# grantjr1842/index-tts

Measured on AMD Instinct MI355X. Metric: synthesised audio seconds per second (IndexTTS-2 infer_v2 hot path), whole job, higher is better.
Workload: dtype f32 (greedy decode + its prefill: exact fp32 MFMA; fp32 accumulate and fp32 activations everywhere) + split-bf16 (fp32 operands as hi+lo bf16, 3 bf16 MFMAs per product) GEMMs, DiT attention and convolutions in s2mel, the latent pass and the vocoder; GPT linear weights STORED as bf16 (rounded once at

## Files before the change

include/idxtts.h:

```cpp
#ifndef IDXTTS_H
#define IDXTTS_H

#include <stddef.h>
#include <stdint.h>

#ifdef __cplusplus
extern "C" {
#endif

typedef struct idxtts_ctx idxtts_ctx;

#define IDXTTS_DTYPE_F32 0
#define IDXTTS_DTYPE_F16 1
#define IDXTTS_DTYPE_BF16 2

int idxtts_version(void);
const char* idxtts_last_error(void);

int idxtts_aa_act_fwd(void* out, const void* in, const float* up_filter, const float* down_filter,
                      const float* log_alpha, const float* log_beta, int B, int C, int T, int dtype,
                      void* stream);

typedef struct idxtts_conv1d idxtts_conv1d;
int idxtts_conv1d_create(const float* weight, const float* bias , int Cout, int Cin, int K,
                         int transposed_stride ,
                         idxtts_conv1d** out);
int idxtts_conv1d_fwd(const idxtts_conv1d* conv, const float* x, float* y, const float* residual ,
                      int B, int T, int dilation, int pad_left, int pad_mode, float scale, int accumulate,
                      void* stream);
int idxtts_conv1d_destroy(idxtts_conv1d* conv);

int idxtts_ctx_load_tensor(idxtts_ctx* ctx, const char* name, const float* data, const int64_t* shape, int ndim);
int idxtts_ctx_finalize(idxtts_ctx* ctx);
int idxtts_ctx_get_tensor(idxtts_ctx* ctx, const char* name, float* host_out, size_t capacity);
int idxtts_ctx_destroy(idxtts_ctx* ctx);
float idxtts_fp8_e4m3_decode(unsigned char code);
unsigned char idxtts_fp8_e4m3_encode(float v);

typedef struct idxtts_bigvgan_config {
  int num_mels;
  int upsample_initial_channel;
  int num_upsamples;
  int upsample_rates[8];
  int upsample_kernel_sizes[8];
  int num_kernels;
  int resblock_kernel_sizes[4];
  int resblock_dilations[4][3];
} idxtts_bigvgan_config;

int idxtts_bigvgan_create(const idxtts_bigvgan_config* cfg, idxtts_ctx** out);
size_t idxtts_bigvgan_workspace_bytes(const idxtts_ctx* ctx, int B, int Tm);
int idxtts_bigvgan_fwd(idxtts_ctx* ctx, const float* mel, float* wav, int B, int Tm, void* workspace,
                       size_t workspace_bytes, int clamp, int stage_idx, float* stage_out, void* stream);
int idxtts_bigvgan_fwd_ragged(idxtts_ctx* ctx, const float* mel, const int* mel_lengths, float* wav, int B, int Tm, void* workspace,
                              size_t workspace_bytes, int clamp, void* stream);

typedef struct idxtts_linear idxtts_linear;
int idxtts_linear_create(const float* weight, const float* bias , int N, int K, int weight_is_kn,
                         idxtts_linear** out);
int idxtts_linear_fwd(const idxtts_linear* lin, const float* x, int ldx, float* y, int ldy, const float* residual ,
                      int ldr, int M, int act, int bf16x3 ,
                      void* stream);
int idxtts_set_gemm_mode(int mode);
int idxtts_get_gemm_mode(void);
int idxtts_set_decode_geometry(int narrow);
int idxtts_get_decode_geometry(void);
int idxtts_set_decode_plane_rows(int min_rows);
int idxtts_get_decode_plane_rows(void);
int idxtts_s2mel_set_overlap(int on);
int idxtts_s2mel_get_overlap(void);
int idxtts_linear_destroy(idxtts_linear* lin);
int idxtts_release_stream(void* stream);
int idxtts_attention_fwd(const float* q, const float* k, const float* v, float* o, long q_batch_stride, int q_token_stride,
                         long kv_batch_stride, int kv_token_stride, long o_batch_stride, int o_token_stride, int B, int H,
                         int Sq, int Sk, int causal, const int* kstart, const int* kend, float scale, void* stream);
int idxtts_attention_bf16x3_fwd(const float* q, const float* k, const float* v, float* o, long q_batch_stride, int q_token_stride,
                         long kv_batch_stride, int kv_token_stride, long o_batch_stride, int o_token_stride, int B, int H,
                         int Sq, int Sk, int causal, const int* kstart, const int* kend, float scale, void* stream);
int idxtts_attention_relkey_fwd(const float* q, const float* k, const float* v, float* o, long batch_stride, int token_stride,
                                long o_batch_stride, int o_token_stride, int B, int H, int S, const int* kend, float scale,
                                const float* rel_key, int rel_left, int rel_right, int split_bf16, void* stream);
int idxtts_layernorm_fwd(const float* x, float* y, const float* gamma, const float* beta, int M, int d, float eps, void* stream);

typedef struct idxtts_gpt_config {
  int model_dim, heads, layers;
  int number_mel_codes;
  int number_text_tokens;
  int start_mel_token, stop_mel_token;
  int mel_pos_len, text_pos_len;
} idxtts_gpt_config;
int idxtts_gpt_create(const idxtts_gpt_config* cfg, idxtts_ctx** out);
int idxtts_gpt_quantize_weights(idxtts_ctx* ctx, int format);
int idxtts_gpt_set_kv_format(idxtts_ctx* ctx, int format);
int idxtts_gpt_get_kv_format(const idxtts_ctx* ctx);
int idxtts_gpt_graph_cache_entries(idxtts_ctx* ctx);
size_t idxtts_gpt_workspace_bytes(const idxtts_ctx* ctx, int B, int S, int max_new_tokens);
int idxtts_gpt_embed(idxtts_ctx* ctx, float* out, int rows, const int* text_ids, const int* text_pos_idx, const int* mel_ids,
                     const int* mel_pos_idx, const float* extra, const int* extra_idx, void* stream);
int idxtts_gpt_generate(idxtts_ctx* ctx, const float* inputs_embeds, const int* pad_left, int B, int P, int max_new_tokens,
                        float repetition_penalty, long long* codes, int* n_steps, float* logits_out, void* workspace,
                        size_t workspace_bytes, int use_graph, void* stream);
int idxtts_gpt_generate_forced(idxtts_ctx* ctx, const float* inputs_embeds, const int* pad_left, int B, int P, int max_new_tokens,
                               float repetition_penalty, const long long* forced_codes, long long* codes, int* n_steps, float* logits_out,
                               void* workspace, size_t workspace_bytes, void* stream);
typedef struct idxtts_sampling {
  int mode;
  float temperature;
  int top_k;
  float top_p;
  const float* exp_noise;
  unsigned long long seed;
} idxtts_sampling;
int idxtts_gpt_generate_sampled(idxtts_ctx* ctx, const float* inputs_embeds, const int* pad_left, int B, int P, int max_new_tokens,
                                float repetition_penalty, const idxtts_sampling* sampling, long long* codes, int* n_steps,
                                float* logits_out, void* workspace, size_t workspace_bytes, int use_graph, void* stream);
typedef struct idxtts_beam {
  int num_beams;
  int do_sample;
  float temperature;
  int top_k;
  float top_p;
  float length_penalty;
  int early_stopping;
  const float* exp_noise;
  unsigned long long seed;
} idxtts_beam;
size_t idxtts_gpt_beam_workspace_bytes(const idxtts_ctx* ctx, int B, int num_beams, int S, int max_new_tokens);
int idxtts_gpt_generate_beam(idxtts_ctx* ctx, const float* inputs_embeds, const int* pad_left, int B, int P, int max_new_tokens,
                             float repetition_penalty, const idxtts_beam* beam, long long* codes, int* n_steps, void* workspace,
                             size_t workspace_bytes, int use_graph, void* stream);
size_t idxtts_gpt_session_workspace_bytes(const idxtts_ctx* ctx, int slots, int max_prompt, int max_new_tokens);
int idxtts_gpt_session_init(idxtts_ctx* ctx, int slots, int max_prompt, int max_new_tokens, float repetition_penalty, void* workspace,
                            size_t workspace_bytes, void* stream);
int idxtts_gpt_session_admit(idxtts_ctx* ctx, int n, const float* inputs_embeds, int ld_rows, const int* prompt_lens,
                             const int* slot_ids, const int* max_new_tokens, void* workspace, void* stream);
#define IDXTTS_SESSION_SAMPLED 1
size_t idxtts_gpt_session_workspace_bytes_ex(const idxtts_ctx* ctx, int slots, int max_prompt, int max_new_tokens, int flags);
int idxtts_gpt_session_init_ex(idxtts_ctx* ctx, int slots, int max_prompt, int max_new_tokens, float repetition_penalty, int flags,
                               void* workspace, size_t workspace_bytes, void* stream);
int idxtts_gpt_session_admit_sampled(idxtts_ctx* ctx, int n, const float* inputs_embeds, int ld_rows, const int* prompt_lens,
                                     const int* slot_ids, const int* max_new_tokens, const idxtts_sampling* per_row, void* workspace,
                                     void* stream);
size_t idxtts_gpt_session_workspace_bytes_beam(const idxtts_ctx* ctx, int slots, int num_beams, int max_prompt, int max_new_tokens);
int idxtts_gpt_session_init_beam(idxtts_ctx* ctx, int slots, int num_beams, int max_prompt, int max_new_tokens, float repetition_penalty,
                                 void* workspace, size_t workspace_bytes, void* stream);
int idxtts_gpt_session_admit_beam(idxtts_ctx* ctx, int n, const float* inputs_embeds, int ld_rows, const int* prompt_lens,
                                  const int* group_ids, const int* max_new_tokens, const idxtts_beam* per_request, void* workspace,
                                  void* stream);
int idxtts_gpt_session_step(idxtts_ctx* ctx, int n_steps, int use_graph, int* finished_slots, int* n_finished, void* workspace,
                            void* stream);
int idxtts_gpt_session_read(idxtts_ctx* ctx, int slot, long long* codes, int* n_codes, void* workspace, void* stream);
int idxtts_gpt_session_release(idxtts_ctx* ctx, void* workspace);
int idxtts_gpt_latent(idxtts_ctx* ctx, const float* emb, const int* pad_left, int B, int S, int mel_start, int M, float* latent,
                      void* workspace, size_t workspace_bytes, void* stream);

typedef struct idxtts_cond_config {
  int input_size;
  int output_size, linear_units, attention_heads, num_blocks, cnn_kernel;
  int perceiver_dim, num_latents, perceiver_depth, perceiver_dim_head, perceiver_mult;
  int emotion;
  int model_dim;
} idxtts_cond_config;
int idxtts_cond_create(const idxtts_cond_config* cfg, idxtts_ctx** out);
size_t idxtts_cond_workspace_bytes(const idxtts_ctx* ctx, int B, int T);
int idxtts_cond_forward(idxtts_ctx* ctx, const float* feats, const int* lengths, int B, int T, float* out, void* workspace,
                        size_t workspace_bytes, void* stream);
int idxtts_emovec_merge(float* out, const float* base, const float* emo, float alpha, size_t n, void* stream);

typedef struct idxtts_w2vbert_config {
  int input_dim, hidden_size, num_heads, intermediate_size;
  int num_layers;
  int left_max, right_max, conv_kernel;
  float layer_norm_eps;
} idxtts_w2vbert_config;
int idxtts_w2vbert_create(const idxtts_w2vbert_config* cfg, idxtts_ctx** out);
size_t idxtts_w2vbert_workspace_bytes(const idxtts_ctx* ctx, int B, int T);
int idxtts_w2vbert_forward(idxtts_ctx* ctx, const float* feats, const int* lengths, int B, int T, float* out, void* workspace,
                           size_t workspace_bytes, void* stream);

typedef struct idxtts_repcodec_config {
  int hidden_size, codebook_size, codebook_dim;
  int vocos_dim, vocos_intermediate_dim, vocos_num_layers;
} idxtts_repcodec_config;
int idxtts_repcodec_create(const idxtts_repcodec_config* cfg, idxtts_ctx** out);
size_t idxtts_repcodec_workspace_bytes(const idxtts_ctx* ctx, int B, int T);
int idxtts_repcodec_quantize(idxtts_ctx* ctx, const float* x, int B, int T, long long* indices, float* quantized, void* workspace,
                             size_t workspace_bytes, void* stream);

typedef struct idxtts_melspec_config {
  int n_fft, hop_size, win_size, num_mels;
} idxtts_melspec_config;
int idxtts_melspec_create(const idxtts_melspec_config* cfg, idxtts_ctx** out);
int idxtts_melspec_frames(const idxtts_ctx* ctx, int n_samples);
size_t idxtts_melspec_workspace_bytes(const idxtts_ctx* ctx, int B, int n_samples);
int idxtts_melspec_forward(idxtts_ctx* ctx, const float* audio, int B, int n_samples, float* mel, void* workspace, size_t workspace_bytes,
                           void* stream);

typedef struct idxtts_campplus_config {
  int feat_dim, embedding_size;
  int m_channels, growth_rate, bn_size, init_channels;
  int num_blocks;
  int block_layers[4], block_dilation[4];
} idxtts_campplus_config;
int idxtts_campplus_create(const idxtts_campplus_config* cfg, idxtts_ctx** out);
size_t idxtts_campplus_workspace_bytes(const idxtts_ctx* ctx, int T);
int idxtts_campplus_forward(idxtts_ctx* ctx, const float* feat, int B, int T, float* style, void* workspace, size_t workspace_bytes, void* stream);

typedef struct idxtts_s2mel_config {
  int hidden_dim, num_heads, depth;
  int in_channels, content_dim, style_dim;
  int wn_hidden, wn_layers, wn_kernel, wn_dilation_rate;
  int lr_channels, lr_in_channels, lr_num_convs;
  int gpt_dim; int gpt_layer_dims[3];
  int codebook_size, codebook_dim, codec_hidden;
  float norm_eps;
} idxtts_s2mel_config;
int idxtts_s2mel_create(const idxtts_s2mel_config* cfg, idxtts_ctx** out);
size_t idxtts_s2mel_cond_workspace_bytes(const idxtts_ctx* ctx, int B, int M, int Tg);
int idxtts_s2mel_prepare_cond(idxtts_ctx* ctx, const float* latent, const long long* codes, const int* code_lens,
                              const int* target_lens, int B, int M, int Tg, float* cond_out, void* workspace,
                              size_t workspace_bytes, void* stream);
int idxtts_s2mel_regulate(idxtts_ctx* ctx, const float* S, const int* in_lens, const int* target_lens, int B, int M, int Tg, float* cond_out,
                          void* workspace, size_t workspace_bytes, void* stream);
size_t idxtts_s2mel_cfm_workspace_bytes(const idxtts_ctx* ctx, int B, int T, int n_steps);
int idxtts_s2mel_cfm(idxtts_ctx* ctx, const float* mu, const int* x_lens, const float* prompt, const int* prompt_lens, int Tp_max,
                     const float* style, const float* z, const float* t_emb, const float* dt, int n_steps, float cfg_rate,
                     float* out, int B, int T, void* workspace, size_t workspace_bytes, void* stream);

size_t idxtts_s2mel_cfm_rows_workspace_bytes(const idxtts_ctx* ctx, int B, int T, int Tp_max, int n_steps);
int idxtts_s2mel_cfm_rows(idxtts_ctx* ctx, const float* gen_cond, const int* target_lens, int Tg_max, const float* const* prompt_conditions,
                          const float* const* ref_mels, const int* prompt_lens, const float* style, const float* z, const float* t_emb,
                          const float* dt, int n_steps, float cfg_rate, float* out, int B, int T, void* workspace, size_t workspace_bytes,
                          void* stream);

int idxtts_s2mel_estimator(idxtts_ctx* ctx, const float* x, const float* prompt, const int* prompt_lens, int Tp_max, const int* x_lens,
                           const float* t_emb, const float* style, const float* mu, float* out, int B, int T, void* workspace,
                           size_t workspace_bytes, void* stream);

typedef struct idxtts_qwen_config {
  int vocab_size;
  int hidden_size;
  int intermediate_size;
  int num_hidden_layers;
  int num_attention_heads;
  int num_key_value_heads;
  int head_dim;
  float rms_norm_eps;
  float rope_theta;
  int tie_word_embeddings;
  int max_context;
} idxtts_qwen_config;
int idxtts_qwen_create(const idxtts_qwen_config* cfg, idxtts_ctx** out);
int idxtts_qwen_set_weight_format(idxtts_ctx* ctx, int format);
size_t idxtts_qwen_workspace_bytes(const idxtts_ctx* ctx, int n_prompt, int max_new_tokens, int n_eos, int n_logit_cols );
int idxtts_qwen_generate(idxtts_ctx* ctx, const int* prompt_ids, int n_prompt, int max_new_tokens, const int* eos_ids, int n_eos,
                         const int* forced_ids , int* out_ids, int* n_out, float* out_logits ,
                         const int* logit_cols , int n_logit_cols, void* workspace, size_t bytes, int use_graph,
                         void* stream);
int idxtts_qwen_step_graph_launches(const idxtts_ctx* ctx);
int idxtts_qwen_max_batch(const idxtts_ctx* ctx);
size_t idxtts_qwen_batch_workspace_bytes(const idxtts_ctx* ctx, int B, const int* n_prompt, const int* max_new_tokens, int n_eos,
                                         int n_logit_cols );
int idxtts_qwen_generate_batch(idxtts_ctx* ctx, int B, const int* prompt_ids, const int* n_prompt, const int* max_new_tokens,
                               const int* eos_ids, int n_eos, const int* forced_ids , int* out_ids, int* n_out,
                               float* out_logits , const int* logit_cols , int n_logit_cols,
                               void* workspace, size_t bytes, int use_graph, void* stream);
int idxtts_qwen_batch_step_graph_launches(const idxtts_ctx* ctx);

int idxtts_profile_enable(int on);
int idxtts_profile_num_kernels(void);
const char* idxtts_profile_kernel_name(int index);
int idxtts_profile_read(int index, double* total_ms, double* flops, double* bytes, long* launches);
int idxtts_profile_event_overhead(void* stream, int launches, double* avg_ms);

#ifdef __cplusplus
}
#endif
#endif
```

index-tts_amd/csrc/capi.hip:

```cpp
#include <cstring>
#include <new>

#include "../../include/idxtts.h"
#include "bigvgan.h"
#include "cond.h"
#include "semantic.h"
#include "codec.h"
#include "audio.h"
#include "campplus.h"
#include "conv1d.h"
#include "ctx.h"
#include "gpt.h"
#include "model_util.h"
#include "s2mel.h"

namespace idxtts {

static thread_local std::string g_last_error;

void set_error(const std::string& msg) { g_last_error = msg; }
int fail(const char* file, int line, const std::string& msg) {
  const char* base = std::strrchr(file, '/');
  g_last_error = std::string(base ? base + 1 : file) + ":" + std::to_string(line) + ": " + msg;
  return 1;
// ... 466 lines not shown
                               static_cast<hipStream_t>(stream));
  API_END
}

int idxtts_gpt_session_step(idxtts_ctx* ctx, int n_steps, int use_graph, int* finished_slots, int* n_finished, void* workspace,
                            void* stream) {
  API_BEGIN
  GPT_MODEL(ctx);
  return m->session_step(workspace, n_steps, use_graph, finished_slots, n_finished, static_cast<hipStream_t>(stream));
  API_END
}

int idxtts_gpt_session_read(idxtts_ctx* ctx, int slot, long long* codes, int* n_codes, void* workspace, void* stream) {
  API_BEGIN
  GPT_MODEL(ctx);
  return m->session_read(workspace, slot, codes, n_codes, static_cast<hipStream_t>(stream));
  API_END
}

int idxtts_gpt_session_release(idxtts_ctx* ctx, void* workspace) {
  API_BEGIN
  GPT_MODEL(ctx);
  return m->session_release(workspace);
  API_END
}

int idxtts_gpt_latent(idxtts_ctx* ctx, const float* emb, const int* pad_left, int B, int S, int mel_start, int M, float* latent,
                      void* workspace, size_t workspace_bytes, void* stream) {
  API_BEGIN
  GPT_MODEL(ctx);
  return m->latent(emb, pad_left, B, S, mel_start, M, latent, workspace, workspace_bytes, static_cast<hipStream_t>(stream));
  API_END
}


int idxtts_cond_create(const idxtts_cond_config* cfg, idxtts_ctx** out) {
  API_BEGIN
  IDX_CHECK(cfg && out, "null pointer");
  std::unique_ptr<idxtts_ctx> ctx(new idxtts_ctx());
  ctx->model.reset(new CondModel(*cfg));
  *out = ctx.release();
  return 0;
  API_END
}

size_t idxtts_cond_workspace_bytes(const idxtts_ctx* ctx, int B, int T) {
  if (!ctx || !ctx->finalized || B <= 0 || T < 3) return 0;
  auto* m = dynamic_cast<const CondModel*>(ctx->model.get());
  return m ? m->workspace_bytes(B, T) : 0;
}

int idxtts_cond_forward(idxtts_ctx* ctx, const float* feats, const int* lengths, int B, int T, float* out, void* workspace,
                        size_t workspace_bytes, void* stream) {
  API_BEGIN
  IDX_CHECK(ctx, "null ctx");
  IDX_CHECK(ctx->finalized, "context not finalized");
  auto* m = dynamic_cast<CondModel*>(ctx->model.get());
  IDX_CHECK(m, "not a conditioning-encoder context");
  return m->forward(feats, lengths, B, T, out, workspace, workspace_bytes, static_cast<hipStream_t>(stream));
  API_END
}

int idxtts_w2vbert_create(const idxtts_w2vbert_config* cfg, idxtts_ctx** out) {
  API_BEGIN
  IDX_CHECK(cfg && out, "null pointer");
  std::unique_ptr<idxtts_ctx> ctx(new idxtts_ctx());
  ctx->model.reset(new W2VBertModel(*cfg));
  *out = ctx.release();
  return 0;
  API_END
}

size_t idxtts_w2vbert_workspace_bytes(const idxtts_ctx* ctx, int B, int T) {
  if (!ctx || !ctx->finalized || B <= 0 || T <= 0) return 0;
  auto* m = dynamic_cast<const W2VBertModel*>(ctx->model.get());
  return m ? m->workspace_bytes(B, T) : 0;
}

int idxtts_w2vbert_forward(idxtts_ctx* ctx, const float* feats, const int* lengths, int B, int T, float* out, void* workspace,
                           size_t workspace_bytes, void* stream) {
  API_BEGIN
  IDX_CHECK(ctx, "null ctx");
  IDX_CHECK(ctx->finalized, "context not finalized");
  auto* m = dynamic_cast<W2VBertModel*>(ctx->model.get());
  IDX_CHECK(m, "not a w2v-bert context");
  return m->forward(feats, lengths, B, T, out, workspace, workspace_bytes, static_cast<hipStream_t>(stream));
  API_END
}

int idxtts_repcodec_create(const idxtts_repcodec_config* cfg, idxtts_ctx** out) {
  API_BEGIN
  IDX_CHECK(cfg && out, "null pointer");
  std::unique_ptr<idxtts_ctx> ctx(new idxtts_ctx());
  ctx->model.reset(new RepCodecModel(*cfg));
  *out = ctx.release();
  return 0;
  API_END
}

size_t idxtts_repcodec_workspace_bytes(const idxtts_ctx* ctx, int B, int T) {
  if (!ctx || !ctx->finalized || B <= 0 || T <= 0) return 0;
  auto* m = dynamic_cast<const RepCodecModel*>(ctx->model.get());
  return m ? m->workspace_bytes(B, T) : 0;
}

int idxtts_repcodec_quantize(idxtts_ctx* ctx, const float* x, int B, int T, long long* indices, float* quantized, void* workspace,
                             size_t workspace_bytes, void* stream) {
  API_BEGIN
  IDX_CHECK(ctx, "null ctx");
  IDX_CHECK(ctx->finalized, "context not finalized");
  auto* m = dynamic_cast<RepCodecModel*>(ctx->model.get());
  IDX_CHECK(m, "not a semantic-codec context");
  return m->quantize(x, B, T, indices, quantized, workspace, workspace_bytes, static_cast<hipStream_t>(stream));
  API_END
}

int idxtts_melspec_create(const idxtts_melspec_config* cfg, idxtts_ctx** out) {
  API_BEGIN
  IDX_CHECK(cfg && out, "null pointer");
  std::unique_ptr<idxtts_ctx> ctx(new idxtts_ctx());
  ctx->model.reset(new MelSpecModel(*cfg));
  *out = ctx.release();
  return 0;
  API_END
}

int idxtts_melspec_frames(const idxtts_ctx* ctx, int n_samples) {
  if (!ctx || n_samples <= 0) return 0;
  auto* m = dynamic_cast<const MelSpecModel*>(ctx->model.get());
  return m ? m->frames(n_samples) : 0;
}

size_t idxtts_melspec_workspace_bytes(const idxtts_ctx* ctx, int B, int n_samples) {
  if (!ctx || !ctx->finalized || B <= 0 || n_samples <= 0) return 0;
  auto* m = dynamic_cast<const MelSpecModel*>(ctx->model.get());
  return m ? m->workspace_bytes(B, n_samples) : 0;
}

int idxtts_melspec_forward(idxtts_ctx* ctx, const float* audio, int B, int n_samples, float* mel, void* workspace, size_t workspace_bytes,
                           void* stream) {
  API_BEGIN
  IDX_CHECK(ctx, "null ctx");
  IDX_CHECK(ctx->finalized, "context not finalized");
  auto* m = dynamic_cast<MelSpecModel*>(ctx->model.get());
  IDX_CHECK(m, "not a mel-spectrogram context");
  return m->forward(audio, B, n_samples, mel, workspace, workspace_bytes, static_cast<hipStream_t>(stream));
  API_END
}

int idxtts_campplus_create(const idxtts_campplus_config* cfg, idxtts_ctx** out) {
  API_BEGIN
  IDX_CHECK(cfg && out, "null pointer");
  std::unique_ptr<idxtts_ctx> ctx(new idxtts_ctx());
  ctx->model.reset(new CamPPlusModel(*cfg));
  *out = ctx.release();
  return 0;
  API_END
}

size_t idxtts_campplus_workspace_bytes(const idxtts_ctx* ctx, int T) {
  if (!ctx || !ctx->finalized || T < 8) return 0;
  auto* m = dynamic_cast<const CamPPlusModel*>(ctx->model.get());
  return m ? m->workspace_bytes(T) : 0;
}

int idxtts_campplus_forward(idxtts_ctx* ctx, const float* feat, int B, int T, float* style, void* workspace, size_t workspace_bytes, void* stream) {
  API_BEGIN
  IDX_CHECK(ctx, "null ctx");
  IDX_CHECK(ctx->finalized, "context not finalized");
  auto* m = dynamic_cast<CamPPlusModel*>(ctx->model.get());
  IDX_CHECK(m, "not a CAMPPlus context");
  return m->forward(feat, B, T, style, workspace, workspace_bytes, static_cast<hipStream_t>(stream));
  API_END
}

int idxtts_emovec_merge(float* out, const float* base, const float* emo, float alpha, size_t n, void* stream) {
  API_BEGIN
  return lerp_rows(out, base, emo, alpha, n, static_cast<hipStream_t>(stream));
  API_END
}

int idxtts_s2mel_create(const idxtts_s2mel_config* cfg, idxtts_ctx** out) {
  API_BEGIN
  IDX_CHECK(cfg && out, "null pointer");
  std::unique_ptr<idxtts_ctx> ctx(new idxtts_ctx());
  ctx->model.reset(new S2MelModel(*cfg));
  *out = ctx.release();
  return 0;
  API_END
}

#define S2MEL_MODEL(ctx)                                      \
  IDX_CHECK(ctx, "null ctx");                                 \
  IDX_CHECK(ctx->finalized, "context not finalized");         \
  auto* m = dynamic_cast<S2MelModel*>(ctx->model.get());      \
  IDX_CHECK(m, "not an s2mel context")

size_t idxtts_s2mel_cond_workspace_bytes(const idxtts_ctx* ctx, int B, int M, int Tg) {
  if (!ctx || !ctx->finalized || B <= 0 || M <= 0 || Tg <= 0) return 0;
  auto* m = dynamic_cast<const S2MelModel*>(ctx->model.get());
  return m ? m->cond_workspace_bytes(B, M, Tg) : 0;
}

int idxtts_s2mel_prepare_cond(idxtts_ctx* ctx, const float* latent, const long long* codes, const int* code_lens,
                              const int* target_lens, int B, int M, int Tg, float* cond_out, void* workspace,
                              size_t workspace_bytes, void* stream) {
  API_BEGIN
  S2MEL_MODEL(ctx);
  return m->prepare_cond(latent, codes, code_lens, target_lens, B, M, Tg, cond_out, workspace, workspace_bytes,
                         static_cast<hipStream_t>(stream));
  API_END
}

int idxtts_s2mel_regulate(idxtts_ctx* ctx, const float* S, const int* in_lens, const int* target_lens, int B, int M, int Tg, float* cond_out,
                          void* workspace, size_t workspace_bytes, void* stream) {
  API_BEGIN
  S2MEL_MODEL(ctx);
  return m->regulate(S, in_lens, target_lens, B, M, Tg, cond_out, workspace, workspace_bytes, static_cast<hipStream_t>(stream));
  API_END
}

size_t idxtts_s2mel_cfm_workspace_bytes(const idxtts_ctx* ctx, int B, int T, int n_steps) {
  if (!ctx || !ctx->finalized || B <= 0 || T <= 0 || n_steps <= 0) return 0;
  auto* m = dynamic_cast<const S2MelModel*>(ctx->model.get());
  return m ? m->cfm_workspace_bytes(B, T, n_steps) : 0;
}

int idxtts_s2mel_cfm(idxtts_ctx* ctx, const float* mu, const int* x_lens, const float* prompt, const int* prompt_lens, int Tp_max,
                     const float* style, const float* z, const float* t_emb, const float* dt, int n_steps, float cfg_rate,
                     float* out, int B, int T, void* workspace, size_t workspace_bytes, void* stream) {
  API_BEGIN
  S2MEL_MODEL(ctx);
  return m->cfm(mu, x_lens, prompt, prompt_lens, Tp_max, style, z, t_emb, dt, n_steps, cfg_rate, out, B, T, workspace,
                workspace_bytes, static_cast<hipStream_t>(stream));
  API_END
}

size_t idxtts_s2mel_cfm_rows_workspace_bytes(const idxtts_ctx* ctx, int B, int T, int Tp_max, int n_steps) {
  if (!ctx || !ctx->finalized || B <= 0 || T <= 0 || Tp_max <= 0 || n_steps <= 0) return 0;
  auto* m = dynamic_cast<const S2MelModel*>(ctx->model.get());
  return m ? m->cfm_rows_workspace_bytes(B, T, Tp_max, n_steps) : 0;
}

int idxtts_s2mel_cfm_rows(idxtts_ctx* ctx, const float* gen_cond, const int* target_lens, int Tg_max, const float* const* prompt_conditions,
                          const float* const* ref_mels, const int* prompt_lens, const float* style, const float* z, const float* t_emb,
                          const float* dt, int n_steps, float cfg_rate, float* out, int B, int T, void* workspace, size_t workspace_bytes,
                          void* stream) {
  API_BEGIN
  S2MEL_MODEL(ctx);
  return m->cfm_rows(gen_cond, target_lens, Tg_max, prompt_conditions, ref_mels, prompt_lens, style, z, t_emb, dt, n_steps, cfg_rate, out,
                     B, T, workspace, workspace_bytes, static_cast<hipStream_t>(stream));
  API_END
}

int idxtts_s2mel_estimator(idxtts_ctx* ctx, const float* x, const float* prompt, const int* prompt_lens, int Tp_max, const int* x_lens,
                           const float* t_emb, const float* style, const float* mu, float* out, int B, int T, void* workspace,
                           size_t workspace_bytes, void* stream) {
  API_BEGIN
  S2MEL_MODEL(ctx);
  return m->estimator(x, prompt, prompt_lens, Tp_max, x_lens, t_emb, style, mu, out, B, T, workspace, workspace_bytes,
                      static_cast<hipStream_t>(stream));
  API_END
}


int idxtts_set_gemm_mode(int mode) {
  set_gemm_mode(mode);
  return 0;
}

int idxtts_get_gemm_mode(void) { return get_gemm_mode(); }

int idxtts_set_decode_geometry(int narrow) {
  set_decode_geometry(narrow);
  return 0;
}

int idxtts_get_decode_geometry(void) { return get_decode_geometry(); }

int idxtts_release_stream(void* stream) {
  API_BEGIN
  hipStream_t st = static_cast<hipStream_t>(stream);
  return gemm_release_stream_scratch(st) || s2mel_release_stream(st);
  API_END
}

int idxtts_set_decode_plane_rows(int min_rows) {
  API_BEGIN
  IDX_CHECK(min_rows == 0 || (min_rows >= 5 && min_rows <= 65), "0 (default), 5..64 or 65 (off)");
  set_decode_plane_rows(min_rows);
  return 0;
  API_END
}

int idxtts_get_decode_plane_rows(void) { return get_decode_plane_rows(); }

int idxtts_s2mel_set_overlap(int on) {
  set_s2mel_overlap(on);
  return 0;
}

int idxtts_s2mel_get_overlap(void) { return get_s2mel_overlap(); }

}
```

index-tts_amd/csrc/gemm.h:

```cpp
#pragma once
#include "common.h"

namespace idxtts {

enum GemmAct { ACT_NONE = 0, ACT_GELU_NEW = 1, ACT_SILU = 2, ACT_SWIGLU = 3, ACT_MISH = 4, ACT_GATE = 5 ,
               ACT_GELU_ERF = 6 , ACT_RELU = 7  };

struct LinearWeights {
  const float* wp = nullptr;
  const float* bias = nullptr;
  int N = 0, K = 0;
  const void* wp16 = nullptr;
};

static inline size_t linear_packed_floats(int N, int K) { return (size_t)cdiv(N, 32) * cdiv(K, 16) * 512; }

void pack_linear(float* dst, const float* w, int N, int K);

struct GemmArgs {
  const float* x = nullptr; int ldx = 0;
  float* y = nullptr; int ldy = 0;
  const void* x_planes = nullptr;
  void* y_planes = nullptr;
  const float* rope = nullptr; int rope_T = 0, rope_cols = 0;
  const float* res = nullptr; int ldr = 0;
  int M = 0;
  int act = ACT_NONE;
  float out_scale = 1.0f;
  int taps = 1, seq_len = 0, dil = 1, pad_left = 0, pad_mode = 0;
  const int* row_len = nullptr;
  int ksplit = 1;
};

int gemm_tn_forward(const LinearWeights& w, const GemmArgs& a, hipStream_t stream);
int gemm_bf16x3_forward(const LinearWeights& w, const GemmArgs& a, hipStream_t stream);
size_t linear_bf16x3_packed_bytes(int N, int K);
void pack_linear_bf16x3(void* dst, const float* w, int N, int K);

enum GemmMode { GEMM_F32 = 0, GEMM_BF16X3 = 1 };
void set_gemm_mode(int mode);
int get_gemm_mode();
int gemm_forward(const LinearWeights& w, const GemmArgs& a, hipStream_t stream);
bool gemm_uses_planes(const LinearWeights& w, const GemmArgs& a);

int gemm_release_stream_scratch(hipStream_t stream);

}
```

index-tts_amd/csrc/gemm.hip:

```cpp
#include <algorithm>
#include <cmath>

#include "device_util.h"
#include "gemm_common.h"
#include "prof.h"

namespace idxtts {

void pack_linear(float* dst, const float* w, int N, int K) {
  const int NT = cdiv(N, 32), KC = cdiv(K, 16);
  for (int nt = 0; nt < NT; ++nt)
    for (int c = 0; c < KC; ++c) {
      float* sub = dst + ((size_t)nt * KC + c) * 512;
      for (int g = 0; g < 2; ++g)
        for (int h = 0; h < 2; ++h)
          for (int j = 0; j < 32; ++j)
            for (int e = 0; e < 4; ++e) {
              const int n = nt * 32 + j, k = c * 16 + 8 * g + 4 * h + e;
              sub[((g * 2 + h) * 32 + j) * 4 + e] = (n < N && k < K) ? w[(size_t)n * K + k] : 0.0f;
            }
    }
}

constexpr int XBLK = 132;

int StreamScratch::acquire(hipStream_t stream, size_t bytes, void** out, bool* grew) {
  int dev_id = 0;
  IDX_HIP(hipGetDevice(&dev_id));
  Block* b = nullptr;
  {
    std::lock_guard<std::mutex> lock(mu_);
    b = &blocks_[std::make_pair(dev_id, stream)];
  }
  const bool grow = b->bytes < bytes;
  if (grew) *grew = grow;
  if (grow) {
    if (b->ptr) IDX_HIP(hipFreeAsync(b->ptr, stream));
    b->ptr = nullptr; b->bytes = 0;
    const size_t nb = bytes + (headroom_div_ ? bytes / headroom_div_ : 0);
    IDX_HIP(hipMallocAsync(&b->ptr, nb, stream));
    b->bytes = nb;
  }
  *out = b->ptr;
  return 0;
}

int StreamScratch::release(hipStream_t stream) {
  int dev_id = 0;
  IDX_HIP(hipGetDevice(&dev_id));
  Block b;
  {
    std::lock_guard<std::mutex> lock(mu_);
    auto it = blocks_.find(std::make_pair(dev_id, stream));
    if (it == blocks_.end()) return 0;
    b = it->second;
    blocks_.erase(it);
  }
  if (b.ptr) IDX_HIP(hipFreeAsync(b.ptr, stream));
  return 0;
}

static StreamScratch g_sk_scratch;
int gemm_release_stream_scratch(hipStream_t stream) { return g_plane_scratch.release(stream) || g_sk_scratch.release(stream); }

__global__ __launch_bounds__(256) void gemm_tn_kernel(const GemmKP p) {
  extern __shared__ __attribute__((aligned(16))) float smem[];
  float (*Xs)[4 * 2 * 4 * XBLK] = reinterpret_cast<float (*)[4 * 2 * 4 * XBLK]>(smem);
  float (*Ws)[4 * 2 * 512] = reinterpret_cast<float (*)[4 * 2 * 512]>(smem + 2 * 4 * 2 * 4 * XBLK);

  const int L = blockIdx.x, xcd = L & 7, q = L >> 3;
  int bn, bm;
  if (p.direct_map) { bn = L / p.mtiles; bm = L - bn * p.mtiles; }
  else if (p.n_fast) { const int bml = q / p.nblocks; bn = q - bml * p.nblocks; bm = bml * 8 + xcd; }
  else { bn = q / p.mt8; bm = (q - bn * p.mt8) * 8 + xcd; }
  if (bm >= p.mtiles) return;

  const int tid = threadIdx.x, wave = tid >> 6, lane = tid & 63;
  const int h = lane >> 5, j = lane & 31;
  const int wm = wave >> 1, wn = wave & 1;

  f32x4 xr[4], wr[4];
  int seq_base[4], seq_t[4], seq_n[4];
  if (p.taps > 1) {
#pragma unroll
    for (int l = 0; l < 4; ++l) {
      const int m = bm * 128 + ((tid + 256 * l) >> 3);
      const int sb = m / p.seq_len;
      seq_base[l] = sb * p.seq_len;
      seq_t[l] = m - sb * p.seq_len;
      seq_n[l] = (p.row_len && m < p.M) ? min(p.row_len[sb], p.seq_len) : p.seq_len;
    }
  }
  auto load_tiles = [&](int kstep) {
    int tap = 0, kk0 = kstep * 32;
    if (p.taps > 1) { tap = kk0 / p.kc; kk0 -= tap * p.kc; }
#pragma unroll
    for (int l = 0; l < 4; ++l) {
      const int idx = tid + 256 * l;
      const int row = idx >> 3, q8 = idx & 7;
      const int m = bm * 128 + row, k = kstep * 32 + q8 * 4;
      f32x4 v = {0.f, 0.f, 0.f, 0.f};
      if (p.taps > 1) {
        int t = seq_t[l] + tap * p.dil - p.pad_left;
        if (p.pad_mode == 1) { t = t < 0 ? -t : t; t = t >= seq_n[l] ? 2 * (seq_n[l] - 1) - t : t; }
        if (m < p.M && k < p.K && t >= 0 && t < seq_n[l])
          v = *reinterpret_cast<const f32x4*>(p.x + (size_t)(seq_base[l] + t) * p.ldx + kk0 + q8 * 4);
      } else if (m < p.M && k < p.K) {
        v = *reinterpret_cast<const f32x4*>(p.x + (size_t)m * p.ldx + k);
      }
      xr[l] = v;
      const int nt = idx >> 8, off = idx & 255;
      const int ntg = bn * 4 + nt, c16 = kstep * 2 + (off >> 7);
      f32x4 u = {0.f, 0.f, 0.f, 0.f};
      if (ntg * 32 < p.N && c16 < p.kc16)
        u = *reinterpret_cast<const f32x4*>(p.wp + ((size_t)ntg * p.kc16 + c16) * 512 + (off & 127) * 4);
      wr[l] = u;
    }
  };
  auto store_tiles = [&](int buf) {
#pragma unroll
    for (int l = 0; l < 4; ++l) {
      const int idx = tid + 256 * l;
      const int row = idx >> 3, q8 = idx & 7;
      const int mt = row >> 5, i = row & 31, c = q8 >> 2, gh = q8 & 3;
      *reinterpret_cast<f32x4*>(&Xs[buf][((mt * 2 + c) * 4 + gh) * XBLK + i * 4]) = xr[l];
      const int nt = idx >> 8, off = idx & 255;
      *reinterpret_cast<f32x4*>(&Ws[buf][nt * 1024 + off * 4]) = wr[l];
    }
  };

  f32x16 acc[2][2], tot[2][2];
#pragma unroll
  for (int a = 0; a < 2; ++a)
#pragma unroll
    for (int b = 0; b < 2; ++b)
#pragma unroll
      for (int r = 0; r < 16; ++r) { acc[a][b][r] = 0.0f; tot[a][b][r] = 0.0f; }

  int ksteps = (p.kc16 + 1) >> 1, ks0 = 0;
  if (p.ksplit > 1) { ks0 = blockIdx.y * p.ksteps_per_split; ksteps = min(ksteps, ks0 + p.ksteps_per_split); }
  int in_group = ks0 % p.kg;
  load_tiles(ks0);
  store_tiles(ks0 & 1);
  __syncthreads();
  for (int ks = ks0; ks < ksteps; ++ks) {
    const bool has_next = ks + 1 < ksteps;
    if (has_next) load_tiles(ks + 1);
    const float* xb = Xs[ks & 1];
    const float* wb = Ws[ks & 1];
#pragma unroll
    for (int c = 0; c < 2; ++c)
#pragma unroll
      for (int g = 0; g < 2; ++g) {
        f32x4 a[2], b[2];
#pragma unroll
        for (int t = 0; t < 2; ++t) {
          a[t] = *reinterpret_cast<const f32x4*>(xb + (((wm * 2 + t) * 2 + c) * 4 + (g * 2 + h)) * XBLK + j * 4);
          b[t] = *reinterpret_cast<const f32x4*>(wb + (wn * 2 + t) * 1024 + c * 512 + (g * 64 + lane) * 4);
        }
#pragma unroll
        for (int s = 0; s < 4; ++s)
#pragma unroll
          for (int mt = 0; mt < 2; ++mt)
#pragma unroll
            for (int nt = 0; nt < 2; ++nt)
              acc[mt][nt] = __builtin_amdgcn_mfma_f32_32x32x2f32(a[mt][s], b[nt][s], acc[mt][nt], 0, 0, 0);
      }
    if (++in_group == p.kg || !has_next) {
      in_group = 0;
#pragma unroll
      for (int mt = 0; mt < 2; ++mt)
#pragma unroll
        for (int nt = 0; nt < 2; ++nt)
#pragma unroll
          for (int r = 0; r < 16; ++r) { tot[mt][nt][r] += acc[mt][nt][r]; acc[mt][nt][r] = 0.0f; }
    }
    if (has_next) store_tiles((ks + 1) & 1);
    __syncthreads();
  }

  if (p.sk_cnt) {
    const __amdgpu_buffer_rsrc_t rs = __builtin_amdgcn_make_buffer_rsrc(p.sk_slab, 0, p.sk_slab_bytes, 0x00020000);
    const int tile = bm * p.nblocks + bn, ntiles = p.mtiles * p.nblocks;
    const int part_stride = ntiles * 16 * 256 * 16;
    const int mine = (tile * 16 * 256 + tid) * 16;
#pragma unroll
    for (int mt = 0; mt < 2; ++mt)
#pragma unroll
      for (int nt = 0; nt < 2; ++nt)
#pragma unroll
        for (int r4 = 0; r4 < 4; ++r4) {
          const f32x4 v = {tot[mt][nt][4 * r4], tot[mt][nt][4 * r4 + 1], tot[mt][nt][4 * r4 + 2], tot[mt][nt][4 * r4 + 3]};
          __builtin_amdgcn_raw_buffer_store_b128(__builtin_bit_cast(u32x4, v), rs, mine + ((mt * 2 + nt) * 4 + r4) * 4096, (int)blockIdx.y * part_stride, 17);
        }
    if (!wg_arrive_last(&p.sk_cnt[tile], (unsigned)p.ksplit)) return;
#pragma unroll
    for (int mt = 0; mt < 2; ++mt)
#pragma unroll
      for (int nt = 0; nt < 2; ++nt)
#pragma unroll
        for (int r = 0; r < 16; ++r) tot[mt][nt][r] = 0.0f;
    for (int g = 0; g < p.ksplit; ++g) {
      u32x4 t[16];
#pragma unroll
      for (int u = 0; u < 16; ++u) t[u] = __builtin_amdgcn_raw_buffer_load_b128(rs, mine + u * 4096, g * part_stride, 16);
#pragma unroll
      for (int u = 0; u < 16; ++u) {
        const f32x4 v = __builtin_bit_cast(f32x4, t[u]);
#pragma unroll
        for (int e = 0; e < 4; ++e) tot[u >> 3][(u >> 2) & 1][4 * (u & 3) + e] += v[e];
      }
    }
    gemm_epilogue(p, tot, bm, bn, wm, wn, h, j);
    return;
  }
  if (p.ksplit > 1) {
    GemmKP q = p;
    q.y = p.y + (size_t)blockIdx.y * p.M * p.ldy;
    q.bias = nullptr; q.res = nullptr; q.row_len = nullptr; q.act = ACT_NONE; q.out_scale = 1.0f;
    gemm_epilogue(q, tot, bm, bn, wm, wn, h, j);
    return;
  }
  gemm_epilogue(p, tot, bm, bn, wm, wn, h, j);
}

int gemm_prepare(const LinearWeights& w, const GemmArgs& a, GemmKP* out, double* flops, double* bytes) {
  IDX_CHECK(a.M > 0 && w.N > 0 && w.K > 0, "bad shape");
  IDX_CHECK((w.K & 3) == 0 && (a.ldx & 3) == 0, "K and ldx must be multiples of 4 (16-byte row segments)");
  IDX_CHECK((reinterpret_cast<uintptr_t>(a.x) & 15) == 0, "x must be 16-byte aligned");
  if (a.act == ACT_SWIGLU || a.act == ACT_GATE) IDX_CHECK((w.N & 63) == 0, "paired activations need N (= 2*hidden) to be a multiple of 64");
  if (a.taps > 1) {
    IDX_CHECK(a.seq_len > 0 && a.M % a.seq_len == 0 && w.K % a.taps == 0 && ((w.K / a.taps) & 31) == 0, "conv mode: K/taps must be a multiple of 32 and M a multiple of seq_len");
    if (a.pad_mode == 1) IDX_CHECK(a.seq_len > (a.taps - 1) * a.dil, "reflect pad needs seq_len > halo");
  }
  if (a.row_len) IDX_CHECK(a.seq_len > 0, "row_len needs seq_len");
  GemmKP p;
  p.x = a.x; p.wp = w.wp; p.bias = w.bias; p.res = a.res; p.y = a.y; p.y_hi = p.y_lo = nullptr; p.rope = nullptr; p.rope_T = 1; p.rope_cols = 0;
  p.M = a.M; p.N = w.N; p.K = w.K; p.ldx = a.ldx; p.ldy = a.ldy; p.ldr = a.ldr;
  p.kc16 = cdiv(w.K, 16);
  p.mtiles = cdiv(a.M, 128);
  p.mt8 = cdiv(p.mtiles, 8);
  p.nblocks = cdiv(w.N, 128);
  p.n_fast = ((double)w.N * w.K * 4.0 <= 8.0 * 1024 * 1024) && a.M > w.N ? 1 : 0;
  p.act = a.act; p.out_scale = a.out_scale;
  p.taps = a.taps; p.kc = w.K / std::max(1, a.taps); p.seq_len = a.seq_len > 0 ? a.seq_len : 1; p.dil = a.dil; p.pad_left = a.pad_left;
  p.pad_mode = a.pad_mode; p.row_len = a.row_len;
  p.ksplit = 1; p.ksteps_per_split = 0;
  p.kg = 0; p.direct_map = 0; p.sk_slab = nullptr; p.sk_cnt = nullptr; p.sk_slab_bytes = 0;
  IDX_CHECK((int64_t)8 * p.nblocks * p.mt8 < (1ll << 31), "grid size");
  *out = p;
  *flops = 2.0 * a.M * (double)w.N * w.K;
  *bytes = 4.0 * ((double)a.M * w.K + (double)w.N * w.K + (double)a.M * w.N * (a.res ? 2.0 : 1.0));
  return 0;
}

int gemm_tn_forward(const LinearWeights& w, const GemmArgs& a, hipStream_t stream) {
  IDX_CHECK(w.wp && a.x && a.y, "null pointer");
  if (a.M == 0) return 0;
  IDX_CHECK(!a.y_planes && !a.rope, "the fp32 GEMM takes and produces fp32 rows only (no fused rotary)");
  GemmKP p;
  double flops, bytes;
  if (gemm_prepare(w, a, &p, &flops, &bytes)) return 1;
  p.ksplit = std::max(1, a.ksplit);
  p.ksteps_per_split = cdiv(cdiv(p.kc16, 2), p.ksplit);
  if (p.ksplit > 1) {
    IDX_CHECK(a.taps <= 1 && a.act == ACT_NONE && !a.res && !a.row_len, "split-K launches produce raw partial slabs");
    IDX_CHECK((p.ksplit - 1) * p.ksteps_per_split < cdiv(p.kc16, 2), "ksplit leaves an empty K range");
  }
  const int ksteps_all = cdiv(p.kc16, 2);
  p.kg = std::max(5, cdiv(ksteps_all, 8));
  const int ngroups = cdiv(ksteps_all, p.kg);
  const int tiles = p.nblocks * p.mtiles;
  if (p.ksplit == 1 && tiles <= 96 && ngroups >= 2) {
    const size_t slab_bytes = (size_t)ngroups * tiles * 65536, cnt_bytes = 4096;
    static_assert(96 * 4 <= 4096, "arrival counters");
    void* sc = nullptr;
    bool grew = false;
    if (g_sk_scratch.acquire(stream, cnt_bytes + slab_bytes, &sc, &grew)) return 1;
    if (grew) IDX_HIP(hipMemsetAsync(sc, 0, cnt_bytes, stream));
    p.sk_cnt = static_cast<unsigned*>(sc);
    p.sk_slab = reinterpret_cast<float*>(static_cast<char*>(sc) + cnt_bytes);
    p.sk_slab_bytes = (int)slab_bytes;
    p.ksplit = ngroups; p.ksteps_per_split = p.kg;
  }
  if (tiles <= 96) p.direct_map = 1;
  const int64_t grid = p.direct_map ? (int64_t)tiles : (int64_t)8 * p.nblocks * p.mt8;
  static const int cat = prof_register("gemm_tn_kernel");
  ProfScope prof(cat, stream, flops, bytes);
  constexpr size_t lds = (size_t)(2 * 4 * 2 * 4 * XBLK + 2 * 4 * 2 * 512) * sizeof(float);
  static DynLdsLimit lds_limit;
  IDX_HIP(lds_limit.set((int)lds, gemm_tn_kernel));
  hipLaunchKernelGGL(gemm_tn_kernel, dim3((unsigned)grid, (unsigned)p.ksplit), dim3(256), lds, stream, p);
  IDX_LAUNCH_CHECK();
  return 0;
}

static int g_gemm_mode = GEMM_BF16X3;
void set_gemm_mode(int mode) { g_gemm_mode = mode == GEMM_F32 ? GEMM_F32 : GEMM_BF16X3; }
int get_gemm_mode() { return g_gemm_mode; }

bool gemm_bf16x3_uses_v2(const LinearWeights& w, const GemmArgs& a);
bool gemm_uses_planes(const LinearWeights& w, const GemmArgs& a) {
  return g_gemm_mode == GEMM_BF16X3 && w.wp16 && a.M >= 256 && gemm_bf16x3_uses_v2(w, a);
}
int gemm_forward(const LinearWeights& w, const GemmArgs& a, hipStream_t stream) {
  if (g_gemm_mode == GEMM_BF16X3 && w.wp16 && a.M >= 256) return gemm_bf16x3_forward(w, a, stream);
  return gemm_tn_forward(w, a, stream);
}

}
```

index-tts_amd/csrc/gemm_bf16x3.hip:

```cpp
#include <algorithm>
#include <cmath>
#include <cstdlib>
#include <cstring>

#include "gemm_common.h"
#include "prof.h"

namespace idxtts {

__device__ __forceinline__ int cdiv_dev(int a, int b) { return (a + b - 1) / b; }

typedef __bf16 bf16x8 __attribute__((ext_vector_type(8)));
typedef __bf16 bf16x4 __attribute__((ext_vector_type(4)));

constexpr int BROW = 40;
constexpr int TILE_HALF = 128 * BROW;
constexpr int WTILE_BYTES = 2 * TILE_HALF * 2;

size_t linear_planes_bytes(int N, int K);
void pack_linear_planes(void* dst, const float* w, int N, int K);
bool gemm_bf16x3_uses_v2(const LinearWeights& w, const GemmArgs& a);
int gemm_bf16x3_v2_forward(GemmKP p, const void* wplanes, const LinearWeights& w, const GemmArgs& a, hipStream_t stream, double flops,
                           double bytes);
bool gemm_bf16x3_uses_v2(const LinearWeights& w, const GemmArgs& a) {
  return w.wp16 && a.M >= 256 && w.N >= 96 && w.K % 16 == 0 && (a.taps <= 1 || (w.K / a.taps) % 16 == 0);
}
static size_t tiles_bytes(int N, int K) { return (size_t)cdiv(N, 128) * cdiv(K, 32) * WTILE_BYTES; }
size_t linear_bf16x3_packed_bytes(int N, int K) { return tiles_bytes(N, K) + linear_planes_bytes(N, K); }

void pack_linear_bf16x3(void* dst, const float* w, int N, int K) {
  uint16_t* o = static_cast<uint16_t*>(dst);
  const int NB = cdiv(N, 128), KS = cdiv(K, 32);
  std::memset(o, 0, tiles_bytes(N, K));
  pack_linear_planes(static_cast<char*>(dst) + tiles_bytes(N, K), w, N, K);
  for (int nb = 0; nb < NB; ++nb)
    for (int ks = 0; ks < KS; ++ks) {
      uint16_t* tile = o + ((size_t)nb * KS + ks) * (2 * TILE_HALF);
      for (int r = 0; r < 128; ++r) {
        const int n = nb * 128 + r;
        if (n >= N) break;
        for (int kk = 0; kk < 32; ++kk) {
          const int k = ks * 32 + kk;
          if (k >= K) break;
          const float x = w[(size_t)n * K + k];
          const uint16_t hi = f2bf(x);
          tile[r * BROW + kk] = hi;
          tile[TILE_HALF + r * BROW + kk] = f2bf(x - bf2f(hi));
        }
      }
    }
}

__global__ __launch_bounds__(256) void gemm_bf16x3_kernel(const GemmKP p) {
  extern __shared__ __attribute__((aligned(16))) __bf16 sm16[];
  __bf16* As = sm16;
  __bf16* Bs = sm16 + 2 * 2 * TILE_HALF;

  const int L = blockIdx.x, xcd = L & 7, q = L >> 3;
  int bn, bm;
  if (p.n_fast) { const int bml = q / p.nblocks; bn = q - bml * p.nblocks; bm = bml * 8 + xcd; }
  else { bn = q / p.mt8; bm = (q - bn * p.mt8) * 8 + xcd; }
  if (bm >= p.mtiles) return;

  const int tid = threadIdx.x, wave = tid >> 6, lane = tid & 63;
  const int h = lane >> 5, j = lane & 31;
  const int wm = wave >> 1, wn = wave & 1;
  const int ksteps = (p.K + 31) >> 5;

  f32x4 xr[4];
  f32x4 wr[5];
  int seq_base[4], seq_t[4], seq_n[4];
  if (p.taps > 1) {
#pragma unroll
    for (int l = 0; l < 4; ++l) {
      const int m = bm * 128 + ((tid + 256 * l) >> 3);
      const int sb = m / p.seq_len;
      seq_base[l] = sb * p.seq_len;
      seq_t[l] = m - sb * p.seq_len;
      seq_n[l] = (p.row_len && m < p.M) ? min(p.row_len[sb], p.seq_len) : p.seq_len;
    }
  }
  const char* wtile0 = reinterpret_cast<const char*>(p.wp) + (size_t)bn * ksteps * WTILE_BYTES;
  auto load_tiles = [&](int kstep) {
    int tap = 0, kk0 = kstep * 32;
    if (p.taps > 1) { tap = kk0 / p.kc; kk0 -= tap * p.kc; }
#pragma unroll
    for (int l = 0; l < 4; ++l) {
      const int idx = tid + 256 * l;
      const int row = idx >> 3, q8 = idx & 7;
      const int m = bm * 128 + row, k = kstep * 32 + q8 * 4;
      f32x4 v = {0.f, 0.f, 0.f, 0.f};
      if (p.taps > 1) {
        int t = seq_t[l] + tap * p.dil - p.pad_left;
        if (p.pad_mode == 1) { t = t < 0 ? -t : t; t = t >= seq_n[l] ? 2 * (seq_n[l] - 1) - t : t; }
        if (m < p.M && k < p.K && t >= 0 && t < seq_n[l])
          v = *reinterpret_cast<const f32x4*>(p.x + (size_t)(seq_base[l] + t) * p.ldx + kk0 + q8 * 4);
      } else if (m < p.M && k < p.K) {
        v = *reinterpret_cast<const f32x4*>(p.x + (size_t)m * p.ldx + k);
      }
      xr[l] = v;
    }
    const f32x4* wsrc = reinterpret_cast<const f32x4*>(wtile0 + (size_t)kstep * WTILE_BYTES);
#pragma unroll
    for (int l = 0; l < 5; ++l) wr[l] = wsrc[tid + 256 * l];
  };
  auto store_tiles = [&](int buf) {
    __bf16* a_hi = As + buf * 2 * TILE_HALF;
    __bf16* a_lo = a_hi + TILE_HALF;
#pragma unroll
    for (int l = 0; l < 4; ++l) {
      const int idx = tid + 256 * l;
      const int row = idx >> 3, q8 = idx & 7;
      const bf16x4 hi = __builtin_convertvector(xr[l], bf16x4);
      const f32x4 back = __builtin_convertvector(hi, f32x4);
      const bf16x4 lo = __builtin_convertvector(xr[l] - back, bf16x4);
      *reinterpret_cast<bf16x4*>(a_hi + row * BROW + q8 * 4) = hi;
      *reinterpret_cast<bf16x4*>(a_lo + row * BROW + q8 * 4) = lo;
    }
    f32x4* wdst = reinterpret_cast<f32x4*>(Bs + buf * 2 * TILE_HALF);
#pragma unroll
    for (int l = 0; l < 5; ++l) wdst[tid + 256 * l] = wr[l];
  };

  f32x16 acc[2][2];
#pragma unroll
  for (int a = 0; a < 2; ++a)
#pragma unroll
    for (int b = 0; b < 2; ++b)
#pragma unroll
      for (int r = 0; r < 16; ++r) acc[a][b][r] = 0.0f;

  load_tiles(0);
  store_tiles(0);
  __syncthreads();
  for (int ks = 0; ks < ksteps; ++ks) {
    const bool has_next = ks + 1 < ksteps;
    if (has_next) load_tiles(ks + 1);
    const __bf16* a_hi = As + (ks & 1) * 2 * TILE_HALF;
    const __bf16* b_hi = Bs + (ks & 1) * 2 * TILE_HALF;
#pragma unroll
    for (int s = 0; s < 2; ++s) {
      bf16x8 ah[2], al[2], bh[2], bl[2];
#pragma unroll
      for (int t = 0; t < 2; ++t) {
        const int ar = (wm * 64 + t * 32 + j) * BROW + s * 16 + h * 8;
        const int br = (wn * 64 + t * 32 + j) * BROW + s * 16 + h * 8;
        ah[t] = *reinterpret_cast<const bf16x8*>(a_hi + ar);
        al[t] = *reinterpret_cast<const bf16x8*>(a_hi + TILE_HALF + ar);
        bh[t] = *reinterpret_cast<const bf16x8*>(b_hi + br);
        bl[t] = *reinterpret_cast<const bf16x8*>(b_hi + TILE_HALF + br);
      }
#pragma unroll
      for (int mt = 0; mt < 2; ++mt)
#pragma unroll
        for (int nt = 0; nt < 2; ++nt) {
          acc[mt][nt] = __builtin_amdgcn_mfma_f32_32x32x16_bf16(al[mt], bh[nt], acc[mt][nt], 0, 0, 0);
          acc[mt][nt] = __builtin_amdgcn_mfma_f32_32x32x16_bf16(ah[mt], bl[nt], acc[mt][nt], 0, 0, 0);
          acc[mt][nt] = __builtin_amdgcn_mfma_f32_32x32x16_bf16(ah[mt], bh[nt], acc[mt][nt], 0, 0, 0);
        }
    }
    if (has_next) store_tiles((ks + 1) & 1);
    __syncthreads();
  }
  gemm_epilogue(p, acc, bm, bn, wm, wn, h, j);
}

template <int TN>
__global__ __launch_bounds__(512) void gemm_bf16x3_big_kernel(const GemmKP p) {
  constexpr int BN = 64 * TN;
  constexpr int NB128 = BN / 128 > 0 ? BN / 128 : 1;
  constexpr int A_HALF = 256 * BROW;
  constexpr int B_HALF = TILE_HALF;
  constexpr int A_STAGE = 2 * A_HALF, B_STAGE = NB128 * 2 * B_HALF;
  constexpr int NWL = (NB128 * 1280 + 511) / 512;
  static_assert(BN == 128 || BN == 256, "tile");
  extern __shared__ __attribute__((aligned(16))) __bf16 sm16[];
  __bf16* As = sm16;
  __bf16* Bs = sm16 + 2 * A_STAGE;

  const int L = blockIdx.x, xcd = L & 7, q = L >> 3;
  int bn, bm;
  if (p.n_fast) { const int bml = q / p.nblocks; bn = q - bml * p.nblocks; bm = bml * 8 + xcd; }
  else { bn = q / p.mt8; bm = (q - bn * p.mt8) * 8 + xcd; }
  if (bm >= p.mtiles) return;

  const int tid = threadIdx.x, wave = tid >> 6, lane = tid & 63;
  const int h = lane >> 5, j = lane & 31;
  const int wm = wave >> 1, wn = wave & 1;
  const int ksteps = (p.K + 31) >> 5;

  f32x4 xr[4];
  f32x4 wr[NWL];
  int seq_base[4], seq_t[4], seq_n[4];
  if (p.taps > 1) {
#pragma unroll
    for (int l = 0; l < 4; ++l) {
      const int m = bm * 256 + ((tid + 512 * l) >> 3);
      const int sb = m / p.seq_len;
      seq_base[l] = sb * p.seq_len;
      seq_t[l] = m - sb * p.seq_len;
      seq_n[l] = (p.row_len && m < p.M) ? min(p.row_len[sb], p.seq_len) : p.seq_len;
    }
  }
  const int n128 = cdiv_dev(p.N, 128);
  auto load_tiles = [&](int kstep) {
    int tap = 0, kk0 = kstep * 32;
    if (p.taps > 1) { tap = kk0 / p.kc; kk0 -= tap * p.kc; }
#pragma unroll
    for (int l = 0; l < 4; ++l) {
      const int idx = tid + 512 * l;
      const int row = idx >> 3, q8 = idx & 7;
      const int m = bm * 256 + row, k = kstep * 32 + q8 * 4;
      f32x4 v = {0.f, 0.f, 0.f, 0.f};
      if (p.taps > 1) {
        int t = seq_t[l] + tap * p.dil - p.pad_left;
        if (p.pad_mode == 1) { t = t < 0 ? -t : t; t = t >= seq_n[l] ? 2 * (seq_n[l] - 1) - t : t; }
        if (m < p.M && k < p.K && t >= 0 && t < seq_n[l])
          v = *reinterpret_cast<const f32x4*>(p.x + (size_t)(seq_base[l] + t) * p.ldx + kk0 + q8 * 4);
      } else if (m < p.M && k < p.K) {
        v = *reinterpret_cast<const f32x4*>(p.x + (size_t)m * p.ldx + k);
      }
      xr[l] = v;
    }
#pragma unroll
    for (int l = 0; l < NWL; ++l) {
      const int idx = tid + 512 * l;
      const int sub = idx / 1280, off = idx - sub * 1280;
      const int nb = bn * NB128 + sub;
      f32x4 v = {0.f, 0.f, 0.f, 0.f};
      if (idx < NB128 * 1280 && nb < n128)
        v = reinterpret_cast<const f32x4*>(reinterpret_cast<const char*>(p.wp) + ((size_t)nb * ksteps + kstep) * WTILE_BYTES)[off];
      wr[l] = v;
    }
  };
  auto store_tiles = [&](int buf) {
    __bf16* a_hi = As + buf * A_STAGE;
    __bf16* a_lo = a_hi + A_HALF;
#pragma unroll
    for (int l = 0; l < 4; ++l) {
      const int idx = tid + 512 * l;
      const int row = idx >> 3, q8 = idx & 7;
      const bf16x4 hi = __builtin_convertvector(xr[l], bf16x4);
      const f32x4 back = __builtin_convertvector(hi, f32x4);
      const bf16x4 lo = __builtin_convertvector(xr[l] - back, bf16x4);
      *reinterpret_cast<bf16x4*>(a_hi + row * BROW + q8 * 4) = hi;
      *reinterpret_cast<bf16x4*>(a_lo + row * BROW + q8 * 4) = lo;
    }
    f32x4* wdst = reinterpret_cast<f32x4*>(Bs + buf * B_STAGE);
#pragma unroll
    for (int l = 0; l < NWL; ++l) {
      const int idx = tid + 512 * l;
      if (idx < NB128 * 1280) wdst[idx] = wr[l];
    }
  };

  f32x16 acc[2][TN];
#pragma unroll
  for (int a = 0; a < 2; ++a)
#pragma unroll
    for (int b = 0; b < TN; ++b)
#pragma unroll
      for (int r = 0; r < 16; ++r) acc[a][b][r] = 0.0f;

  load_tiles(0);
  store_tiles(0);
  __syncthreads();
  for (int ks = 0; ks < ksteps; ++ks) {
    const bool has_next = ks + 1 < ksteps;
    if (has_next) load_tiles(ks + 1);
    const __bf16* a_hi = As + (ks & 1) * A_STAGE;
    const __bf16* b_st = Bs + (ks & 1) * B_STAGE;
#pragma unroll
    for (int s = 0; s < 2; ++s) {
      bf16x8 ah[2], al[2], bh[TN], bl[TN];
#pragma unroll
      for (int t = 0; t < 2; ++t) {
        const int ar = (wm * 64 + t * 32 + j) * BROW + s * 16 + h * 8;
        ah[t] = *reinterpret_cast<const bf16x8*>(a_hi + ar);
        al[t] = *reinterpret_cast<const bf16x8*>(a_hi + A_HALF + ar);
      }
#pragma unroll
      for (int t = 0; t < TN; ++t) {
        const int col = wn * 32 * TN + t * 32 + j;
        const __bf16* bt = b_st + (col >> 7) * 2 * B_HALF + (col & 127) * BROW + s * 16 + h * 8;
        bh[t] = *reinterpret_cast<const bf16x8*>(bt);
        bl[t] = *reinterpret_cast<const bf16x8*>(bt + B_HALF);
      }
#pragma unroll
      for (int mt = 0; mt < 2; ++mt)
#pragma unroll
        for (int nt = 0; nt < TN; ++nt) {
          acc[mt][nt] = __builtin_amdgcn_mfma_f32_32x32x16_bf16(al[mt], bh[nt], acc[mt][nt], 0, 0, 0);
          acc[mt][nt] = __builtin_amdgcn_mfma_f32_32x32x16_bf16(ah[mt], bl[nt], acc[mt][nt], 0, 0, 0);
          acc[mt][nt] = __builtin_amdgcn_mfma_f32_32x32x16_bf16(ah[mt], bh[nt], acc[mt][nt], 0, 0, 0);
        }
    }
    if (has_next) store_tiles((ks + 1) & 1);
    __syncthreads();
  }
  gemm_epilogue_t<2, TN>(p, acc, bm * 256 + wm * 64, bn * BN + wn * 32 * TN, h, j);
}

template <int TN>
static int launch_big(GemmKP p, const LinearWeights& w, const GemmArgs& a, hipStream_t stream, double flops, double bytes) {
  constexpr int BN = 64 * TN, NB128 = BN / 128;
  p.mtiles = cdiv(a.M, 256);
  p.mt8 = cdiv(p.mtiles, 8);
  p.nblocks = cdiv(w.N, BN);
  const int64_t grid = (int64_t)8 * p.nblocks * p.mt8;
  IDX_CHECK(grid < (1ll << 31), "grid size");
  constexpr size_t lds = (size_t)(2 * 2 * 256 * BROW + 2 * NB128 * 2 * TILE_HALF) * sizeof(__bf16);
  static DynLdsLimit lds_limit;
  IDX_HIP(lds_limit.set((int)lds, gemm_bf16x3_big_kernel<TN>));
  static const int cat = prof_register(TN == 2 ? "gemm_bf16x3_big_kernel<2>" : "gemm_bf16x3_big_kernel<4>");
  ProfScope prof(cat, stream, flops, bytes);
  hipLaunchKernelGGL(gemm_bf16x3_big_kernel<TN>, dim3((unsigned)grid), dim3(512), lds, stream, p);
  IDX_LAUNCH_CHECK();
  return 0;
}

int gemm_bf16x3_forward(const LinearWeights& w, const GemmArgs& a, hipStream_t stream) {
  IDX_CHECK(w.wp16 && (a.x || a.x_planes) && (a.y || a.y_planes), "null pointer (split-bf16 weights not packed?)");
  if (a.M == 0) return 0;
  if (a.x_planes || a.y_planes || !a.x || !a.y || a.rope) IDX_CHECK(gemm_bf16x3_uses_v2(w, a), "operand planes are only understood by the LDS-DMA kernel (shape not eligible)");
  IDX_CHECK(a.ksplit <= 1, "split-K is a feature of the exact-fp32 kernel");
  GemmKP p;
  double flops, bytes;
  if (gemm_prepare(w, a, &p, &flops, &bytes)) return 1;
  p.wp = reinterpret_cast<const float*>(w.wp16);
  if (gemm_bf16x3_uses_v2(w, a))
    return gemm_bf16x3_v2_forward(p, static_cast<const char*>(w.wp16) + tiles_bytes(w.N, w.K), w, a, stream, flops, bytes);
  if (a.M >= 4096) {
    const bool paired = a.act == ACT_SWIGLU || a.act == ACT_GATE;
    if (w.N >= 256 && !paired) return launch_big<4>(p, w, a, stream, flops, bytes);
    return launch_big<2>(p, w, a, stream, flops, bytes);
  }
  constexpr size_t lds = (size_t)(2 * 2 * 2 * TILE_HALF) * sizeof(__bf16);
  static DynLdsLimit lds_limit;
  IDX_HIP(lds_limit.set((int)lds, gemm_bf16x3_kernel));
  static const int cat = prof_register("gemm_bf16x3_kernel");
  ProfScope prof(cat, stream, flops, bytes);
  hipLaunchKernelGGL(gemm_bf16x3_kernel, dim3((unsigned)(8 * p.nblocks * p.mt8)), dim3(256), lds, stream, p);
  IDX_LAUNCH_CHECK();
  return 0;
}

}
```

index-tts_amd/csrc/gemm_bf16x3_v2.hip:

```cpp
#include <algorithm>
#include <cstdlib>
#include <cstring>

#include "gemm_common.h"
#include "prof.h"

namespace idxtts {

typedef __bf16 bf16x8 __attribute__((ext_vector_type(8)));
typedef __bf16 bf16x4 __attribute__((ext_vector_type(4)));

size_t linear_planes_bytes(int N, int K) { return (size_t)2 * cdiv(K, 16) * (cdiv(N, 256) * 256) * 16 * sizeof(uint16_t); }

void pack_linear_planes(void* dst, const float* w, int N, int K) {
  uint16_t* o = static_cast<uint16_t*>(dst);
  const int KC = cdiv(K, 16), NP = cdiv(N, 256) * 256;
  std::memset(o, 0, linear_planes_bytes(N, K));
  uint16_t* lo = o + (size_t)KC * NP * 16;
  for (int n = 0; n < N; ++n)
    for (int k = 0; k < K; ++k) {
      const float x = w[(size_t)n * K + k];
      const uint16_t hi = f2bf(x);
      const size_t idx = ((size_t)(k >> 4) * NP + n) * 16 + (k & 15);
      o[idx] = hi;
      lo[idx] = f2bf(x - bf2f(hi));
    }
}

__global__ __launch_bounds__(256) void split_planes_kernel(const float* __restrict__ x, int ldx, int M, int K, __bf16* __restrict__ hi,
                                                           __bf16* __restrict__ lo) {
  const int k = blockIdx.y * 64 + (threadIdx.x & 15) * 4;
#pragma unroll
  for (int i = 0; i < 4; ++i) {
    const int m = blockIdx.x * 64 + (threadIdx.x >> 4) + 16 * i;
    if (m >= M || k >= ((K + 15) & ~15)) continue;
    const f32x4 v = k < K ? *reinterpret_cast<const f32x4*>(x + (size_t)m * ldx + k) : f32x4{0.f, 0.f, 0.f, 0.f};
    bf16x4 h, l;
    split_bf16_x4(v, h, l);
    const size_t o = ((size_t)(k >> 4) * M + m) * 16 + (k & 15);
    *reinterpret_cast<bf16x4*>(hi + o) = h;
    *reinterpret_cast<bf16x4*>(lo + o) = l;
  }
}

#ifdef V2_TIMING
static unsigned long long* g_v2_stamps = nullptr;
extern "C" int idxtts_dbg_v2_stamps(void* buf) { g_v2_stamps = static_cast<unsigned long long*>(buf); return 0; }
#define V2_STAMP(k) do { if (q.stamps && tid == 64) q.stamps[(size_t)blockIdx.x * 8 + (k)] = __builtin_amdgcn_s_memtime(); } while (0)
#define V2_RSTAMP(k) do { if (q.stamps && tid == 64) q.stamps[(size_t)blockIdx.x * 8 + (k)] = __builtin_amdgcn_s_memrealtime(); } while (0)
#else
#define V2_STAMP(k)
#define V2_RSTAMP(k)
#endif

struct GemmV2P {
  GemmKP g;
  const __bf16* a_hi; const __bf16* a_lo;
  const __bf16* b_hi; const __bf16* b_lo;
  int a_rows, npad, nstages;
  int a_bytes, b_bytes;
  int a_plane, b_plane;
  int cs, nbg;
#ifdef V2_TIMING
  unsigned long long* stamps;
#endif
};

struct V2Rsrc { __amdgpu_buffer_rsrc_t a, b; };

#define V2_WAITCNT(vm) __builtin_amdgcn_s_waitcnt(((vm) & 15) | (((vm) >> 4) << 14) | 0x70)

template <bool TAPS, int EPI, int CFG>
__device__ __forceinline__ void gemm_v2_tile(const GemmV2P& q, const int bm, const int bn, const int tid) {
  constexpr int NSTAGE = CFG ? 3 : 4;
  constexpr int WMW = CFG ? 2 : 4, WNW = 2, TN = CFG ? 2 : 4;
  constexpr int BM = 64 * WMW, BN = 32 * TN * WNW;
  static_assert(BM / 32 == WMW * WNW && BN / 32 == WMW * WNW, "one 32-row block of A and of B per wave and plane");
  constexpr int PLANE = BM * 32;
  constexpr int STAGE_BYTES = 4 * PLANE;
  constexpr int PPW = 4;
  const GemmKP& p = q.g;
  extern __shared__ __attribute__((aligned(1024))) char smv2[];

  const int wave = __builtin_amdgcn_readfirstlane(tid >> 6), lane = tid & 63;
  const int h = lane >> 5, j = lane & 31;
  const int wm = wave >> 1, wn = wave & 1;

  const int lrow = lane >> 1;
  const int dunit = (lane & 1) ^ ((lrow >> 3) & 1);
  const int a_m = bm * BM + 32 * wave + lrow;
  const __amdgpu_buffer_rsrc_t rA = __builtin_amdgcn_make_buffer_rsrc(const_cast<__bf16*>(q.a_hi), 0, q.a_bytes, 0x00020000);
  const __amdgpu_buffer_rsrc_t rB = __builtin_amdgcn_make_buffer_rsrc(const_cast<__bf16*>(q.b_hi), 0, q.b_bytes, 0x00020000);
  const int voffB = (bn * BN + 32 * wave + lrow) * 32 + dunit * 16;
  int voffA = min(a_m, q.a_rows - 1) * 32 + dunit * 16;
  int seq_base = 0, seq_t = 0, seq_n = 0;
  if (TAPS) {
    const int sb = a_m / p.seq_len;
    seq_base = sb * p.seq_len;
    seq_t = a_m - seq_base;
    seq_n = (p.row_len && a_m < p.M) ? min(p.row_len[sb], p.seq_len) : p.seq_len;
  }
  auto tap_voff = [&](int tap) -> int {
    int t = seq_t + tap * p.dil - p.pad_left;
    if (p.pad_mode == 1) { t = t < 0 ? -t : t; t = t >= seq_n ? 2 * (seq_n - 1) - t : t; }
    const bool ok = a_m < p.M && t >= 0 && t < seq_n;
    return ok ? (seq_base + t) * 32 + dunit * 16 : (int)0x80000000;
  };
  V2_STAMP(0); V2_RSTAMP(4);
  const int ns = q.nstages;
  const int sA = q.a_rows * 32, sB = q.npad * 32;
  const int cpt = TAPS ? (p.kc >> 4) : ns;
  int ist = 0, soA = 0, soB = 0, ich = 0, itap = 0, wslot = 0, rslot = 0;
  if (TAPS) voffA = tap_voff(0);
  char* const lds_w = smv2 + wave * 1024;
  auto issue_piece = [&](int pi) {
    auto dst = (__attribute__((address_space(3))) void*)(lds_w + wslot * STAGE_BYTES + pi * PLANE);
    if (pi == 0) __builtin_amdgcn_raw_ptr_buffer_load_lds(rA, dst, 16, voffA, soA, 0, 0);
    else if (pi == 1) __builtin_amdgcn_raw_ptr_buffer_load_lds(rA, dst, 16, voffA, soA + q.a_plane, 0, 0);
    else if (pi == 2) __builtin_amdgcn_raw_ptr_buffer_load_lds(rB, dst, 16, voffB, soB, 0, 0);
    else __builtin_amdgcn_raw_ptr_buffer_load_lds(rB, dst, 16, voffB, soB + q.b_plane, 0, 0);
  };
  auto advance = [&]() {
    ++ist;
    wslot = wslot + 1 == NSTAGE ? 0 : wslot + 1;
    soB += sB;
    soA += sA;
    if (TAPS) {
      if (++ich == cpt) { ich = 0; soA = 0; ++itap; voffA = tap_voff(itap); }
    }
  };

  const int sw = (h ^ ((j >> 3) & 1)) * 16;
  const int a_off = (wm * 64 + j) * 32 + sw;
  const int b_offr = (wn * TN * 32 + j) * 32 + sw;

  f32x16 acc[2][TN];
#pragma unroll
  for (int a = 0; a < 2; ++a)
#pragma unroll
    for (int b = 0; b < TN; ++b)
#pragma unroll
      for (int r = 0; r < 16; ++r) acc[a][b][r] = 0.0f;

  for (int s = 0; s < NSTAGE; ++s)
    if (s < ns) {
#pragma unroll
      for (int pi = 0; pi < PPW; ++pi) issue_piece(pi);
      advance();
    }

  struct Frag { bf16x8 ah[2], al[2], bh[TN], bl[TN]; };
  auto wait_stage = [&](int s) {
    const int rem = ns - 1 - s;
    if (NSTAGE >= 4 && rem >= 2) V2_WAITCNT(2 * PPW);
    else if (NSTAGE >= 3 && rem >= 1) V2_WAITCNT(PPW);
    else V2_WAITCNT(0);
    __builtin_amdgcn_s_barrier();
    __builtin_amdgcn_sched_barrier(0);
  };
  auto load_frags = [&](Frag& f) {
    const char* st = smv2 + rslot * STAGE_BYTES;
    rslot = rslot + 1 == NSTAGE ? 0 : rslot + 1;
#pragma unroll
    for (int t = 0; t < 2; ++t) {
      f.ah[t] = *reinterpret_cast<const bf16x8*>(st + a_off + t * 1024);
      f.al[t] = *reinterpret_cast<const bf16x8*>(st + PLANE + a_off + t * 1024);
    }
#pragma unroll
    for (int t = 0; t < TN; ++t) {
      f.bh[t] = *reinterpret_cast<const bf16x8*>(st + 2 * PLANE + b_offr + t * 1024);
      f.bl[t] = *reinterpret_cast<const bf16x8*>(st + 3 * PLANE + b_offr + t * 1024);
    }
  };
  auto compute = [&](const Frag& f, const bool more) {
#define V2_MFMA3(mt, nt)                                                                                         \
    acc[mt][nt] = __builtin_amdgcn_mfma_f32_32x32x16_bf16(f.al[mt], f.bh[nt], acc[mt][nt], 0, 0, 0);             \
    acc[mt][nt] = __builtin_amdgcn_mfma_f32_32x32x16_bf16(f.ah[mt], f.bl[nt], acc[mt][nt], 0, 0, 0);             \
    acc[mt][nt] = __builtin_amdgcn_mfma_f32_32x32x16_bf16(f.ah[mt], f.bh[nt], acc[mt][nt], 0, 0, 0);
    if constexpr (TN == 4) { V2_MFMA3(0, 0) V2_MFMA3(0, 1) } else { V2_MFMA3(0, 0) }
    __builtin_amdgcn_sched_barrier(0);
    if (more) issue_piece(0);
    __builtin_amdgcn_sched_barrier(0);
    if constexpr (TN == 4) { V2_MFMA3(0, 2) V2_MFMA3(0, 3) } else { V2_MFMA3(0, 1) }
    __builtin_amdgcn_sched_barrier(0);
    if (more) issue_piece(1);
    __builtin_amdgcn_sched_barrier(0);
    if constexpr (TN == 4) { V2_MFMA3(1, 0) V2_MFMA3(1, 1) } else { V2_MFMA3(1, 0) }
    __builtin_amdgcn_sched_barrier(0);
    if (more) issue_piece(2);
    __builtin_amdgcn_sched_barrier(0);
    if constexpr (TN == 4) { V2_MFMA3(1, 2) V2_MFMA3(1, 3) } else { V2_MFMA3(1, 1) }
    __builtin_amdgcn_sched_barrier(0);
    if (more) { issue_piece(3); advance(); }
    __builtin_amdgcn_sched_barrier(0);
#undef V2_MFMA3
  };

  Frag f0, f1;
  {
    const int rem = ns - 1;
    if (NSTAGE >= 4 && rem >= 3) V2_WAITCNT(3 * PPW);
    else if (NSTAGE >= 3 && rem >= 2) V2_WAITCNT(2 * PPW);
    else if (rem >= 1) V2_WAITCNT(PPW);
    else V2_WAITCNT(0);
    __builtin_amdgcn_s_barrier();
    __builtin_amdgcn_sched_barrier(0);
  }
  V2_STAMP(1);
  load_frags(f0);
  int i = 0;
  for (; i + NSTAGE + 1 < ns; i += 2) {
    V2_WAITCNT((NSTAGE - 2) * PPW);
    __builtin_amdgcn_s_barrier();
    __builtin_amdgcn_sched_barrier(0);
    load_frags(f1);
    compute(f0, true);
    V2_WAITCNT((NSTAGE - 2) * PPW);
    __builtin_amdgcn_s_barrier();
    __builtin_amdgcn_sched_barrier(0);
    load_frags(f0);
    compute(f1, true);
  }
  for (; i < ns; i += 2) {
    if (i + 1 < ns) { wait_stage(i + 1); load_frags(f1); }
    else V2_WAITCNT(0);
    compute(f0, ist < ns);
    if (i + 1 < ns) {
      if (i + 2 < ns) { wait_stage(i + 2); load_frags(f0); }
      else V2_WAITCNT(0);
      compute(f1, ist < ns);
    }
  }
  V2_STAMP(2);
  auto write_pass = [&](int ps, float* lds, int RS) {
    const int mt = ps >> 1, hh = ps & 1;
#pragma unroll
    for (int nt = 0; nt < TN; ++nt)
#pragma unroll
      for (int qq = 0; qq < 2; ++qq)
#pragma unroll
        for (int e = 0; e < 4; ++e) lds[(8 * qq + 4 * h + e) * RS + nt * 32 + j] = acc[mt][nt][(2 * hh + qq) * 4 + e];
  };
  gemm_epilogue_wave<EPI, TN, 3>(p, write_pass, reinterpret_cast<float*>(smv2), bm * BM + wm * 64, bn * BN + wn * TN * 32, wave, lane);
  V2_STAMP(6);
#ifdef V2_TIMING
  asm volatile("s_waitcnt vmcnt(0)" ::: "memory");
#endif
  V2_STAMP(3); V2_RSTAMP(5);
}

template <bool TAPS, int EPI, int CFG>
__global__ __launch_bounds__(CFG ? 256 : 512, CFG ? 3 : 2) void gemm_bf16x3_v2_kernel(const GemmV2P q) {
  const GemmKP& p = q.g;
  const int L = blockIdx.x, xcd = L & 7, qq = L >> 3;
  int bn, bm;
  if (p.n_fast) {
    const int cs = q.cs, cg = xcd % cs, rc = xcd / cs;
    const int bml = qq / q.nbg, bnl = qq - bml * q.nbg;
    bm = bml * (8 / cs) + rc;
    bn = cg * q.nbg + bnl;
    if (bn >= p.nblocks) return;
  } else { bn = qq / p.mt8; bm = (qq - bn * p.mt8) * 8 + xcd; }
  if (bm >= p.mtiles) return;
  gemm_v2_tile<TAPS, EPI, CFG>(q, bm, bn, threadIdx.x);
}

StreamScratch g_plane_scratch(8);

int gemm_bf16x3_v2_forward(GemmKP p, const void* wplanes, const LinearWeights& w, const GemmArgs& a, hipStream_t stream, double flops,
                           double bytes) {
  IDX_CHECK(w.K % 16 == 0 && (a.taps <= 1 || (w.K / a.taps) % 16 == 0), "v2 needs K % 16 == 0");
  const int xk = a.taps > 1 ? w.K / a.taps : w.K;
  const size_t plane = (size_t)(xk / 16) * a.M * 16 * sizeof(__bf16);
  void* scratch = nullptr;
  if (!a.x_planes && g_plane_scratch.acquire(stream, 2 * plane, &scratch)) return 1;
  const __bf16* hi = static_cast<const __bf16*>(a.x_planes ? a.x_planes : scratch);
  const __bf16* lo = hi + plane / sizeof(__bf16);
  if (!a.x_planes) {
    static const int cat_split = prof_register("split_planes_kernel");
    ProfScope prof(cat_split, stream, 0.0, 8.0 * a.M * (double)xk);
    hipLaunchKernelGGL(split_planes_kernel, dim3(cdiv(a.M, 64), cdiv(xk, 64)), dim3(256), 0, stream, a.x, a.ldx, a.M, xk, const_cast<__bf16*>(hi), const_cast<__bf16*>(lo));
    IDX_LAUNCH_CHECK();
  }
  GemmV2P q;
  q.g = p;
  if (a.y_planes) {
    const int n_out = (a.act == ACT_SWIGLU || a.act == ACT_GATE) ? w.N / 2 : w.N;
    IDX_CHECK(n_out % 16 == 0 && (a.ldy & 3) == 0, "output planes need N_out % 16 == 0");
    q.g.y_hi = static_cast<__bf16*>(a.y_planes);
    q.g.y_lo = q.g.y_hi + plane_elems(a.M, n_out);
  }
  if (a.rope) {
    IDX_CHECK(a.rope_T > 0 && a.rope_cols % 64 == 0 && a.act == ACT_NONE && (a.ldy & 3) == 0, "fused rotary arguments");
    q.g.rope = a.rope; q.g.rope_T = a.rope_T; q.g.rope_cols = a.rope_cols;
  }
  const int cfg = 1;
  const int BMh = cfg ? 128 : 256, BNh = cfg ? 128 : 256;
  q.g.mtiles = cdiv(a.M, BMh);
  q.g.mt8 = cdiv(q.g.mtiles, 8);
  q.g.nblocks = cdiv(w.N, BNh);
  q.a_hi = hi; q.a_lo = lo; q.a_rows = a.M;
  q.npad = cdiv(w.N, 256) * 256;
  q.b_hi = static_cast<const __bf16*>(wplanes);
  q.b_lo = q.b_hi + (size_t)(w.K / 16) * q.npad * 16;
  q.nstages = w.K / 16;
#ifdef V2_TIMING
  q.stamps = g_v2_stamps;
#endif
  const size_t b_plane = (size_t)(w.K / 16) * q.npad * 32;
  IDX_CHECK(2 * plane < (1ull << 31) && 2 * b_plane < (1ull << 31), "operand planes beyond the 2 GiB a buffer offset addresses");
  q.a_plane = (int)plane; q.a_bytes = (int)(2 * plane);
  q.b_plane = (int)b_plane; q.b_bytes = (int)(2 * b_plane);
  q.cs = 1;
  static const double cs_bytes = [] { const char* e = getenv("IDXTTS_GEMM_CS_BYTES"); return e ? atof(e) : 3.2e6; }();
  if (!q.g.n_fast && (double)w.N * w.K * 4.0 <= 8.0 * cs_bytes && a.M > w.N) q.g.n_fast = 1;
  if (q.g.n_fast) {
    while (q.cs < 8 && (double)w.N * w.K * 4.0 / q.cs > cs_bytes && q.g.nblocks >= 2 * q.cs) q.cs *= 2;
  }
  q.nbg = cdiv(q.g.nblocks, q.cs);
  const int64_t grid = q.g.n_fast ? (int64_t)8 * q.nbg * cdiv(q.g.mtiles, 8 / q.cs) : (int64_t)8 * q.g.nblocks * q.g.mt8;
  IDX_CHECK(grid < (1ll << 31), "grid size");
  static const int cat = prof_register("gemm_bf16x3_v2_kernel");
  ProfScope prof(cat, stream, flops, bytes);
  const int lds = cfg ? 3 * (4 * 128 * 32) : 4 * (4 * 256 * 32);
  const bool paired = a.act == ACT_SWIGLU || a.act == ACT_GATE;
  IDX_CHECK(!(a.rope && (a.res || paired)), "the rotary epilogue takes no residual and no paired activation");
  IDX_CHECK(!a.row_len || a.seq_len >= 16, "row masks need seq_len >= 16");
  const int epi = a.rope ? EPI_ROPE : paired ? EPI_PAIRED : a.act != ACT_NONE ? EPI_ACT : EPI_PLAIN;
  typedef void (*KernelFn)(const GemmV2P);
#define V2_ROW(T, C) gemm_bf16x3_v2_kernel<T, EPI_PLAIN, C>, gemm_bf16x3_v2_kernel<T, EPI_ROPE, C>, gemm_bf16x3_v2_kernel<T, EPI_PAIRED, C>, gemm_bf16x3_v2_kernel<T, EPI_ACT, C>
  static const KernelFn kernels[2][2][4] = {{{V2_ROW(false, 0)}, {V2_ROW(true, 0)}}, {{V2_ROW(false, 1)}, {V2_ROW(true, 1)}}};
  static DynLdsLimit lds_limit[2];
  IDX_HIP(lds_limit[0].set(4 * (4 * 256 * 32), V2_ROW(false, 0), V2_ROW(true, 0)));
  IDX_HIP(lds_limit[1].set(3 * (4 * 128 * 32), V2_ROW(false, 1), V2_ROW(true, 1)));
#undef V2_ROW
  hipLaunchKernelGGL(kernels[cfg][a.taps > 1 ? 1 : 0][epi], dim3((unsigned)grid), dim3(cfg ? 256 : 512), lds, stream, q);
  IDX_LAUNCH_CHECK();
  return 0;
}

}
```

index-tts_amd/csrc/s2mel.h:

```cpp
#pragma once
#include "../../include/idxtts.h"
#include "attention.h"
#include "ctx.h"
#include "decode.h"
#include "gemm.h"
#include "norm.h"
#include "prof.h"
#include "s2mel_ops.h"

namespace idxtts {

struct DiTBlock {
  LinearWeights wqkv, wo, w13, w2, skip_a, skip_b;
  const float *attn_g = nullptr, *ffn_g = nullptr;
};

struct WNLayer {
  LinearWeights in_gate;
  LinearWeights res, skip;
  bool has_res = true;
};

struct CfmBuffers;
struct CondBuffers { float *a, *b, *s, *stats; int *idx_code, *idx_row, *idx_interp, *tlen; size_t bytes; };

struct S2MelModel : ModelBase {
  idxtts_s2mel_config cfg;
  std::vector<DiTBlock> blocks;
  const float* final_g = nullptr;
  LinearWeights mod_all, cond_proj, merge, temb0, temb2, t2emb0, t2emb2, skiplin_a, skiplin_b, conv1, res_proj, final_lin,
      final_mod, conv2, wn_cond;
  std::vector<WNLayer> wn;
  LinearWeights lr_in, lr_out;
  std::vector<LinearWeights> lr_conv;
  std::vector<const float*> lr_gn_g, lr_gn_b;
  LinearWeights gl[3];
  const float* vq_table = nullptr;
  const float* rope = nullptr; int rope_len = 0;
  int ffn = 0;

  explicit S2MelModel(const idxtts_s2mel_config& c);
  bool accepts(const std::string& name) const override;
  int finalize(std::map<std::string, HostTensor>& t, DeviceArena& arena) override;

  size_t cfm_workspace_bytes(int B, int T, int n_steps) const;
  int cfm(const float* mu, const int* x_lens_host, const float* prompt, const int* prompt_lens_host, int Tp_max, const float* style,
          const float* z, const float* t_emb, const float* dt_host, int n_steps, float cfg_rate, float* out, int B, int T,
          void* ws, size_t ws_bytes, hipStream_t st);
  size_t cfm_rows_workspace_bytes(int B, int T, int Tp_max, int n_steps) const;
  int cfm_rows(const float* gen_cond, const int* target_lens_host, int Tg_max, const float* const* prompt_cond_host,
               const float* const* ref_mel_host, const int* prompt_lens_host, const float* style, const float* z, const float* t_emb,
               const float* dt_host, int n_steps, float cfg_rate, float* out, int B, int T, void* ws, size_t ws_bytes, hipStream_t st);
  int estimator(const float* x, const float* prompt, const int* prompt_lens_host, int Tp_max, const int* x_lens_host, const float* t_emb,
                const float* style, const float* mu, float* out_tm, int B, int T, void* ws, size_t ws_bytes, hipStream_t st);
  size_t cond_workspace_bytes(int B, int M, int Tg) const;
  int cfm_solve(CfmBuffers& w, const float* mu, const int* x_lens_host, const float* prompt, const int* prompt_lens_host, int Tp_max,
                const float* style, const float* z, const float* t_emb, const float* dt_host, int n_steps, float cfg_rate, int B, int T,
                hipStream_t st);
  int regulate_rows(const float* s_rows, const CondBuffers& w, int B, int M, int Tg, float* cond_out, hipStream_t st);
  int regulate(const float* S, const int* in_lens_host, const int* target_lens_host, int B, int M, int Tg, float* cond_out, void* ws,
               size_t ws_bytes, hipStream_t st);
  int prepare_cond(const float* latent, const long long* codes, const int* code_lens_host, const int* target_lens_host, int B, int M,
                   int Tg, float* cond_out, void* ws, size_t ws_bytes, hipStream_t st);
};

void set_s2mel_overlap(int on);
int get_s2mel_overlap();
int s2mel_release_stream(hipStream_t st);

}
```

index-tts_amd/csrc/s2mel.hip:

```cpp
#include <cmath>
#include <cstring>

#include <map>
#include <mutex>
#include <utility>

#include "model_util.h"
#include "s2mel.h"

namespace idxtts {

S2MelModel::S2MelModel(const idxtts_s2mel_config& c) : cfg(c) {}

bool S2MelModel::accepts(const std::string& name) const {
  static const char* prefixes[] = {"cfm.estimator.", "length_regulator.", "gpt_layer.", "semantic_codec.", "rope_cache"};
  for (const char* p : prefixes)
    if (name.rfind(p, 0) == 0) return true;
  return false;
}

namespace {

std::vector<float> col_slice(const std::vector<float>& w, int N, int K, int k0, int k1) {
  std::vector<float> o((size_t)N * (k1 - k0));
  for (int n = 0; n < N; ++n) std::memcpy(&o[(size_t)n * (k1 - k0)], &w[(size_t)n * K + k0], (k1 - k0) * sizeof(float));
  return o;
}

std::vector<float> pair_pack(const float* a, const float* b, int H, int K) {
  std::vector<float> o((size_t)2 * H * K);
  for (int blk = 0; blk < H / 32; ++blk) {
    std::memcpy(&o[(size_t)(blk * 64) * K], a + (size_t)blk * 32 * K, (size_t)32 * K * sizeof(float));
    std::memcpy(&o[(size_t)(blk * 64 + 32) * K], b + (size_t)blk * 32 * K, (size_t)32 * K * sizeof(float));
  }
  return o;
}

std::vector<float> conv_to_rows(const std::vector<float>& w, int Cout, int Cin, int k) {
  std::vector<float> o((size_t)Cout * Cin * k);
  for (int co = 0; co < Cout; ++co)
    for (int ci = 0; ci < Cin; ++ci)
      for (int kk = 0; kk < k; ++kk) o[((size_t)co * k + kk) * Cin + ci] = w[((size_t)co * Cin + ci) * k + kk];
  return o;
}

}

int S2MelModel::finalize(std::map<std::string, HostTensor>& t, DeviceArena& arena) {
  const int D = cfg.hidden_dim, C = cfg.in_channels, Wh = cfg.wn_hidden, depth = cfg.depth;
  IDX_CHECK(D == cfg.num_heads * 64, "head_dim must be 64");
  IDX_CHECK(Wh == D, "the reference's FinalLayer requires wavenet.hidden_dim == DiT.hidden_dim");
  IDX_CHECK((D & 31) == 0 && (Wh & 31) == 0 && (cfg.lr_channels & 31) == 0, "channel counts must be multiples of 32");
  {
    const int nh = (int)(2 * (4 * D) / 3);
    ffn = (nh % 256 == 0) ? nh : nh + 256 - (nh % 256);
  }
  const std::string e = "cfm.estimator";
  blocks.resize(depth);
  std::vector<float> mod_w, mod_b;
  auto append_mod = [&](const std::string& name) -> int {
    HostTensor *w = nullptr, *b = nullptr;
    if (need(t, name + ".project_layer.weight", {2 * D, D}, &w) || need(t, name + ".project_layer.bias", {2 * D}, &b)) return 1;
    mod_w.insert(mod_w.end(), w->data.begin(), w->data.end());
    mod_b.insert(mod_b.end(), b->data.begin(), b->data.end());
    return 0;
  };
  for (int i = 0; i < depth; ++i) {
    DiTBlock& B = blocks[i];
    const std::string p = e + ".transformer.layers." + std::to_string(i);
    if (linear_from(t, arena, p + ".attention.wqkv", 3 * D, D, false, WP16_ALWAYS, &B.wqkv)) return 1;
    if (linear_from(t, arena, p + ".attention.wo", D, D, false, WP16_ALWAYS, &B.wo)) return 1;
    HostTensor *w1 = nullptr, *w3 = nullptr;
    if (need(t, p + ".feed_forward.w1.weight", {ffn, D}, &w1) || need(t, p + ".feed_forward.w3.weight", {ffn, D}, &w3)) return 1;
    if (make_linear(arena, pair_pack(w1->data.data(), w3->data.data(), ffn, D).data(), nullptr, 2 * ffn, D, {WP16_ALWAYS}, &B.w13)) return 1;
    if (linear_from(t, arena, p + ".feed_forward.w2", D, ffn, false, WP16_ALWAYS, &B.w2)) return 1;
    HostTensor *g = nullptr;
    if (need(t, p + ".attention_norm.norm.weight", {D}, &g) || up(arena, g->data, &B.attn_g)) return 1;
    if (need(t, p + ".ffn_norm.norm.weight", {D}, &g) || up(arena, g->data, &B.ffn_g)) return 1;
    if (append_mod(p + ".attention_norm") || append_mod(p + ".ffn_norm")) return 1;
    if (i > depth / 2) {
      HostTensor *sw = nullptr, *sb = nullptr;
      if (need(t, p + ".skip_in_linear.weight", {D, 2 * D}, &sw) || need(t, p + ".skip_in_linear.bias", {D}, &sb)) return 1;
      if (make_linear(arena, col_slice(sw->data, D, 2 * D, 0, D).data(), sb->data.data(), D, D, {WP16_ALWAYS}, &B.skip_a)) return 1;
      if (make_linear(arena, col_slice(sw->data, D, 2 * D, D, 2 * D).data(), nullptr, D, D, {WP16_ALWAYS}, &B.skip_b)) return 1;
    }
  }
  {
    HostTensor* g = nullptr;
    if (need(t, e + ".transformer.norm.norm.weight", {D}, &g) || up(arena, g->data, &final_g)) return 1;
    if (append_mod(e + ".transformer.norm")) return 1;
    if (make_linear(arena, mod_w.data(), mod_b.data(), (2 * depth + 1) * 2 * D, D, {WP16_ALWAYS}, &mod_all)) return 1;
  }
  const int Win = 2 * C + D + cfg.style_dim;
  if (linear_from(t, arena, e + ".cond_projection", D, cfg.content_dim, true, WP16_ALWAYS, &cond_proj)) return 1;
  if (linear_from(t, arena, e + ".cond_x_merge_linear", D, Win, true, WP16_ALWAYS, &merge)) return 1;
  if (linear_from(t, arena, e + ".t_embedder.mlp.0", D, 256, true, WP16_ALWAYS, &temb0) || linear_from(t, arena, e + ".t_embedder.mlp.2", D, D, true, WP16_ALWAYS, &temb2)) return 1;
  if (linear_from(t, arena, e + ".t_embedder2.mlp.0", Wh, 256, true, WP16_ALWAYS, &t2emb0) || linear_from(t, arena, e + ".t_embedder2.mlp.2", Wh, Wh, true, WP16_ALWAYS, &t2emb2)) return 1;
  {
    HostTensor *sw = nullptr, *sb = nullptr;
    if (need(t, e + ".skip_linear.weight", {D, D + C}, &sw) || need(t, e + ".skip_linear.bias", {D}, &sb)) return 1;
    if (make_linear(arena, col_slice(sw->data, D, D + C, 0, D).data(), sb->data.data(), D, D, {WP16_ALWAYS}, &skiplin_a)) return 1;
    if (make_linear(arena, col_slice(sw->data, D, D + C, D, D + C).data(), nullptr, D, C, {WP16_ALWAYS}, &skiplin_b)) return 1;
  }
  if (linear_from(t, arena, e + ".conv1", Wh, D, true, WP16_ALWAYS, &conv1)) return 1;
  if (linear_from(t, arena, e + ".res_projection", Wh, D, true, WP16_ALWAYS, &res_proj)) return 1;
  if (linear_from(t, arena, e + ".final_layer.linear", Wh, Wh, true, WP16_ALWAYS, &final_lin)) return 1;
  if (linear_from(t, arena, e + ".final_layer.adaLN_modulation.1", 2 * Wh, Wh, true, WP16_ALWAYS, &final_mod)) return 1;
  {
    HostTensor *w = nullptr, *b = nullptr;
    if (need(t, e + ".conv2.weight", {C, Wh, 1}, &w) || need(t, e + ".conv2.bias", {C}, &b)) return 1;
    if (make_linear(arena, w->data.data(), b->data.data(), C, Wh, {WP16_ALWAYS}, &conv2)) return 1;
  }
  const int L = cfg.wn_layers, k = cfg.wn_kernel;
  wn.resize(L);
  {
    HostTensor *cw = nullptr, *cb = nullptr;
    if (need(t, e + ".wavenet.cond_layer.conv.conv.weight", {2 * Wh * L, Wh, 1}, &cw) ||
        need(t, e + ".wavenet.cond_layer.conv.conv.bias", {2 * Wh * L}, &cb)) return 1;
    std::vector<float> cw_perm, cb_perm;
    for (int l = 0; l < L; ++l) {
      WNLayer& W = wn[l];
      const std::string p = e + ".wavenet.in_layers." + std::to_string(l) + ".conv.conv";
      HostTensor *iw = nullptr, *ib = nullptr;
      if (need(t, p + ".weight", {2 * Wh, Wh, k}, &iw) || need(t, p + ".bias", {2 * Wh}, &ib)) return 1;
      const std::vector<float> rows = conv_to_rows(iw->data, 2 * Wh, Wh, k);
      if (make_linear(arena, pair_pack(rows.data(), rows.data() + (size_t)Wh * k * Wh, Wh, k * Wh).data(), nullptr, 2 * Wh, k * Wh, {WP16_ALWAYS}, &W.in_gate)) return 1;
      const float* cwl = cw->data.data() + (size_t)l * 2 * Wh * Wh;
      const std::vector<float> cwp = pair_pack(cwl, cwl + (size_t)Wh * Wh, Wh, Wh);
      cw_perm.insert(cw_perm.end(), cwp.begin(), cwp.end());
      std::vector<float> bsum(2 * Wh);
      for (int c = 0; c < 2 * Wh; ++c) bsum[c] = cb->data[(size_t)l * 2 * Wh + c] + ib->data[c];
      const std::vector<float> bp = pair_pack(bsum.data(), bsum.data() + Wh, Wh, 1);
      cb_perm.insert(cb_perm.end(), bp.begin(), bp.end());
      const std::string r = e + ".wavenet.res_skip_layers." + std::to_string(l) + ".conv.conv";
      const int rc = l < L - 1 ? 2 * Wh : Wh;
      HostTensor *rw = nullptr, *rb = nullptr;
      if (need(t, r + ".weight", {rc, Wh, 1}, &rw) || need(t, r + ".bias", {rc}, &rb)) return 1;
      if (l < L - 1) {
        std::vector<float> w_res(rw->data.begin(), rw->data.begin() + (size_t)Wh * Wh), b_res(rb->data.begin(), rb->data.begin() + Wh);
        std::vector<float> w_skip(rw->data.begin() + (size_t)Wh * Wh, rw->data.end()), b_skip(rb->data.begin() + Wh, rb->data.end());
        if (make_linear(arena, w_res.data(), b_res.data(), Wh, Wh, {WP16_ALWAYS}, &W.res) || make_linear(arena, w_skip.data(), b_skip.data(), Wh, Wh, {WP16_ALWAYS}, &W.skip)) return 1;
      } else {
        W.has_res = false;
        if (make_linear(arena, rw->data.data(), rb->data.data(), Wh, Wh, {WP16_ALWAYS}, &W.skip)) return 1;
      }
    }
    if (make_linear(arena, cw_perm.data(), cb_perm.data(), 2 * Wh * L, Wh, {WP16_ALWAYS}, &wn_cond)) return 1;
  }
  const int LC = cfg.lr_channels;
  if (linear_from(t, arena, "length_regulator.content_in_proj", LC, cfg.lr_in_channels, true, WP16_ALWAYS, &lr_in)) return 1;
  lr_conv.resize(cfg.lr_num_convs);
  lr_gn_g.resize(cfg.lr_num_convs);
  lr_gn_b.resize(cfg.lr_num_convs);
  for (int n = 0; n < cfg.lr_num_convs; ++n) {
    HostTensor *w = nullptr, *b = nullptr, *g = nullptr, *bb = nullptr;
    const std::string p = "length_regulator.model." + std::to_string(3 * n);
    if (need(t, p + ".weight", {LC, LC, 3}, &w) || need(t, p + ".bias", {LC}, &b)) return 1;
    if (make_linear(arena, conv_to_rows(w->data, LC, LC, 3).data(), b->data.data(), LC, 3 * LC, {WP16_ALWAYS}, &lr_conv[n])) return 1;
    const std::string q = "length_regulator.model." + std::to_string(3 * n + 1);
    if (need(t, q + ".weight", {LC}, &g) || need(t, q + ".bias", {LC}, &bb)) return 1;
    if (up(arena, g->data, &lr_gn_g[n]) || up(arena, bb->data, &lr_gn_b[n])) return 1;
  }
  {
    HostTensor *w = nullptr, *b = nullptr;
    const std::string p = "length_regulator.model." + std::to_string(3 * cfg.lr_num_convs);
    if (need(t, p + ".weight", {LC, LC, 1}, &w) || need(t, p + ".bias", {LC}, &b)) return 1;
    if (make_linear(arena, w->data.data(), b->data.data(), LC, LC, {WP16_ALWAYS}, &lr_out)) return 1;
  }
  {
    const int dims[4] = {cfg.gpt_dim, cfg.gpt_layer_dims[0], cfg.gpt_layer_dims[1], cfg.gpt_layer_dims[2]};
    for (int n = 0; n < 3; ++n)
      if (linear_from(t, arena, "gpt_layer." + std::to_string(n), dims[n + 1], dims[n], true, WP16_ALWAYS, &gl[n])) return 1;
    IDX_CHECK(dims[3] == cfg.codec_hidden && cfg.codec_hidden == cfg.lr_in_channels, "gpt_layer / codec / length-regulator widths");
  }
  {
    HostTensor *cb = nullptr, *ow = nullptr, *ob = nullptr;
    const std::string q = "semantic_codec.quantizer.quantizers.0";
    if (need(t, q + ".codebook.weight", {cfg.codebook_size, cfg.codebook_dim}, &cb) ||
        need(t, q + ".out_project.weight", {cfg.codec_hidden, cfg.codebook_dim, 1}, &ow) ||
        need(t, q + ".out_project.bias", {cfg.codec_hidden}, &ob)) return 1;
    std::vector<float> table((size_t)cfg.codebook_size * cfg.codec_hidden);
    for (int v = 0; v < cfg.codebook_size; ++v)
      for (int h = 0; h < cfg.codec_hidden; ++h) {
        float acc = 0.0f;
        for (int c = 0; c < cfg.codebook_dim; ++c) acc = std::fmaf(cb->data[(size_t)v * cfg.codebook_dim + c], ow->data[(size_t)h * cfg.codebook_dim + c], acc);
        table[(size_t)v * cfg.codec_hidden + h] = acc + ob->data[h];
      }
    if (up(arena, table, &vq_table)) return 1;
  }
  {
    auto it = t.find("rope_cache");
    if (it == t.end()) IDX_FAIL("missing tensor 'rope_cache' ([T][32][2] cos/sin table, precompute_freqs_cis)");
    IDX_CHECK(it->second.shape.size() == 3 && it->second.shape[1] == 32 && it->second.shape[2] == 2, "rope_cache must be [T][32][2]");
    rope_len = (int)it->second.shape[0];
    if (up(arena, it->second.data, &rope)) return 1;
  }
  return 0;
}

struct CfmBuffers {
  float *x_in, *ha, *hb, *hmid, *hn, *qkv, *att, *ff, *xres, *wn_x, *wn_acts, *wn_out, *vout, *condp, *xstate;
  void *hn_p, *att_p, *ff_p, *acts_p;
  void *h_p, *wnx_p, *xres_p;
  std::vector<void*> skips_p;
  std::vector<float*> skips;
  float *t1, *t1s, *mods, *fmod, *t2, *wnb, *tmp_steps;
  int *lens2, *plen, *lens2t;
  int tail_t0 = 0;
  size_t bytes;
};

static CfmBuffers carve_cfm(const S2MelModel& m, void* ws, int B, int T, int n_steps) {
  const auto& c = m.cfg;
  const int D = c.hidden_dim, C = c.in_channels, Wh = c.wn_hidden;
  const size_t M2 = (size_t)2 * B * T;
  const int Win = 2 * C + D + c.style_dim;
  CfmBuffers b;
  Carver k(ws);
  b.x_in = k.take<float>(M2 * Win);
  b.ha = k.take<float>(M2 * D);
  b.hb = k.take<float>(M2 * D);
  b.hmid = k.take<float>(M2 * D);
  b.hn = k.take<float>(M2 * D);
  b.qkv = k.take<float>(M2 * 3 * D);
  b.att = k.take<float>(M2 * D);
  b.ff = k.take<float>(M2 * m.ffn);
  b.xres = k.take<float>(M2 * D);
  b.hn_p = k.take<float>(M2 * std::max(D, Wh));
  b.att_p = k.take<float>(M2 * D);
  b.ff_p = k.take<float>(M2 * m.ffn);
  b.acts_p = k.take<float>(M2 * Wh);
  b.h_p = k.take<float>(M2 * D);
  b.wnx_p = k.take<float>(M2 * Wh);
  b.xres_p = k.take<float>(M2 * D);
  b.wn_x = k.take<float>(M2 * Wh);
  b.wn_acts = k.take<float>(M2 * Wh);
  b.wn_out = k.take<float>(M2 * Wh);
  b.vout = k.take<float>(M2 * C);
  b.condp = k.take<float>((size_t)B * T * D);
  b.xstate = k.take<float>((size_t)B * C * T);
  for (int i = 0; i < c.depth / 2; ++i) b.skips.push_back(k.take<float>(M2 * D));
  for (int i = 0; i < c.depth / 2; ++i) b.skips_p.push_back(k.take<float>(M2 * D));
  b.t1 = k.take<float>((size_t)n_steps * D);
  b.t1s = k.take<float>((size_t)n_steps * D);
  b.tmp_steps = k.take<float>((size_t)n_steps * std::max(D, Wh));
  b.mods = k.take<float>((size_t)n_steps * (2 * c.depth + 1) * 2 * D);
  b.fmod = k.take<float>((size_t)n_steps * 2 * Wh);
  b.t2 = k.take<float>((size_t)n_steps * Wh);
  b.wnb = k.take<float>((size_t)n_steps * c.wn_layers * 2 * Wh);
  b.lens2 = k.take<int>(2 * B);
  b.plen = k.take<int>(B);
  b.lens2t = k.take<int>(2 * B);
  b.bytes = (k.off + 255) & ~(size_t)255;
  return b;
}

size_t S2MelModel::cfm_workspace_bytes(int B, int T, int n_steps) const { return carve_cfm(*this, nullptr, B, T, n_steps).bytes; }

static CfmBuffers half_view(const S2MelModel& m, const CfmBuffers& w, int h, int B, int T) {
  const auto& c = m.cfg;
  const int D = c.hidden_dim, C = c.in_channels, Wh = c.wn_hidden, Win = 2 * C + D + c.style_dim;
  const size_t R = (size_t)h * B * T;
  CfmBuffers v = w;
  auto sh = [&](float* p, int cols) { return p + R * cols; };
  auto shp = [&](void* p, int cols) -> void* { return static_cast<float*>(p) + R * cols; };
  v.x_in = sh(w.x_in, Win); v.ha = sh(w.ha, D); v.hb = sh(w.hb, D); v.hmid = sh(w.hmid, D); v.hn = sh(w.hn, D); v.qkv = sh(w.qkv, 3 * D);
  v.att = sh(w.att, D); v.ff = sh(w.ff, m.ffn); v.xres = sh(w.xres, D); v.wn_x = sh(w.wn_x, Wh); v.wn_acts = sh(w.wn_acts, Wh);
  v.wn_out = sh(w.wn_out, Wh); v.vout = sh(w.vout, C);
  v.hn_p = shp(w.hn_p, std::max(D, Wh)); v.att_p = shp(w.att_p, D); v.ff_p = shp(w.ff_p, m.ffn); v.acts_p = shp(w.acts_p, Wh);
  v.h_p = shp(w.h_p, D); v.wnx_p = shp(w.wnx_p, Wh); v.xres_p = shp(w.xres_p, D);
  for (size_t i = 0; i < w.skips.size(); ++i) { v.skips[i] = sh(w.skips[i], D); v.skips_p[i] = shp(w.skips_p[i], D); }
  v.lens2 = w.lens2 + h * B; v.lens2t = w.lens2t + h * B;
  return v;
}

static int gemm(const LinearWeights& w, const float* x, int ldx, float* y, int ldy, int M, hipStream_t st, int act = ACT_NONE,
                const float* res = nullptr, int ldr = 0, const void* xp = nullptr, void* yp = nullptr) {
  GemmArgs a;
  a.x = xp ? nullptr : x; a.ldx = ldx; a.y = y; a.ldy = ldy; a.M = M; a.act = act; a.res = res; a.ldr = ldr;
  a.x_planes = xp; a.y_planes = yp;
  return gemm_forward(w, a, st);
}

static int dit_eval(S2MelModel& m, CfmBuffers& w, int N2, int T, int step, hipStream_t st, hipEvent_t lag_event) {
  const auto& c = m.cfg;
  const int D = c.hidden_dim, C = c.in_channels, Wh = c.wn_hidden, depth = c.depth, half = depth / 2;
  const int M = N2 * T, Win = 2 * C + D + c.style_dim;
  const float* mods = w.mods + (size_t)step * (2 * depth + 1) * 2 * D;
  bool chain = true;
  {
    GemmArgs pr;
    pr.M = M;
    const LinearWeights* used[] = {&m.blocks[0].wqkv, &m.blocks[0].wo, &m.blocks[0].w13, &m.blocks[0].w2, &m.skiplin_a, &m.final_lin,
                                   &m.wn[0].skip};
    for (const LinearWeights* lw : used) chain = chain && gemm_uses_planes(*lw, pr);
  }
  bool chain_wn = chain;
  {
    GemmArgs pr;
    pr.M = M;
    const LinearWeights* used[] = {&m.skiplin_b, &m.conv1, &m.res_proj, &m.wn[0].res};
    for (const LinearWeights* lw : used) chain_wn = chain_wn && gemm_uses_planes(*lw, pr);
    pr.taps = c.wn_kernel; pr.seq_len = T;
    chain_wn = chain_wn && gemm_uses_planes(m.wn[0].in_gate, pr);
  }
  void* const hn_p = chain ? w.hn_p : nullptr;
  const int t0 = w.tail_t0, Tt = T - t0, Mt = N2 * Tt;
  bool chain_t = chain, chain_wn_t = chain_wn;
  if (t0 > 0) {
    GemmArgs pr;
    pr.M = Mt;
    const LinearWeights* used[] = {&m.blocks[0].wo, &m.blocks[0].w13, &m.blocks[0].w2, &m.skiplin_a, &m.final_lin, &m.wn[0].skip};
    for (const LinearWeights* lw : used) chain_t = chain_t && gemm_uses_planes(*lw, pr);
    chain_wn_t = chain_t && chain_wn && gemm_uses_planes(m.skiplin_b, pr) && gemm_uses_planes(m.conv1, pr) && gemm_uses_planes(m.res_proj, pr) &&
                 gemm_uses_planes(m.wn[0].res, pr);
    pr.taps = c.wn_kernel; pr.seq_len = Tt;
    chain_wn_t = chain_wn_t && gemm_uses_planes(m.wn[0].in_gate, pr);
  }
  float* const hnt_f = chain_t ? nullptr : w.hn;
  void* const hnt_p = chain_t ? w.hn_p : nullptr;
  auto ada_rows = [&](const float* x, const float* g, int mod_idx, int rows, bool planes) {
    RowsNormArgs n;
    n.x_in = x; n.ld_in = D; n.y = planes ? nullptr : w.hn; n.y_planes = planes ? w.hn_p : nullptr; n.ld_y = D; n.M = rows; n.d = D;
    n.mode = NORM_ADA_RMS; n.eps = c.norm_eps; n.g1 = g;
    n.mod_a = mods + (size_t)mod_idx * 2 * D; n.mod_b = n.mod_a + D; n.ld_mod = 0; n.rows_per_batch = 0;
    return rows_norm_forward(n, st);
  };
  auto ada = [&](const float* x, const float* g, int mod_idx) { return ada_rows(x, g, mod_idx, M, chain); };
  if (lag_event && depth < 2) IDX_HIP(hipEventRecord(lag_event, st));
  bool h_compact = false;
  if (gemm(m.merge, w.x_in, Win, w.ha, D, M, st)) return 1;
  float* h = w.ha;
  int pushed = 0;
  for (int i = 0; i < depth; ++i) {
    DiTBlock& B = m.blocks[i];
    if (i > half) {
      float* skip = w.skips[--pushed];
      void* skip_p = chain ? w.skips_p[pushed] : nullptr;
      if (gemm(B.skip_a, h, D, w.hmid, D, M, st, ACT_NONE, nullptr, 0, chain ? w.h_p : nullptr)) return 1;
      float* dst = (h == w.ha) ? w.hb : w.ha;
      if (gemm(B.skip_b, skip, D, dst, D, M, st, ACT_NONE, w.hmid, D, skip_p)) return 1;
      h = dst;
    }
    if (ada(h, B.attn_g, 2 * i)) return 1;
    bool qkv_planes = false;
    {
      GemmArgs g;
      g.x = chain ? nullptr : w.hn; g.x_planes = hn_p; g.ldx = D; g.y = w.qkv; g.ldy = 3 * D; g.M = M;
      const bool fuse_rope = gemm_uses_planes(B.wqkv, g);
      qkv_planes = fuse_rope && D == 64 * c.num_heads;
      if (fuse_rope) { g.rope = m.rope; g.rope_T = T; g.rope_cols = 2 * D; }
      if (qkv_planes) { g.y = nullptr; g.y_planes = w.qkv; }
      if (gemm_forward(B.wqkv, g, st)) return 1;
      if (!fuse_rope && rotary_qk(w.qkv, M, c.num_heads, T, m.rope, st)) return 1;
    }
    AttnPlanesArgs ap;
    ap.planes = w.qkv; ap.Mrows = M; ap.ncols = 3 * D; ap.q_col = 0; ap.k_col = D; ap.v_col = 2 * D; ap.T = T; ap.q_row0 = 0; ap.Sq = T;
    ap.B = N2; ap.H = c.num_heads; ap.kend = w.lens2; ap.scale = 0.125f; ap.o = w.att; ap.o_bs = (long)T * D; ap.o_ts = D;
    AttnArgs a;
    a.q = w.qkv; a.k = w.qkv + D; a.v = w.qkv + 2 * D; a.o = w.att;
    a.q_bs = a.k_bs = a.v_bs = (long)T * 3 * D; a.o_bs = (long)T * D;
    a.q_ts = a.k_ts = a.v_ts = 3 * D; a.o_ts = D;
    a.B = N2; a.H = c.num_heads; a.Sq = T; a.Sk = T; a.causal = 0; a.kend = w.lens2; a.scale = 0.125f;
    a.split_bf16 = get_gemm_mode() == GEMM_BF16X3;
    if (i == depth - 1 && t0 > 0 && i >= half) {
      a.q = w.qkv + (size_t)t0 * 3 * D; a.Sq = Tt; a.o_bs = (long)Tt * D;
      ap.q_row0 = t0; ap.Sq = Tt; ap.o_bs = (long)Tt * D;
      if (chain_t) { a.o = nullptr; a.o_planes = w.att_p; ap.o = nullptr; ap.o_planes = w.att_p; }
      if (qkv_planes ? flash_attn_planes_forward(ap, st) : flash_attn_forward(a, st)) return 1;
      if (gather_tail_rows(w.xres, D, h, D, D, N2, T, t0, st)) return 1;
      if (gemm(B.wo, w.att, D, w.hmid, D, Mt, st, ACT_NONE, w.xres, D, chain_t ? w.att_p : nullptr)) return 1;
      if (ada_rows(w.hmid, B.ffn_g, 2 * i + 1, Mt, chain_t)) return 1;
      if (gemm(B.w13, w.hn, D, chain_t ? nullptr : w.ff, m.ffn, Mt, st, ACT_SWIGLU, nullptr, 0, hnt_p, chain_t ? w.ff_p : nullptr)) return 1;
      float* dst = (h == w.ha) ? w.hb : w.ha;
      if (gemm(B.w2, w.ff, m.ffn, dst, D, Mt, st, ACT_NONE, w.hmid, D, chain_t ? w.ff_p : nullptr, nullptr)) return 1;
      h = dst;
      h_compact = true;
      break;
    }
    if (chain) { a.o = nullptr; a.o_planes = w.att_p; ap.o = nullptr; ap.o_planes = w.att_p; }
    if (qkv_planes ? flash_attn_planes_forward(ap, st) : flash_attn_forward(a, st)) return 1;
    if (i == 0 && lag_event) IDX_HIP(hipEventRecord(lag_event, st));
    if (gemm(B.wo, w.att, D, w.hmid, D, M, st, ACT_NONE, h, D, chain ? w.att_p : nullptr)) return 1;
    if (ada(w.hmid, B.ffn_g, 2 * i + 1)) return 1;
    if (gemm(B.w13, w.hn, D, chain ? nullptr : w.ff, m.ffn, M, st, ACT_SWIGLU, nullptr, 0, hn_p, chain ? w.ff_p : nullptr)) return 1;
    float* dst = (i < half) ? w.skips[pushed] : ((h == w.ha) ? w.hb : w.ha);
    void* dst_p = !chain ? nullptr : (i < half ? w.skips_p[pushed] : (i + 1 < depth && i + 1 > half ? w.h_p : nullptr));
    if (gemm(B.w2, w.ff, m.ffn, dst, D, M, st, ACT_NONE, w.hmid, D, chain ? w.ff_p : nullptr, dst_p)) return 1;
    if (i < half) ++pushed;
    h = dst;
  }
  const float* ht = h;
  const float* xin_t = w.x_in;
  int ld_xin = Win;
  const int* lens_t = w.lens2;
  if (t0 > 0) {
    if (!h_compact) {
      float* hc = (h == w.ha) ? w.hb : w.ha;
      if (gather_tail_rows(hc, D, h, D, D, N2, T, t0, st)) return 1;
      ht = hc;
    }
    if (gather_tail_rows(w.qkv, C, w.x_in, Win, C, N2, T, t0, st)) return 1;
    xin_t = w.qkv; ld_xin = C; lens_t = w.lens2t;
  }
  {
    RowsNormArgs n;
    n.x_in = ht; n.ld_in = D; n.y = hnt_f; n.y_planes = hnt_p; n.ld_y = D; n.M = Mt; n.d = D; n.mode = NORM_ADA_RMS; n.eps = c.norm_eps; n.g1 = m.final_g;
    n.mod_a = mods + (size_t)(2 * depth) * 2 * D; n.mod_b = n.mod_a + D; n.ld_mod = 0; n.rows_per_batch = 0;
    if (rows_norm_forward(n, st)) return 1;
  }
  if (gemm(m.skiplin_a, w.hn, D, w.hmid, D, Mt, st, ACT_NONE, nullptr, 0, hnt_p)) return 1;
  if (gemm(m.skiplin_b, xin_t, ld_xin, w.xres, D, Mt, st, ACT_NONE, w.hmid, D, nullptr, chain_wn_t ? w.xres_p : nullptr)) return 1;
  if (gemm(m.conv1, w.xres, D, w.wn_x, Wh, Mt, st, ACT_NONE, nullptr, 0, chain_wn_t ? w.xres_p : nullptr, chain_wn_t ? w.wnx_p : nullptr)) return 1;
  const int L = c.wn_layers, k = c.wn_kernel;
  for (int l = 0; l < L; ++l) {
    WNLayer& W = m.wn[l];
    int dil = 1;
    for (int q = 0; q < l; ++q) dil *= c.wn_dilation_rate;
    LinearWeights in = W.in_gate;
    in.bias = w.wnb + ((size_t)step * L + l) * 2 * Wh;
    GemmArgs g;
    g.x = chain_wn_t ? nullptr : w.wn_x; g.x_planes = chain_wn_t ? w.wnx_p : nullptr; g.ldx = Wh; g.y = chain_t ? nullptr : w.wn_acts; g.y_planes = chain_t ? w.acts_p : nullptr; g.ldy = Wh; g.M = Mt; g.act = ACT_GATE;
    g.taps = k; g.seq_len = Tt; g.dil = dil; g.pad_left = (k - 1) / 2 * dil; g.pad_mode = 1; g.row_len = lens_t;
    if (gemm_forward(in, g, st)) return 1;
    if (W.has_res) {
      GemmArgs r;
      r.x = chain_t ? nullptr : w.wn_acts; r.x_planes = chain_t ? w.acts_p : nullptr; r.ldx = Wh; r.y = w.wn_x; r.y_planes = chain_wn_t ? w.wnx_p : nullptr; r.ldy = Wh; r.res = w.wn_x; r.ldr = Wh; r.M = Mt; r.seq_len = Tt; r.row_len = lens_t;
      if (gemm_forward(W.res, r, st)) return 1;
    }
    GemmArgs sk;
    sk.x = chain_t ? nullptr : w.wn_acts; sk.x_planes = chain_t ? w.acts_p : nullptr; sk.ldx = Wh; sk.y = w.wn_out; sk.ldy = Wh; sk.M = Mt;
    if (l > 0) { sk.res = w.wn_out; sk.ldr = Wh; }
    if (l == L - 1) { sk.seq_len = Tt; sk.row_len = lens_t; }
    if (gemm_forward(W.skip, sk, st)) return 1;
  }
  if (gemm(m.res_proj, w.xres, D, w.hmid, Wh, Mt, st, ACT_NONE, w.wn_out, Wh, chain_wn_t ? w.xres_p : nullptr)) return 1;
  {
    RowsNormArgs n;
    n.x_in = w.hmid; n.ld_in = Wh; n.y = hnt_f; n.y_planes = hnt_p; n.ld_y = Wh; n.M = Mt; n.d = Wh; n.mode = NORM_MOD_LN; n.eps = 1e-6f;
    n.mod_a = w.fmod + (size_t)step * 2 * Wh; n.mod_b = n.mod_a + Wh; n.ld_mod = 0; n.rows_per_batch = 0;
    if (rows_norm_forward(n, st)) return 1;
  }
  if (gemm(m.final_lin, w.hn, Wh, w.att, Wh, Mt, st, ACT_NONE, nullptr, 0, hnt_p)) return 1;
  return gemm(m.conv2, w.att, Wh, w.vout, C, Mt, st);
}

struct HalfStreams { hipStream_t side = nullptr; hipEvent_t fork = nullptr, lag = nullptr, join = nullptr; };
static std::map<std::pair<int, hipStream_t>, HalfStreams> g_half_streams;
static std::mutex g_half_mu;
static int g_s2mel_overlap = 0;
void set_s2mel_overlap(int on) { g_s2mel_overlap = on ? 1 : 0; }
int get_s2mel_overlap() { return g_s2mel_overlap; }

static int half_streams_for(hipStream_t st, HalfStreams* out) {
  int dev = 0;
  IDX_HIP(hipGetDevice(&dev));
  std::lock_guard<std::mutex> lk(g_half_mu);
  HalfStreams& hs = g_half_streams[std::make_pair(dev, st)];
  if (!hs.side) {
    int prio = 0;
    if (st) IDX_HIP(hipStreamGetPriority(st, &prio));
    IDX_HIP(hipStreamCreateWithPriority(&hs.side, hipStreamNonBlocking, prio));
    IDX_HIP(hipEventCreateWithFlags(&hs.fork, hipEventDisableTiming));
    IDX_HIP(hipEventCreateWithFlags(&hs.lag, hipEventDisableTiming));
    IDX_HIP(hipEventCreateWithFlags(&hs.join, hipEventDisableTiming));
  }
  *out = hs;
  return 0;
}

int s2mel_release_stream(hipStream_t st) {
  int dev = 0;
  IDX_HIP(hipGetDevice(&dev));
  HalfStreams hs;
  {
    std::lock_guard<std::mutex> lk(g_half_mu);
    auto it = g_half_streams.find(std::make_pair(dev, st));
    if (it == g_half_streams.end()) return 0;
    hs = it->second;
    g_half_streams.erase(it);
  }
  if (hs.side) { (void)hipStreamSynchronize(hs.side); (void)hipStreamDestroy(hs.side); }
  if (hs.fork) (void)hipEventDestroy(hs.fork);
  if (hs.lag) (void)hipEventDestroy(hs.lag);
  if (hs.join) (void)hipEventDestroy(hs.join);
  return 0;
}

static bool halves_on_two_streams(hipStream_t st) {
  hipStreamCaptureStatus cap = hipStreamCaptureStatusNone;
  (void)hipStreamIsCapturing(st, &cap);
  return g_s2mel_overlap && !prof_enabled() && cap == hipStreamCaptureStatusNone;
}

static int dit_eval_halves(S2MelModel& m, CfmBuffers& w, int B, int T, int step, bool two_streams, hipStream_t st) {
  if (!two_streams) return dit_eval(m, w, 2 * B, T, step, st, nullptr);
  CfmBuffers v0 = half_view(m, w, 0, B, T);
  CfmBuffers v1 = half_view(m, w, 1, B, T);
  HalfStreams hs;
  if (half_streams_for(st, &hs)) return 1;
  IDX_HIP(hipEventRecord(hs.fork, st));
  IDX_HIP(hipStreamWaitEvent(hs.side, hs.fork, 0));
  if (dit_eval(m, v0, B, T, step, st, hs.lag)) return 1;
  IDX_HIP(hipStreamWaitEvent(hs.side, hs.lag, 0));
  if (dit_eval(m, v1, B, T, step, hs.side, nullptr)) return 1;
  IDX_HIP(hipEventRecord(hs.join, hs.side));
  IDX_HIP(hipStreamWaitEvent(st, hs.join, 0));
  return 0;
}

int S2MelModel::cfm(const float* mu, const int* x_lens_host, const float* prompt, const int* prompt_lens_host, int Tp_max,
                    const float* style, const float* z, const float* t_emb, const float* dt_host, int n_steps, float cfg_rate,
                    float* out, int B, int T, void* ws, size_t ws_bytes, hipStream_t st) {
  IDX_CHECK(mu && x_lens_host && prompt && prompt_lens_host && style && z && t_emb && dt_host && out, "null pointer");
  IDX_CHECK(B > 0 && T > 0 && n_steps > 0 && Tp_max > 0, "shape");
  IDX_CHECK(cfg_rate > 0.0f, "the stacked-CFG path needs inference_cfg_rate > 0 (reference default 0.7)");
  IDX_CHECK(T <= rope_len, "sequence longer than the rope cache");
  IDX_CHECK(ws && ws_bytes >= cfm_workspace_bytes(B, T, n_steps), "workspace too small");
  CfmBuffers w = carve_cfm(*this, ws, B, T, n_steps);
  if (cfm_solve(w, mu, x_lens_host, prompt, prompt_lens_host, Tp_max, style, z, t_emb, dt_host, n_steps, cfg_rate, B, T, st)) return 1;
  IDX_HIP(hipMemcpyAsync(out, w.xstate, (size_t)B * cfg.in_channels * T * sizeof(float), hipMemcpyDeviceToDevice, st));
  return 0;
}

int S2MelModel::cfm_solve(CfmBuffers& w, const float* mu, const int* x_lens_host, const float* prompt, const int* prompt_lens_host,
                          int Tp_max, const float* style, const float* z, const float* t_emb, const float* dt_host, int n_steps,
                          float cfg_rate, int B, int T, hipStream_t st) {
  const int D = cfg.hidden_dim, C = cfg.in_channels, Wh = cfg.wn_hidden, depth = cfg.depth, L = cfg.wn_layers;
  std::vector<int> lens2(2 * B), plen(B);
  for (int b = 0; b < B; ++b) {
    IDX_CHECK(x_lens_host[b] > 0 && x_lens_host[b] <= T && prompt_lens_host[b] >= 0 && prompt_lens_host[b] <= std::min(Tp_max, x_lens_host[b]), "lengths");
    lens2[b] = lens2[B + b] = x_lens_host[b];
    plen[b] = prompt_lens_host[b];
  }
  {
    int halo = 0, dil = 1, pmin = plen[0];
    for (int l = 0; l < L; ++l) { halo += (cfg.wn_kernel - 1) / 2 * dil; dil *= cfg.wn_dilation_rate; }
    for (int b = 0; b < B; ++b) pmin = std::min(pmin, plen[b]);
    w.tail_t0 = pmin - halo >= 64 ? pmin - halo : 0;
  }
  std::vector<int> lens2t(2 * B);
  for (int i = 0; i < 2 * B; ++i) lens2t[i] = lens2[i] - w.tail_t0;
  IDX_HIP(hipMemcpyAsync(w.lens2, lens2.data(), 2 * B * sizeof(int), hipMemcpyHostToDevice, st));
  IDX_HIP(hipMemcpyAsync(w.lens2t, lens2t.data(), 2 * B * sizeof(int), hipMemcpyHostToDevice, st));
  IDX_HIP(hipMemcpyAsync(w.plen, plen.data(), B * sizeof(int), hipMemcpyHostToDevice, st));
  IDX_HIP(hipStreamSynchronize(st));
  if (gemm(temb0, t_emb, 256, w.tmp_steps, D, n_steps, st, ACT_SILU) || gemm(temb2, w.tmp_steps, D, w.t1, D, n_steps, st)) return 1;
  if (gemm(mod_all, w.t1, D, w.mods, (2 * depth + 1) * 2 * D, n_steps, st)) return 1;
  if (silu_rows(w.t1s, w.t1, (size_t)n_steps * D, st) || gemm(final_mod, w.t1s, Wh, w.fmod, 2 * Wh, n_steps, st)) return 1;
  if (gemm(t2emb0, t_emb, 256, w.tmp_steps, Wh, n_steps, st, ACT_SILU) || gemm(t2emb2, w.tmp_steps, Wh, w.t2, Wh, n_steps, st)) return 1;
  if (gemm(wn_cond, w.t2, Wh, w.wnb, L * 2 * Wh, n_steps, st)) return 1;
  if (gemm(cond_proj, mu, cfg.content_dim, w.condp, D, B * T, st)) return 1;
  if (cfm_init_state(w.xstate, z, w.plen, B, C, T, st)) return 1;
  const bool two_streams = halves_on_two_streams(st);
  for (int s = 0; s < n_steps; ++s) {
    CfmPackArgs pk;
    pk.x_in = w.x_in; pk.ld = 2 * C + D + cfg.style_dim; pk.x = w.xstate; pk.prompt = prompt; pk.prompt_len = w.plen;
    pk.cond = w.condp; pk.cond_null = cond_proj.bias; pk.style = style;
    pk.B = B; pk.T = T; pk.C = C; pk.D = D; pk.S = cfg.style_dim; pk.Tp_max = Tp_max;
    pk.x_only = s > 0;
    if (cfm_pack(pk, st)) return 1;
    if (dit_eval_halves(*this, w, B, T, s, two_streams, st)) return 1;
    CfmEulerArgs eu;
    eu.x = w.xstate; eu.v = w.vout; eu.v_null = two_streams ? w.vout + (size_t)B * T * C : nullptr; eu.ldv = C; eu.prompt_len = w.plen; eu.B = B; eu.T = T; eu.C = C; eu.dt = dt_host[s]; eu.cfg_rate = cfg_rate;
    eu.v_t0 = w.tail_t0; eu.v_T = T - w.tail_t0;
    if (cfm_euler(eu, st)) return 1;
  }
  return 0;
}

struct CfmRowsBuffers { float *mu, *prompt; const float **pcond, **ref_mel; int* gen_len; size_t bytes; };

static CfmRowsBuffers carve_cfm_rows(const S2MelModel& m, void* ws, size_t base, int B, int T, int Tp_max) {
  const auto& c = m.cfg;
  CfmRowsBuffers b;
  Carver k(ws ? static_cast<char*>(ws) + base : nullptr);
  b.mu = k.take<float>((size_t)B * T * c.content_dim);
  b.prompt = k.take<float>((size_t)B * c.in_channels * Tp_max);
  b.pcond = k.take<const float*>(B);
  b.ref_mel = k.take<const float*>(B);
  b.gen_len = k.take<int>(B);
  b.bytes = base + ((k.off + 255) & ~(size_t)255);
  return b;
}

size_t S2MelModel::cfm_rows_workspace_bytes(int B, int T, int Tp_max, int n_steps) const {
  return carve_cfm_rows(*this, nullptr, cfm_workspace_bytes(B, T, n_steps), B, T, Tp_max).bytes;
}

int S2MelModel::cfm_rows(const float* gen_cond, const int* target_lens_host, int Tg_max, const float* const* prompt_cond_host,
                         const float* const* ref_mel_host, const int* prompt_lens_host, const float* style, const float* z,
                         const float* t_emb, const float* dt_host, int n_steps, float cfg_rate, float* out, int B, int T, void* ws,
                         size_t ws_bytes, hipStream_t st) {
  IDX_CHECK(gen_cond && target_lens_host && prompt_cond_host && ref_mel_host && prompt_lens_host && style && z && t_emb && dt_host && out,
            "null pointer");
  IDX_CHECK(B > 0 && T > 0 && Tg_max > 0 && n_steps > 0, "shape");
  IDX_CHECK(cfg_rate > 0.0f, "the stacked-CFG path needs inference_cfg_rate > 0 (reference default 0.7)");
  IDX_CHECK(T <= rope_len, "sequence longer than the rope cache");
  IDX_CHECK(cfg.content_dim % 4 == 0 && ((uintptr_t)gen_cond & 15) == 0, "gen_cond must be 16-byte aligned (content_dim % 4 == 0)");
  std::vector<int> xl(B), tg(B);
  int Tp_max = 0, T_need = 0;
  for (int b = 0; b < B; ++b) {
    const int Tp = prompt_lens_host[b], Tg = target_lens_host[b];
    IDX_CHECK(Tp > 0 && Tg > 0 && Tg <= Tg_max, "prompt_lens / target_lens out of range");
    IDX_CHECK(prompt_cond_host[b] && ref_mel_host[b], "null prompt table entry");
    IDX_CHECK(((uintptr_t)prompt_cond_host[b] & 15) == 0, "prompt_condition rows must be 16-byte aligned");
    xl[b] = Tp + Tg;
    tg[b] = Tg;
    Tp_max = std::max(Tp_max, Tp);
    T_need = std::max(T_need, Tp + Tg);
  }
  IDX_CHECK(T == T_need, "T must be max_b(prompt_lens[b] + target_lens[b])");
  IDX_CHECK(ws && ws_bytes >= cfm_rows_workspace_bytes(B, T, Tp_max, n_steps), "workspace too small");
  CfmBuffers w = carve_cfm(*this, ws, B, T, n_steps);
  CfmRowsBuffers r = carve_cfm_rows(*this, ws, w.bytes, B, T, Tp_max);
  IDX_HIP(hipMemcpyAsync(r.pcond, prompt_cond_host, B * sizeof(float*), hipMemcpyHostToDevice, st));
  IDX_HIP(hipMemcpyAsync(r.ref_mel, ref_mel_host, B * sizeof(float*), hipMemcpyHostToDevice, st));
  IDX_HIP(hipMemcpyAsync(r.gen_len, tg.data(), B * sizeof(int), hipMemcpyHostToDevice, st));
  IDX_HIP(hipMemcpyAsync(w.plen, prompt_lens_host, B * sizeof(int), hipMemcpyHostToDevice, st));
  CfmRowsPackArgs pk;
  pk.mu = r.mu; pk.prompt = r.prompt; pk.pcond = r.pcond; pk.ref_mel = r.ref_mel; pk.gen = gen_cond; pk.prompt_len = w.plen;
  pk.gen_len = r.gen_len; pk.B = B; pk.T = T; pk.Dc = cfg.content_dim; pk.C = cfg.in_channels; pk.Tp_max = Tp_max; pk.Tg_max = Tg_max;
  if (cfm_rows_pack(pk, st)) return 1;
  if (cfm_solve(w, r.mu, xl.data(), r.prompt, prompt_lens_host, Tp_max, style, z, t_emb, dt_host, n_steps, cfg_rate, B, T, st)) return 1;
  return cfm_rows_emit(out, w.xstate, w.plen, r.gen_len, B, cfg.in_channels, T, Tg_max, st);
}

int S2MelModel::estimator(const float* x, const float* prompt, const int* prompt_lens_host, int Tp_max, const int* x_lens_host,
                          const float* t_emb, const float* style, const float* mu, float* out_tm, int B, int T, void* ws, size_t ws_bytes,
                          hipStream_t st) {
  IDX_CHECK(x && prompt && prompt_lens_host && x_lens_host && t_emb && style && mu && out_tm, "null pointer");
  IDX_CHECK(B > 0 && T > 0 && Tp_max > 0 && T <= rope_len, "shape");
  IDX_CHECK(ws && ws_bytes >= cfm_workspace_bytes(B, T, 1), "workspace too small");
  const int D = cfg.hidden_dim, C = cfg.in_channels, Wh = cfg.wn_hidden, depth = cfg.depth, L = cfg.wn_layers;
  CfmBuffers w = carve_cfm(*this, ws, B, T, 1);
  std::vector<int> lens2(2 * B), plen(B);
  for (int b = 0; b < B; ++b) {
    IDX_CHECK(x_lens_host[b] > 0 && x_lens_host[b] <= T && prompt_lens_host[b] >= 0 && prompt_lens_host[b] <= std::min(Tp_max, T), "lengths");
    lens2[b] = lens2[B + b] = x_lens_host[b];
    plen[b] = prompt_lens_host[b];
  }
  IDX_HIP(hipMemcpyAsync(w.lens2, lens2.data(), 2 * B * sizeof(int), hipMemcpyHostToDevice, st));
  IDX_HIP(hipMemcpyAsync(w.plen, plen.data(), B * sizeof(int), hipMemcpyHostToDevice, st));
  IDX_HIP(hipStreamSynchronize(st));
  if (gemm(temb0, t_emb, 256, w.tmp_steps, D, 1, st, ACT_SILU) || gemm(temb2, w.tmp_steps, D, w.t1, D, 1, st)) return 1;
  if (gemm(mod_all, w.t1, D, w.mods, (2 * depth + 1) * 2 * D, 1, st)) return 1;
  if (silu_rows(w.t1s, w.t1, (size_t)D, st) || gemm(final_mod, w.t1s, Wh, w.fmod, 2 * Wh, 1, st)) return 1;
  if (gemm(t2emb0, t_emb, 256, w.tmp_steps, Wh, 1, st, ACT_SILU) || gemm(t2emb2, w.tmp_steps, Wh, w.t2, Wh, 1, st)) return 1;
  if (gemm(wn_cond, w.t2, Wh, w.wnb, L * 2 * Wh, 1, st)) return 1;
  if (gemm(cond_proj, mu, cfg.content_dim, w.condp, D, B * T, st)) return 1;
  IDX_HIP(hipMemcpyAsync(w.xstate, x, (size_t)B * C * T * sizeof(float), hipMemcpyDeviceToDevice, st));
  CfmPackArgs pk;
  pk.x_in = w.x_in; pk.ld = 2 * C + D + cfg.style_dim; pk.x = w.xstate; pk.prompt = prompt; pk.prompt_len = w.plen;
  pk.cond = w.condp; pk.cond_null = cond_proj.bias; pk.style = style;
  pk.B = B; pk.T = T; pk.C = C; pk.D = D; pk.S = cfg.style_dim; pk.Tp_max = Tp_max;
  if (cfm_pack(pk, st)) return 1;
  {
    CfmBuffers v0 = half_view(*this, w, 0, B, T);
    if (dit_eval(*this, v0, B, T, 0, st, nullptr)) return 1;
  }
  IDX_HIP(hipMemcpyAsync(out_tm, w.vout, (size_t)B * T * C * sizeof(float), hipMemcpyDeviceToDevice, st));
  return 0;
}


static CondBuffers carve_cond(const S2MelModel& m, void* ws, int B, int M, int Tg) {
  const auto& c = m.cfg;
  CondBuffers b;
  Carver k(ws);
  const size_t rows = (size_t)B * std::max(M, Tg);
  const int wide = std::max(std::max(c.codec_hidden, c.lr_channels), std::max(c.gpt_layer_dims[0], c.gpt_layer_dims[1]));
  b.a = k.take<float>(rows * wide);
  b.b = k.take<float>(rows * wide);
  b.s = k.take<float>(rows * wide);
  b.stats = k.take<float>(2 * B);
  b.idx_code = k.take<int>((size_t)B * M);
  b.idx_row = k.take<int>((size_t)B * M);
  b.idx_interp = k.take<int>((size_t)B * Tg);
  b.tlen = k.take<int>(B);
  b.bytes = (k.off + 255) & ~(size_t)255;
  return b;
}

size_t S2MelModel::cond_workspace_bytes(int B, int M, int Tg) const { return carve_cond(*this, nullptr, B, M, Tg).bytes; }

int S2MelModel::prepare_cond(const float* latent, const long long* codes, const int* code_lens_host, const int* target_lens_host,
                             int B, int M, int Tg, float* cond_out, void* ws, size_t ws_bytes, hipStream_t st) {
  IDX_CHECK(latent && codes && code_lens_host && target_lens_host && cond_out, "null pointer");
  IDX_CHECK(B > 0 && M > 0 && Tg > 0, "shape");
  IDX_CHECK(ws && ws_bytes >= cond_workspace_bytes(B, M, Tg), "workspace too small");
  const int Hc = cfg.codec_hidden;
  CondBuffers w = carve_cond(*this, ws, B, M, Tg);
  std::vector<long long> hc((size_t)B * M);
  IDX_HIP(hipMemcpyAsync(hc.data(), codes, hc.size() * sizeof(long long), hipMemcpyDeviceToHost, st));
  IDX_HIP(hipStreamSynchronize(st));
  std::vector<int> ic((size_t)B * M), ir((size_t)B * M), ii((size_t)B * Tg, -1), tl(B);
  for (int b = 0; b < B; ++b) {
    const int mb = code_lens_host[b], tb = target_lens_host[b];
    IDX_CHECK(mb > 0 && mb <= M && tb > 0 && tb <= Tg, "code_lens / target_lens out of range");
    tl[b] = tb;
    for (int i = 0; i < M; ++i) {
      const long long cde = hc[(size_t)b * M + i];
      IDX_CHECK(i >= mb || (cde >= 0 && cde < cfg.codebook_size), "semantic code out of the codebook");
      ic[(size_t)b * M + i] = i < mb ? (int)cde : -1;
      ir[(size_t)b * M + i] = i < mb ? b * M + i : -1;
    }
    const float scale = (float)mb / (float)tb;
    for (int j = 0; j < tb; ++j) ii[(size_t)b * Tg + j] = b * M + std::min((int)std::floor((float)j * scale), mb - 1);
  }
  IDX_HIP(hipMemcpyAsync(w.idx_code, ic.data(), ic.size() * sizeof(int), hipMemcpyHostToDevice, st));
  IDX_HIP(hipMemcpyAsync(w.idx_row, ir.data(), ir.size() * sizeof(int), hipMemcpyHostToDevice, st));
  IDX_HIP(hipMemcpyAsync(w.idx_interp, ii.data(), ii.size() * sizeof(int), hipMemcpyHostToDevice, st));
  IDX_HIP(hipMemcpyAsync(w.tlen, tl.data(), B * sizeof(int), hipMemcpyHostToDevice, st));
  IDX_HIP(hipStreamSynchronize(st));
  const int rowsM = B * M;
  if (gemm(gl[0], latent, cfg.gpt_dim, w.a, gl[0].N, rowsM, st) || gemm(gl[1], w.a, gl[0].N, w.b, gl[1].N, rowsM, st) ||
      gemm(gl[2], w.b, gl[1].N, w.a, Hc, rowsM, st)) return 1;
  GatherArgs ga;
  ga.out = w.s; ga.ld_out = Hc; ga.d = Hc;
  ga.table[0] = vq_table; ga.idx[0] = w.idx_code;
  ga.table[1] = w.a; ga.idx[1] = w.idx_row;
  if (gather_sum_rows(ga, rowsM, st)) return 1;
  return regulate_rows(w.s, w, B, M, Tg, cond_out, st);
}

int S2MelModel::regulate_rows(const float* s_rows, const CondBuffers& w, int B, int M, int Tg, float* cond_out, hipStream_t st) {
  const int Hc = cfg.codec_hidden, LC = cfg.lr_channels;
  const int rowsM = B * M, rowsT = B * Tg;
  if (gemm(lr_in, s_rows, Hc, w.a, LC, rowsM, st)) return 1;
  GatherArgs gi;
  gi.out = w.b; gi.ld_out = LC; gi.d = LC; gi.table[0] = w.a; gi.idx[0] = w.idx_interp;
  if (gather_sum_rows(gi, rowsT, st)) return 1;
  float* cur = w.b;
  float* other = w.a;
  for (int n = 0; n < cfg.lr_num_convs; ++n) {
    GemmArgs g;
    g.x = cur; g.ldx = LC; g.y = other; g.ldy = LC; g.M = rowsT; g.taps = 3; g.seq_len = Tg; g.dil = 1; g.pad_left = 1; g.pad_mode = 0;
    if (gemm_forward(lr_conv[n], g, st)) return 1;
    if (groupnorm1_mish(cur, other, lr_gn_g[n], lr_gn_b[n], w.tlen, B, Tg, LC, 1e-5f, w.stats, st)) return 1;
  }
  GemmArgs o;
  o.x = cur; o.ldx = LC; o.y = cond_out; o.ldy = LC; o.M = rowsT; o.seq_len = Tg; o.row_len = w.tlen;
  return gemm_forward(lr_out, o, st);
}

int S2MelModel::regulate(const float* S, const int* in_lens_host, const int* target_lens_host, int B, int M, int Tg, float* cond_out,
                         void* ws, size_t ws_bytes, hipStream_t st) {
  IDX_CHECK(S && in_lens_host && target_lens_host && cond_out, "null pointer");
  IDX_CHECK(B > 0 && M > 0 && Tg > 0, "shape");
  IDX_CHECK(ws && ws_bytes >= cond_workspace_bytes(B, M, Tg), "workspace too small");
  CondBuffers w = carve_cond(*this, ws, B, M, Tg);
  std::vector<int> ii((size_t)B * Tg, -1), tl(B);
  for (int b = 0; b < B; ++b) {
    const int mb = in_lens_host[b], tb = target_lens_host[b];
    IDX_CHECK(mb > 0 && mb <= M && tb > 0 && tb <= Tg, "in_lens / target_lens out of range");
    tl[b] = tb;
    const float scale = (float)mb / (float)tb;
    for (int j = 0; j < tb; ++j) ii[(size_t)b * Tg + j] = b * M + std::min((int)std::floor((float)j * scale), mb - 1);
  }
  IDX_HIP(hipMemcpyAsync(w.idx_interp, ii.data(), ii.size() * sizeof(int), hipMemcpyHostToDevice, st));
  IDX_HIP(hipMemcpyAsync(w.tlen, tl.data(), B * sizeof(int), hipMemcpyHostToDevice, st));
  IDX_HIP(hipStreamSynchronize(st));
  return regulate_rows(S, w, B, M, Tg, cond_out, st);
}

}
```

index-tts_amd/indextts_amd/_lib.py:

```python
from __future__ import annotations

import ctypes
import os
from ctypes import POINTER, c_char_p, c_float, c_int, c_int64, c_size_t, c_void_p

_HERE = os.path.dirname(os.path.abspath(__file__))
LIB_PATH = os.path.join(_HERE, "libidxtts_hip.so")

SYMBOLS = [
    "idxtts_version", "idxtts_last_error", "idxtts_aa_act_fwd",
    "idxtts_conv1d_create", "idxtts_conv1d_fwd", "idxtts_conv1d_destroy",
    "idxtts_ctx_load_tensor", "idxtts_ctx_finalize", "idxtts_ctx_get_tensor", "idxtts_ctx_destroy",
    "idxtts_fp8_e4m3_decode", "idxtts_fp8_e4m3_encode",
    "idxtts_bigvgan_create", "idxtts_bigvgan_workspace_bytes", "idxtts_bigvgan_fwd", "idxtts_bigvgan_fwd_ragged",
    "idxtts_profile_enable", "idxtts_profile_num_kernels", "idxtts_profile_kernel_name", "idxtts_profile_read", "idxtts_profile_event_overhead",
    "idxtts_linear_create", "idxtts_linear_fwd", "idxtts_linear_destroy", "idxtts_release_stream", "idxtts_attention_fwd", "idxtts_attention_bf16x3_fwd", "idxtts_attention_relkey_fwd", "idxtts_layernorm_fwd",
    "idxtts_gpt_create", "idxtts_gpt_quantize_weights", "idxtts_gpt_set_kv_format", "idxtts_gpt_get_kv_format", "idxtts_gpt_workspace_bytes", "idxtts_gpt_embed", "idxtts_gpt_generate", "idxtts_gpt_generate_forced", "idxtts_gpt_generate_sampled", "idxtts_gpt_latent",
    "idxtts_gpt_beam_workspace_bytes", "idxtts_gpt_generate_beam",
    "idxtts_gpt_session_workspace_bytes", "idxtts_gpt_session_init", "idxtts_gpt_session_admit", "idxtts_gpt_session_step",
    "idxtts_gpt_session_read", "idxtts_gpt_session_release", "idxtts_gpt_session_workspace_bytes_ex", "idxtts_gpt_session_init_ex",
    "idxtts_gpt_session_admit_sampled", "idxtts_gpt_session_workspace_bytes_beam", "idxtts_gpt_session_init_beam",
    "idxtts_gpt_session_admit_beam",
    "idxtts_s2mel_create", "idxtts_s2mel_cond_workspace_bytes", "idxtts_s2mel_prepare_cond",
    "idxtts_s2mel_cfm_workspace_bytes", "idxtts_s2mel_cfm", "idxtts_set_gemm_mode", "idxtts_get_gemm_mode", "idxtts_set_decode_geometry", "idxtts_get_decode_geometry", "idxtts_set_decode_plane_rows", "idxtts_get_decode_plane_rows", "idxtts_s2mel_set_overlap", "idxtts_s2mel_get_overlap",
    "idxtts_s2mel_estimator", "idxtts_s2mel_cfm_rows_workspace_bytes", "idxtts_s2mel_cfm_rows", "idxtts_s2mel_regulate", "idxtts_cond_create", "idxtts_cond_workspace_bytes", "idxtts_cond_forward", "idxtts_emovec_merge",
    "idxtts_gpt_graph_cache_entries", "idxtts_w2vbert_create", "idxtts_w2vbert_workspace_bytes", "idxtts_w2vbert_forward",
    "idxtts_repcodec_create", "idxtts_repcodec_workspace_bytes", "idxtts_repcodec_quantize",
    "idxtts_melspec_create", "idxtts_melspec_frames", "idxtts_melspec_workspace_bytes", "idxtts_melspec_forward",
    "idxtts_campplus_create", "idxtts_campplus_workspace_bytes", "idxtts_campplus_forward",
    "idxtts_qwen_create", "idxtts_qwen_set_weight_format", "idxtts_qwen_workspace_bytes", "idxtts_qwen_generate",
    "idxtts_qwen_step_graph_launches", "idxtts_qwen_max_batch", "idxtts_qwen_batch_workspace_bytes", "idxtts_qwen_generate_batch",
    "idxtts_qwen_batch_step_graph_launches",
]


class BigVGANConfigC(ctypes.Structure):
    _fields_ = [
        ("num_mels", c_int), ("upsample_initial_channel", c_int), ("num_upsamples", c_int),
        ("upsample_rates", c_int * 8), ("upsample_kernel_sizes", c_int * 8),
        ("num_kernels", c_int), ("resblock_kernel_sizes", c_int * 4),
        ("resblock_dilations", (c_int * 3) * 4),
    ]


class GPTConfigC(ctypes.Structure):
    _fields_ = [(n, c_int) for n in ("model_dim", "heads", "layers", "number_mel_codes", "number_text_tokens",
                                     "start_mel_token", "stop_mel_token", "mel_pos_len", "text_pos_len")]


class SamplingC(ctypes.Structure):
    _fields_ = [("mode", c_int), ("temperature", c_float), ("top_k", c_int), ("top_p", c_float), ("exp_noise", c_void_p),
                ("seed", ctypes.c_ulonglong)]


class CondConfigC(ctypes.Structure):
    _fields_ = [(n, c_int) for n in ("input_size", "output_size", "linear_units", "attention_heads", "num_blocks", "cnn_kernel",
                                     "perceiver_dim", "num_latents", "perceiver_depth", "perceiver_dim_head", "perceiver_mult",
                                     "emotion", "model_dim")]


class W2VBertConfigC(ctypes.Structure):
    _fields_ = [(n, c_int) for n in ("input_dim", "hidden_size", "num_heads", "intermediate_size", "num_layers", "left_max", "right_max",
                                     "conv_kernel")] + [("layer_norm_eps", c_float)]


class RepCodecConfigC(ctypes.Structure):
    _fields_ = [(n, c_int) for n in ("hidden_size", "codebook_size", "codebook_dim", "vocos_dim", "vocos_intermediate_dim", "vocos_num_layers")]


class MelSpecConfigC(ctypes.Structure):
    _fields_ = [(n, c_int) for n in ("n_fft", "hop_size", "win_size", "num_mels")]


class CamPPlusConfigC(ctypes.Structure):
    _fields_ = [(n, c_int) for n in ("feat_dim", "embedding_size", "m_channels", "growth_rate", "bn_size", "init_channels", "num_blocks")] + [
        ("block_layers", c_int * 4), ("block_dilation", c_int * 4)]


class QwenConfigC(ctypes.Structure):
    _fields_ = ([(n, c_int) for n in ("vocab_size", "hidden_size", "intermediate_size", "num_hidden_layers", "num_attention_heads",
                                      "num_key_value_heads", "head_dim")]
                + [("rms_norm_eps", c_float), ("rope_theta", c_float), ("tie_word_embeddings", c_int), ("max_context", c_int)])


class BeamC(ctypes.Structure):
    _fields_ = [("num_beams", c_int), ("do_sample", c_int), ("temperature", c_float), ("top_k", c_int), ("top_p", c_float),
                ("length_penalty", c_float), ("early_stopping", c_int), ("exp_noise", c_void_p), ("seed", ctypes.c_ulonglong)]


class S2MelConfigC(ctypes.Structure):
    _fields_ = ([(n, c_int) for n in ("hidden_dim", "num_heads", "depth", "in_channels", "content_dim", "style_dim", "wn_hidden",
                                      "wn_layers", "wn_kernel", "wn_dilation_rate", "lr_channels", "lr_in_channels",
                                      "lr_num_convs", "gpt_dim")]
                + [("gpt_layer_dims", c_int * 3)]
                + [(n, c_int) for n in ("codebook_size", "codebook_dim", "codec_hidden")] + [("norm_eps", c_float)])


_lib = None


def load() -> ctypes.CDLL:
    global _lib
    if _lib is not None:
        return _lib
    if not os.path.exists(LIB_PATH):
        raise RuntimeError(
            f"libidxtts_hip.so not found at {LIB_PATH}: build it with "
            "`python -c 'import __graft_entry__ as g; g.build()'` (or `make -C index-tts_amd/csrc`). "
            "There is no CPU/PyTorch fallback for the HIP path.")
    lib = ctypes.CDLL(LIB_PATH)
    lib.idxtts_version.restype = c_int
    lib.idxtts_last_error.restype = c_char_p
    lib.idxtts_aa_act_fwd.argtypes = [c_void_p] * 6 + [c_int] * 4 + [c_void_p]
    lib.idxtts_conv1d_create.argtypes = [c_void_p, c_void_p, c_int, c_int, c_int, c_int, POINTER(c_void_p)]
    lib.idxtts_conv1d_fwd.argtypes = [c_void_p, c_void_p, c_void_p, c_void_p, c_int, c_int, c_int, c_int, c_int,
                                      c_float, c_int, c_void_p]
    lib.idxtts_conv1d_destroy.argtypes = [c_void_p]
    lib.idxtts_ctx_load_tensor.argtypes = [c_void_p, c_char_p, c_void_p, POINTER(c_int64), c_int]
    lib.idxtts_ctx_finalize.argtypes = [c_void_p]
    lib.idxtts_ctx_get_tensor.argtypes = [c_void_p, c_char_p, c_void_p, c_size_t]
    lib.idxtts_fp8_e4m3_decode.argtypes = [ctypes.c_ubyte]
    lib.idxtts_fp8_e4m3_decode.restype = ctypes.c_float
    lib.idxtts_fp8_e4m3_encode.argtypes = [ctypes.c_float]
    lib.idxtts_fp8_e4m3_encode.restype = ctypes.c_ubyte
    lib.idxtts_gpt_quantize_weights.argtypes = [c_void_p, c_int]
    lib.idxtts_gpt_set_kv_format.argtypes = [c_void_p, c_int]
    lib.idxtts_gpt_get_kv_format.argtypes = [c_void_p]
    lib.idxtts_ctx_destroy.argtypes = [c_void_p]
    lib.idxtts_bigvgan_create.argtypes = [POINTER(BigVGANConfigC), POINTER(c_void_p)]
    lib.idxtts_bigvgan_workspace_bytes.argtypes = [c_void_p, c_int, c_int]
    lib.idxtts_bigvgan_workspace_bytes.restype = c_size_t
    lib.idxtts_bigvgan_fwd.argtypes = [c_void_p, c_void_p, c_void_p, c_int, c_int, c_void_p, c_size_t, c_int, c_int,
                                       c_void_p, c_void_p]
    lib.idxtts_bigvgan_fwd_ragged.argtypes = [c_void_p, c_void_p, c_void_p, c_void_p, c_int, c_int, c_void_p, c_size_t, c_int, c_void_p]
    c_long = ctypes.c_long
    lib.idxtts_linear_create.argtypes = [c_void_p, c_void_p, c_int, c_int, c_int, POINTER(c_void_p)]
    lib.idxtts_linear_fwd.argtypes = [c_void_p, c_void_p, c_int, c_void_p, c_int, c_void_p, c_int, c_int, c_int, c_int, c_void_p]
    lib.idxtts_set_gemm_mode.argtypes = [c_int]
    lib.idxtts_linear_destroy.argtypes = [c_void_p]
    lib.idxtts_attention_fwd.argtypes = [c_void_p] * 4 + [c_long, c_int, c_long, c_int, c_long, c_int, c_int, c_int, c_int, c_int,
                                                          c_int, c_void_p, c_void_p, c_float, c_void_p]
    lib.idxtts_attention_bf16x3_fwd.argtypes = lib.idxtts_attention_fwd.argtypes
    lib.idxtts_attention_relkey_fwd.argtypes = [c_void_p] * 4 + [c_long, c_int, c_long, c_int, c_int, c_int, c_int, c_void_p, c_float, c_void_p, c_int, c_int,
                                                                 c_int, c_void_p]
    lib.idxtts_layernorm_fwd.argtypes = [c_void_p, c_void_p, c_void_p, c_void_p, c_int, c_int, c_float, c_void_p]
    lib.idxtts_gpt_create.argtypes = [POINTER(GPTConfigC), POINTER(c_void_p)]
    lib.idxtts_gpt_workspace_bytes.argtypes = [c_void_p, c_int, c_int, c_int]
    lib.idxtts_gpt_workspace_bytes.restype = c_size_t
    lib.idxtts_gpt_embed.argtypes = [c_void_p, c_void_p, c_int] + [c_void_p] * 7
    lib.idxtts_gpt_generate.argtypes = [c_void_p, c_void_p, c_void_p, c_int, c_int, c_int, c_float, c_void_p, POINTER(c_int),
                                        c_void_p, c_void_p, c_size_t, c_int, c_void_p]
    lib.idxtts_gpt_generate_forced.argtypes = [c_void_p, c_void_p, c_void_p, c_int, c_int, c_int, c_float, c_void_p, c_void_p, POINTER(c_int),
                                               c_void_p, c_void_p, c_size_t, c_void_p]
    lib.idxtts_gpt_generate_sampled.argtypes = [c_void_p, c_void_p, c_void_p, c_int, c_int, c_int, c_float, POINTER(SamplingC), c_void_p,
                                                POINTER(c_int), c_void_p, c_void_p, c_size_t, c_int, c_void_p]
    lib.idxtts_gpt_beam_workspace_bytes.argtypes = [c_void_p, c_int, c_int, c_int, c_int]
    lib.idxtts_gpt_beam_workspace_bytes.restype = c_size_t
    lib.idxtts_gpt_generate_beam.argtypes = [c_void_p, c_void_p, c_void_p, c_int, c_int, c_int, c_float, POINTER(BeamC), c_void_p,
                                             POINTER(c_int), c_void_p, c_size_t, c_int, c_void_p]
    lib.idxtts_gpt_session_workspace_bytes.argtypes = [c_void_p, c_int, c_int, c_int]
    lib.idxtts_gpt_session_workspace_bytes.restype = c_size_t
    lib.idxtts_gpt_session_init.argtypes = [c_void_p, c_int, c_int, c_int, c_float, c_void_p, c_size_t, c_void_p]
    lib.idxtts_gpt_session_admit.argtypes = [c_void_p, c_int, c_void_p, c_int, c_void_p, c_void_p, c_void_p, c_void_p, c_void_p]
    lib.idxtts_gpt_session_step.argtypes = [c_void_p, c_int, c_int, c_void_p, POINTER(c_int), c_void_p, c_void_p]
    lib.idxtts_gpt_session_read.argtypes = [c_void_p, c_int, c_void_p, POINTER(c_int), c_void_p, c_void_p]
    lib.idxtts_gpt_session_release.argtypes = [c_void_p, c_void_p]
    lib.idxtts_gpt_session_workspace_bytes_ex.argtypes = [c_void_p, c_int, c_int, c_int, c_int]
    lib.idxtts_gpt_session_workspace_bytes_ex.restype = c_size_t
    lib.idxtts_gpt_session_init_ex.argtypes = [c_void_p, c_int, c_int, c_int, c_float, c_int, c_void_p, c_size_t, c_void_p]
    lib.idxtts_gpt_session_admit_sampled.argtypes = [c_void_p, c_int, c_void_p, c_int, c_void_p, c_void_p, c_void_p, c_void_p, c_void_p,
                                                     c_void_p]
    lib.idxtts_gpt_session_workspace_bytes_beam.argtypes = [c_void_p, c_int, c_int, c_int, c_int]
    lib.idxtts_gpt_session_workspace_bytes_beam.restype = c_size_t
    lib.idxtts_gpt_session_init_beam.argtypes = [c_void_p, c_int, c_int, c_int, c_int, c_float, c_void_p, c_size_t, c_void_p]
    lib.idxtts_gpt_session_admit_beam.argtypes = [c_void_p, c_int, c_void_p, c_int, c_void_p, c_void_p, c_void_p, c_void_p, c_void_p,
                                                  c_void_p]
    lib.idxtts_gpt_latent.argtypes = [c_void_p, c_void_p, c_void_p, c_int, c_int, c_int, c_int, c_void_p, c_void_p, c_size_t, c_void_p]
    lib.idxtts_s2mel_create.argtypes = [POINTER(S2MelConfigC), POINTER(c_void_p)]
    lib.idxtts_s2mel_cond_workspace_bytes.argtypes = [c_void_p, c_int, c_int, c_int]
    lib.idxtts_s2mel_cond_workspace_bytes.restype = c_size_t
    lib.idxtts_s2mel_prepare_cond.argtypes = [c_void_p, c_void_p, c_void_p, c_void_p, c_void_p, c_int, c_int, c_int, c_void_p,
                                              c_void_p, c_size_t, c_void_p]
    lib.idxtts_s2mel_cfm_workspace_bytes.argtypes = [c_void_p, c_int, c_int, c_int]
    lib.idxtts_s2mel_cfm_workspace_bytes.restype = c_size_t
    lib.idxtts_s2mel_cfm.argtypes = [c_void_p, c_void_p, c_void_p, c_void_p, c_void_p, c_int, c_void_p, c_void_p, c_void_p, c_void_p,
                                     c_int, c_float, c_void_p, c_int, c_int, c_void_p, c_size_t, c_void_p]
    lib.idxtts_s2mel_cfm_rows_workspace_bytes.argtypes = [c_void_p, c_int, c_int, c_int, c_int]
    lib.idxtts_s2mel_cfm_rows_workspace_bytes.restype = c_size_t
    lib.idxtts_s2mel_cfm_rows.argtypes = [c_void_p, c_void_p, c_void_p, c_int, c_void_p, c_void_p, c_void_p, c_void_p, c_void_p, c_void_p,
                                          c_void_p, c_int, c_float, c_void_p, c_int, c_int, c_void_p, c_size_t, c_void_p]
    lib.idxtts_s2mel_regulate.argtypes = [c_void_p, c_void_p, c_void_p, c_void_p, c_int, c_int, c_int, c_void_p, c_void_p, c_size_t, c_void_p]
    lib.idxtts_s2mel_estimator.argtypes = [c_void_p, c_void_p, c_void_p, c_void_p, c_int, c_void_p, c_void_p, c_void_p, c_void_p, c_void_p,
                                           c_int, c_int, c_void_p, c_size_t, c_void_p]
    lib.idxtts_cond_create.argtypes = [POINTER(CondConfigC), POINTER(c_void_p)]
    lib.idxtts_cond_workspace_bytes.argtypes = [c_void_p, c_int, c_int]
    lib.idxtts_cond_workspace_bytes.restype = c_size_t
    lib.idxtts_cond_forward.argtypes = [c_void_p, c_void_p, c_void_p, c_int, c_int, c_void_p, c_void_p, c_size_t, c_void_p]
    lib.idxtts_emovec_merge.argtypes = [c_void_p, c_void_p, c_void_p, c_float, c_size_t, c_void_p]
    lib.idxtts_campplus_create.argtypes = [POINTER(CamPPlusConfigC), POINTER(c_void_p)]
    lib.idxtts_campplus_workspace_bytes.argtypes = [c_void_p, c_int]
    lib.idxtts_campplus_workspace_bytes.restype = c_size_t
    lib.idxtts_campplus_forward.argtypes = [c_void_p, c_void_p, c_int, c_int, c_void_p, c_void_p, c_size_t, c_void_p]
    lib.idxtts_melspec_create.argtypes = [POINTER(MelSpecConfigC), POINTER(c_void_p)]
    lib.idxtts_melspec_frames.argtypes = [c_void_p, c_int]
    lib.idxtts_melspec_workspace_bytes.argtypes = [c_void_p, c_int, c_int]
    lib.idxtts_melspec_workspace_bytes.restype = c_size_t
    lib.idxtts_melspec_forward.argtypes = [c_void_p, c_void_p, c_int, c_int, c_void_p, c_void_p, c_size_t, c_void_p]
    lib.idxtts_repcodec_create.argtypes = [POINTER(RepCodecConfigC), POINTER(c_void_p)]
    lib.idxtts_repcodec_workspace_bytes.argtypes = [c_void_p, c_int, c_int]
    lib.idxtts_repcodec_workspace_bytes.restype = c_size_t
    lib.idxtts_repcodec_quantize.argtypes = [c_void_p, c_void_p, c_int, c_int, c_void_p, c_void_p, c_void_p, c_size_t, c_void_p]
    lib.idxtts_gpt_graph_cache_entries.argtypes = [c_void_p]
    lib.idxtts_w2vbert_create.argtypes = [POINTER(W2VBertConfigC), POINTER(c_void_p)]
    lib.idxtts_w2vbert_workspace_bytes.argtypes = [c_void_p, c_int, c_int]
    lib.idxtts_w2vbert_workspace_bytes.restype = c_size_t
    lib.idxtts_w2vbert_forward.argtypes = [c_void_p, c_void_p, c_void_p, c_int, c_int, c_void_p, c_void_p, c_size_t, c_void_p]
    lib.idxtts_qwen_create.argtypes = [POINTER(QwenConfigC), POINTER(c_void_p)]
    lib.idxtts_qwen_set_weight_format.argtypes = [c_void_p, c_int]
    lib.idxtts_qwen_workspace_bytes.argtypes = [c_void_p, c_int, c_int, c_int, c_int]
    lib.idxtts_qwen_workspace_bytes.restype = c_size_t
    lib.idxtts_qwen_generate.argtypes = [c_void_p, c_void_p, c_int, c_int, c_void_p, c_int, c_void_p, c_void_p, POINTER(c_int), c_void_p,
                                         c_void_p, c_int, c_void_p, c_size_t, c_int, c_void_p]
    lib.idxtts_qwen_step_graph_launches.argtypes = [c_void_p]
    lib.idxtts_qwen_max_batch.argtypes = [c_void_p]
    lib.idxtts_qwen_batch_workspace_bytes.argtypes = [c_void_p, c_int, c_void_p, c_void_p, c_int, c_int]
    lib.idxtts_qwen_batch_workspace_bytes.restype = c_size_t
    lib.idxtts_qwen_generate_batch.argtypes = [c_void_p, c_int, c_void_p, c_void_p, c_void_p, c_void_p, c_int, c_void_p, c_void_p, c_void_p,
                                               c_void_p, c_void_p, c_int, c_void_p, c_size_t, c_int, c_void_p]
    lib.idxtts_qwen_batch_step_graph_launches.argtypes = [c_void_p]
    lib.idxtts_profile_enable.argtypes = [c_int]
    lib.idxtts_profile_kernel_name.argtypes = [c_int]
    lib.idxtts_profile_kernel_name.restype = c_char_p
    lib.idxtts_profile_read.argtypes = [c_int, POINTER(ctypes.c_double), POINTER(ctypes.c_double),
                                        POINTER(ctypes.c_double), POINTER(ctypes.c_long)]
    for name in SYMBOLS:
        getattr(lib, name)
    _lib = lib
    return lib


def check(rc: int) -> None:
    if rc != 0:
        msg = load().idxtts_last_error()
        raise RuntimeError("libidxtts_hip: " + (msg.decode("utf-8", "replace") if msg else f"error {rc}"))


def ptr(t) -> c_void_p:
    if t is None:
        return c_void_p(0)
    return c_void_p(t.data_ptr())


def current_stream() -> c_void_p:
    import torch
    return c_void_p(torch.cuda.current_stream().cuda_stream)


def load_state_dict(ctx: c_void_p, state_dict, before_finalize=None) -> None:
    import numpy as np
    import torch
    lib = load()
    for name, value in state_dict.items():
        if isinstance(value, torch.Tensor):
            arr = value.detach().to(dtype=torch.float32).contiguous()
            shape = tuple(arr.shape)
            dptr = c_void_p(arr.data_ptr())
        else:
            arr = np.ascontiguousarray(value, dtype=np.float32)
            shape = arr.shape
            dptr = c_void_p(arr.ctypes.data)
        cshape = (c_int64 * max(1, len(shape)))(*shape)
        check(lib.idxtts_ctx_load_tensor(ctx, name.encode(), dptr, cshape, len(shape)))
    if before_finalize is not None:
        before_finalize(ctx)
    check(lib.idxtts_ctx_finalize(ctx))


def get_tensor(ctx: c_void_p, name: str, shape):
    import numpy as np
    out = np.empty(shape, dtype=np.float32)
    check(load().idxtts_ctx_get_tensor(ctx, name.encode(), c_void_p(out.ctypes.data), out.size))
    return out


def profile_enable(on: bool) -> None:
    check(load().idxtts_profile_enable(int(on)))


def profile_event_overhead(launches: int = 200) -> float:
    out = ctypes.c_double()
    lib = load()
    lib.idxtts_profile_event_overhead.argtypes = [c_void_p, c_int, POINTER(ctypes.c_double)]
    check(lib.idxtts_profile_event_overhead(current_stream(), int(launches), ctypes.byref(out)))
    return out.value


def profile_read() -> dict:
    lib = load()
    out = {}
    for i in range(lib.idxtts_profile_num_kernels()):
        ms, fl, by, n = ctypes.c_double(), ctypes.c_double(), ctypes.c_double(), ctypes.c_long()
        check(lib.idxtts_profile_read(i, ctypes.byref(ms), ctypes.byref(fl), ctypes.byref(by), ctypes.byref(n)))
        if n.value:
            out[lib.idxtts_profile_kernel_name(i).decode()] = {
                "ms": ms.value, "flops": fl.value, "bytes": by.value, "launches": n.value}
    return out


GEMM_F32, GEMM_BF16X3 = 0, 1
SESSION_SAMPLED = 1


class StreamWorkspaces:

    def __init__(self, max_entries: int = 8):
        import collections
        import threading
        self.max_entries = max_entries
        self._ws = collections.OrderedDict()
        self._lock = threading.Lock()

    def get(self, need: int, device):
        import torch
        if need <= 0:
            raise RuntimeError("workspace query returned 0")
        device = torch.device(device)
        key = (device.index, int(torch.cuda.current_stream(device).cuda_stream))
        with self._lock:
            ws = self._ws.pop(key, None)
            if ws is None or ws.numel() < need:
                ws = None
                ws = torch.empty(need, dtype=torch.uint8, device=device)
            self._ws[key] = ws
            while len(self._ws) > self.max_entries:
                self._ws.popitem(last=False)
        return ws


def set_gemm_mode(mode: int) -> None:
    check(load().idxtts_set_gemm_mode(int(mode)))


def get_gemm_mode() -> int:
    return int(load().idxtts_get_gemm_mode())


def set_decode_geometry(narrow: bool) -> None:
    check(load().idxtts_set_decode_geometry(int(bool(narrow))))


def get_decode_geometry() -> bool:
    return bool(load().idxtts_get_decode_geometry())


def release_stream(stream) -> None:
    check(load().idxtts_release_stream(c_void_p(int(stream.cuda_stream))))


def set_decode_plane_rows(min_rows: int) -> None:
    check(load().idxtts_set_decode_plane_rows(int(min_rows)))


def get_decode_plane_rows() -> int:
    return int(load().idxtts_get_decode_plane_rows())


def set_s2mel_overlap(on: bool) -> None:
    check(load().idxtts_s2mel_set_overlap(int(bool(on))))


def get_s2mel_overlap() -> bool:
    return bool(load().idxtts_s2mel_get_overlap())
```

Measured before the change: 183.6.

## Fuse s2mel skip-in, WN res/skip and step-invariant merge GEMMs in split-bf16 kernel

Extends the split-bf16 LDS-DMA GEMM with two variants: one reads its K dimension from two separate operand plane buffers, and one routes the two column halves of its output to separate destinations with separate residuals. These variants merge the two DiT skip_in GEMMs into a single launch and the WaveNet res and skip GEMMs into a single launch. The condition part of the cond_x merge linear, which does not change across Euler steps, is computed once per call, and each step then adds it as a residual to a smaller x-only GEMM. This reduces kernel launches and redundant arithmetic in the CFM loop, at the cost of extra weight copies, a new base buffer and more kernel template instances. Everything is on by default and controlled by a bitmask.

```diff
diff --git a/include/idxtts.h b/include/idxtts.h
--- a/include/idxtts.h
+++ b/include/idxtts.h
@@ -69,6 +69,9 @@
 int idxtts_get_decode_plane_rows(void);
 int idxtts_s2mel_set_overlap(int on);
 int idxtts_s2mel_get_overlap(void);
+int idxtts_s2mel_set_fused(int mask);
+int idxtts_s2mel_get_fused(void);
+long long idxtts_s2mel_fused_launches(int form);
 int idxtts_linear_destroy(idxtts_linear* lin);
 int idxtts_release_stream(void* stream);
 int idxtts_attention_fwd(const float* q, const float* k, const float* v, float* o, long q_batch_stride, int q_token_stride,
diff --git a/index-tts_amd/csrc/capi.hip b/index-tts_amd/csrc/capi.hip
--- a/index-tts_amd/csrc/capi.hip
+++ b/index-tts_amd/csrc/capi.hip
@@ -792,4 +792,13 @@
 
 int idxtts_s2mel_get_overlap(void) { return get_s2mel_overlap(); }
 
-}
+int idxtts_s2mel_set_fused(int mask) {
+  set_s2mel_fused(mask);
+  return 0;
+}
+
+int idxtts_s2mel_get_fused(void) { return get_s2mel_fused(); }
+
+long long idxtts_s2mel_fused_launches(int form) { return s2mel_fused_launches(form); }
+
+}
diff --git a/index-tts_amd/csrc/gemm.h b/index-tts_amd/csrc/gemm.h
--- a/index-tts_amd/csrc/gemm.h
+++ b/index-tts_amd/csrc/gemm.h
@@ -22,6 +22,12 @@
   float* y = nullptr; int ldy = 0;
   const void* x_planes = nullptr;
   void* y_planes = nullptr;
+  const void* x2_planes = nullptr; int k2_chunk = 0;
+  int n_split = 0;
+  float* y2 = nullptr; int ldy2 = 0;
+  const float* res2 = nullptr; int ldr2 = 0;
+  void* y2_planes = nullptr;
+  bool mask_lo = true, mask_hi = true;
   const float* rope = nullptr; int rope_T = 0, rope_cols = 0;
   const float* res = nullptr; int ldr = 0;
   int M = 0;
diff --git a/index-tts_amd/csrc/gemm.hip b/index-tts_amd/csrc/gemm.hip
--- a/index-tts_amd/csrc/gemm.hip
+++ b/index-tts_amd/csrc/gemm.hip
@@ -257,7 +257,7 @@
 int gemm_tn_forward(const LinearWeights& w, const GemmArgs& a, hipStream_t stream) {
   IDX_CHECK(w.wp && a.x && a.y, "null pointer");
   if (a.M == 0) return 0;
-  IDX_CHECK(!a.y_planes && !a.rope, "the fp32 GEMM takes and produces fp32 rows only (no fused rotary)");
+  IDX_CHECK(!a.y_planes && !a.rope && !a.x2_planes && !a.n_split, "the fp32 GEMM takes and produces fp32 rows only (no fused rotary, one input, one output)");
   GemmKP p;
   double flops, bytes;
   if (gemm_prepare(w, a, &p, &flops, &bytes)) return 1;
diff --git a/index-tts_amd/csrc/gemm_bf16x3.hip b/index-tts_amd/csrc/gemm_bf16x3.hip
--- a/index-tts_amd/csrc/gemm_bf16x3.hip
+++ b/index-tts_amd/csrc/gemm_bf16x3.hip
@@ -322,7 +322,7 @@
 int gemm_bf16x3_forward(const LinearWeights& w, const GemmArgs& a, hipStream_t stream) {
   IDX_CHECK(w.wp16 && (a.x || a.x_planes) && (a.y || a.y_planes), "null pointer (split-bf16 weights not packed?)");
   if (a.M == 0) return 0;
-  if (a.x_planes || a.y_planes || !a.x || !a.y || a.rope) IDX_CHECK(gemm_bf16x3_uses_v2(w, a), "operand planes are only understood by the LDS-DMA kernel (shape not eligible)");
+  if (a.x_planes || a.y_planes || !a.x || !a.y || a.rope || a.x2_planes || a.n_split) IDX_CHECK(gemm_bf16x3_uses_v2(w, a), "operand planes are only understood by the LDS-DMA kernel (shape not eligible)");
   IDX_CHECK(a.ksplit <= 1, "split-K is a feature of the exact-fp32 kernel");
   GemmKP p;
   double flops, bytes;
diff --git a/index-tts_amd/csrc/gemm_bf16x3_v2.hip b/index-tts_amd/csrc/gemm_bf16x3_v2.hip
--- a/index-tts_amd/csrc/gemm_bf16x3_v2.hip
+++ b/index-tts_amd/csrc/gemm_bf16x3_v2.hip
@@ -61,6 +61,9 @@
   int a_bytes, b_bytes;
   int a_plane, b_plane;
   int cs, nbg;
+  const __bf16* a2_hi; int k2_chunk, a2_bytes, a2_plane;
+  int n_split, ldy2, ldr2, mask_lo, mask_hi;
+  float* y2; const float* res2; __bf16* y2_hi; __bf16* y2_lo;
 #ifdef V2_TIMING
   unsigned long long* stamps;
 #endif
@@ -70,7 +73,11 @@
 
 #define V2_WAITCNT(vm) __builtin_amdgcn_s_waitcnt(((vm) & 15) | (((vm) >> 4) << 14) | 0x70)
 
-template <bool TAPS, int EPI, int CFG>
+enum { V2_PLAIN = 0, V2_K2 = 1, V2_NSPLIT = 2 };
+template <bool ON> struct V2K2State { __amdgpu_buffer_rsrc_t second, cur; int lo_plane; };
+template <> struct V2K2State<false> {};
+
+template <bool TAPS, int EPI, int CFG, int VAR = V2_PLAIN>
 __device__ __forceinline__ void gemm_v2_tile(const GemmV2P& q, const int bm, const int bn, const int tid) {
   constexpr int NSTAGE = CFG ? 3 : 4;
   constexpr int WMW = CFG ? 2 : 4, WNW = 2, TN = CFG ? 2 : 4;
@@ -106,6 +113,11 @@
     const bool ok = a_m < p.M && t >= 0 && t < seq_n;
     return ok ? (seq_base + t) * 32 + dunit * 16 : (int)0x80000000;
   };
+  V2K2State<VAR == V2_K2> k2;
+  if constexpr (VAR == V2_K2) {
+    k2.second = __builtin_amdgcn_make_buffer_rsrc(const_cast<__bf16*>(q.a2_hi), 0, q.a2_bytes, 0x00020000);
+    k2.cur = rA; k2.lo_plane = q.a_plane;
+  }
   V2_STAMP(0); V2_RSTAMP(4);
   const int ns = q.nstages;
   const int sA = q.a_rows * 32, sB = q.npad * 32;
@@ -115,6 +127,10 @@
   char* const lds_w = smv2 + wave * 1024;
   auto issue_piece = [&](int pi) {
     auto dst = (__attribute__((address_space(3))) void*)(lds_w + wslot * STAGE_BYTES + pi * PLANE);
+    if constexpr (VAR == V2_K2) {
+      if (pi == 0) { __builtin_amdgcn_raw_ptr_buffer_load_lds(k2.cur, dst, 16, voffA, soA, 0, 0); return; }
+      if (pi == 1) { __builtin_amdgcn_raw_ptr_buffer_load_lds(k2.cur, dst, 16, voffA, soA + k2.lo_plane, 0, 0); return; }
+    }
     if (pi == 0) __builtin_amdgcn_raw_ptr_buffer_load_lds(rA, dst, 16, voffA, soA, 0, 0);
     else if (pi == 1) __builtin_amdgcn_raw_ptr_buffer_load_lds(rA, dst, 16, voffA, soA + q.a_plane, 0, 0);
     else if (pi == 2) __builtin_amdgcn_raw_ptr_buffer_load_lds(rB, dst, 16, voffB, soB, 0, 0);
@@ -127,6 +143,11 @@
     soA += sA;
     if (TAPS) {
       if (++ich == cpt) { ich = 0; soA = 0; ++itap; voffA = tap_voff(itap); }
+    }
+    if constexpr (VAR == V2_K2) {
+      const bool second = ist >= q.k2_chunk;
+      k2.cur = second ? k2.second : rA;
+      k2.lo_plane = second ? q.a2_plane : q.a_plane;
     }
   };
 
@@ -241,7 +262,15 @@
 #pragma unroll
         for (int e = 0; e < 4; ++e) lds[(8 * qq + 4 * h + e) * RS + nt * 32 + j] = acc[mt][nt][(2 * hh + qq) * 4 + e];
   };
-  gemm_epilogue_wave<EPI, TN, 3>(p, write_pass, reinterpret_cast<float*>(smv2), bm * BM + wm * 64, bn * BN + wn * TN * 32, wave, lane);
+  if constexpr (VAR == V2_NSPLIT) {
+    GemmKP pe = p;
+    const bool hi_side = bn * BN >= q.n_split;
+    if (hi_side) { pe.y = q.y2; pe.ldy = q.ldy2; pe.res = q.res2; pe.ldr = q.ldr2; pe.y_hi = q.y2_hi; pe.y_lo = q.y2_lo; }
+    if (!(hi_side ? q.mask_hi : q.mask_lo)) pe.row_len = nullptr;
+    gemm_epilogue_wave<EPI, TN, 3>(pe, write_pass, reinterpret_cast<float*>(smv2), bm * BM + wm * 64, bn * BN + wn * TN * 32, wave, lane);
+  } else {
+    gemm_epilogue_wave<EPI, TN, 3>(p, write_pass, reinterpret_cast<float*>(smv2), bm * BM + wm * 64, bn * BN + wn * TN * 32, wave, lane);
+  }
   V2_STAMP(6);
 #ifdef V2_TIMING
   asm volatile("s_waitcnt vmcnt(0)" ::: "memory");
@@ -249,7 +278,7 @@
   V2_STAMP(3); V2_RSTAMP(5);
 }
 
-template <bool TAPS, int EPI, int CFG>
+template <bool TAPS, int EPI, int CFG, int VAR = V2_PLAIN>
 __global__ __launch_bounds__(CFG ? 256 : 512, CFG ? 3 : 2) void gemm_bf16x3_v2_kernel(const GemmV2P q) {
   const GemmKP& p = q.g;
   const int L = blockIdx.x, xcd = L & 7, qq = L >> 3;
@@ -262,7 +291,7 @@
     if (bn >= p.nblocks) return;
   } else { bn = qq / p.mt8; bm = (qq - bn * p.mt8) * 8 + xcd; }
   if (bm >= p.mtiles) return;
-  gemm_v2_tile<TAPS, EPI, CFG>(q, bm, bn, threadIdx.x);
+  gemm_v2_tile<TAPS, EPI, CFG, VAR>(q, bm, bn, threadIdx.x);
 }
 
 StreamScratch g_plane_scratch(8);
@@ -270,7 +299,12 @@
 int gemm_bf16x3_v2_forward(GemmKP p, const void* wplanes, const LinearWeights& w, const GemmArgs& a, hipStream_t stream, double flops,
                            double bytes) {
   IDX_CHECK(w.K % 16 == 0 && (a.taps <= 1 || (w.K / a.taps) % 16 == 0), "v2 needs K % 16 == 0");
-  const int xk = a.taps > 1 ? w.K / a.taps : w.K;
+  const int var = a.x2_planes ? V2_K2 : a.n_split ? V2_NSPLIT : V2_PLAIN;
+  if (var != V2_PLAIN)
+    IDX_CHECK(a.taps <= 1 && !a.rope && a.act == ACT_NONE && !(a.x2_planes && a.n_split), "a second operand / a column split: plain linear launches only");
+  if (var == V2_K2) IDX_CHECK(a.x_planes && a.k2_chunk > 0 && a.k2_chunk < w.K / 16, "x2_planes: both inputs as planes, k2_chunk inside K");
+  if (var == V2_NSPLIT) IDX_CHECK(a.n_split % 128 == 0 && a.n_split < w.N && (a.y2 || a.y2_planes), "n_split: a multiple of the 128-column tile, inside N");
+  const int xk = a.taps > 1 ? w.K / a.taps : var == V2_K2 ? a.k2_chunk * 16 : w.K;
   const size_t plane = (size_t)(xk / 16) * a.M * 16 * sizeof(__bf16);
   void* scratch = nullptr;
   if (!a.x_planes && g_plane_scratch.acquire(stream, 2 * plane, &scratch)) return 1;
@@ -285,7 +319,7 @@
   GemmV2P q;
   q.g = p;
   if (a.y_planes) {
-    const int n_out = (a.act == ACT_SWIGLU || a.act == ACT_GATE) ? w.N / 2 : w.N;
+    const int n_out = (a.act == ACT_SWIGLU || a.act == ACT_GATE) ? w.N / 2 : var == V2_NSPLIT ? a.n_split : w.N;
     IDX_CHECK(n_out % 16 == 0 && (a.ldy & 3) == 0, "output planes need N_out % 16 == 0");
     q.g.y_hi = static_cast<__bf16*>(a.y_planes);
     q.g.y_lo = q.g.y_hi + plane_elems(a.M, n_out);
@@ -310,6 +344,26 @@
   const size_t b_plane = (size_t)(w.K / 16) * q.npad * 32;
   IDX_CHECK(2 * plane < (1ull << 31) && 2 * b_plane < (1ull << 31), "operand planes beyond the 2 GiB a buffer offset addresses");
   q.a_plane = (int)plane; q.a_bytes = (int)(2 * plane);
+  q.a2_hi = nullptr; q.k2_chunk = 0; q.a2_bytes = 0; q.a2_plane = 0;
+  q.n_split = 0; q.ldy2 = q.ldr2 = 0; q.mask_lo = q.mask_hi = 1; q.y2 = nullptr; q.res2 = nullptr; q.y2_hi = q.y2_lo = nullptr;
+  if (var == V2_K2) {
+    const size_t lead = (size_t)a.k2_chunk * a.M * 32;
+    const size_t plane2 = (size_t)(w.K / 16 - a.k2_chunk) * a.M * 32;
+    IDX_CHECK(lead + 2 * plane2 < (1ull << 31), "operand planes beyond the 2 GiB a buffer offset addresses");
+    q.a2_hi = reinterpret_cast<const __bf16*>(static_cast<const char*>(a.x2_planes) - lead);
+    q.k2_chunk = a.k2_chunk; q.a2_plane = (int)plane2; q.a2_bytes = (int)(lead + 2 * plane2);
+  }
+  if (var == V2_NSPLIT) {
+    const int n2 = w.N - a.n_split;
+    IDX_CHECK((!a.y2 || (a.ldy2 & 3) == 0) && (!a.y2_planes || n2 % 16 == 0), "second output: ldy2 % 4 == 0, planes need columns % 16 == 0");
+    q.n_split = a.n_split; q.ldy2 = a.ldy2; q.ldr2 = a.ldr2; q.mask_lo = a.mask_lo; q.mask_hi = a.mask_hi;
+    q.y2 = a.y2 ? a.y2 - a.n_split : nullptr;
+    q.res2 = a.res2 ? a.res2 - a.n_split : nullptr;
+    if (a.y2_planes) {
+      q.y2_hi = static_cast<__bf16*>(a.y2_planes) - plane_elems(a.M, a.n_split);
+      q.y2_lo = q.y2_hi + plane_elems(a.M, n2);
+    }
+  }
   q.b_plane = (int)b_plane; q.b_bytes = (int)(2 * b_plane);
   q.cs = 1;
   static const double cs_bytes = [] { const char* e = getenv("IDXTTS_GEMM_CS_BYTES"); return e ? atof(e) : 3.2e6; }();
@@ -334,7 +388,13 @@
   IDX_HIP(lds_limit[0].set(4 * (4 * 256 * 32), V2_ROW(false, 0), V2_ROW(true, 0)));
   IDX_HIP(lds_limit[1].set(3 * (4 * 128 * 32), V2_ROW(false, 1), V2_ROW(true, 1)));
 #undef V2_ROW
-  hipLaunchKernelGGL(kernels[cfg][a.taps > 1 ? 1 : 0][epi], dim3((unsigned)grid), dim3(cfg ? 256 : 512), lds, stream, q);
+  KernelFn fn = kernels[cfg][a.taps > 1 ? 1 : 0][epi];
+  if (var != V2_PLAIN) {
+    static DynLdsLimit lds_limit_var;
+    IDX_HIP(lds_limit_var.set(3 * (4 * 128 * 32), gemm_bf16x3_v2_kernel<false, EPI_PLAIN, 1, V2_K2>, gemm_bf16x3_v2_kernel<false, EPI_PLAIN, 1, V2_NSPLIT>));
+    fn = var == V2_K2 ? gemm_bf16x3_v2_kernel<false, EPI_PLAIN, 1, V2_K2> : gemm_bf16x3_v2_kernel<false, EPI_PLAIN, 1, V2_NSPLIT>;
+  }
+  hipLaunchKernelGGL(fn, dim3((unsigned)grid), dim3(cfg ? 256 : 512), lds, stream, q);
   IDX_LAUNCH_CHECK();
   return 0;
 }
diff --git a/index-tts_amd/csrc/s2mel.h b/index-tts_amd/csrc/s2mel.h
--- a/index-tts_amd/csrc/s2mel.h
+++ b/index-tts_amd/csrc/s2mel.h
@@ -11,13 +11,16 @@
 namespace idxtts {
 
 struct DiTBlock {
-  LinearWeights wqkv, wo, w13, w2, skip_a, skip_b;
+  LinearWeights wqkv, wo, w13, w2;
+  LinearWeights skip_in;
+  LinearWeights skip_a, skip_b;
   const float *attn_g = nullptr, *ffn_g = nullptr;
 };
 
 struct WNLayer {
   LinearWeights in_gate;
   LinearWeights res, skip;
+  LinearWeights res_skip;
   bool has_res = true;
 };
 
@@ -28,6 +31,7 @@
   idxtts_s2mel_config cfg;
   std::vector<DiTBlock> blocks;
   const float* final_g = nullptr;
+  LinearWeights merge_x, merge_c;
   LinearWeights mod_all, cond_proj, merge, temb0, temb2, t2emb0, t2emb2, skiplin_a, skiplin_b, conv1, res_proj, final_lin,
       final_mod, conv2, wn_cond;
   std::vector<WNLayer> wn;
@@ -67,5 +71,9 @@
 void set_s2mel_overlap(int on);
 int get_s2mel_overlap();
 int s2mel_release_stream(hipStream_t st);
+enum { S2MEL_FUSE_SKIP_IN = 1, S2MEL_FUSE_RES_SKIP = 2, S2MEL_FUSE_MERGE = 4, S2MEL_FUSE_ALL = 7 };
+void set_s2mel_fused(int mask);
+int get_s2mel_fused();
+long long s2mel_fused_launches(int form);
 
 }
diff --git a/index-tts_amd/csrc/s2mel.hip b/index-tts_amd/csrc/s2mel.hip
--- a/index-tts_amd/csrc/s2mel.hip
+++ b/index-tts_amd/csrc/s2mel.hip
@@ -1,6 +1,8 @@
 #include <cmath>
+#include <cstdlib>
 #include <cstring>
 
+#include <atomic>
 #include <map>
 #include <mutex>
 #include <utility>
@@ -81,6 +83,7 @@
     if (i > depth / 2) {
       HostTensor *sw = nullptr, *sb = nullptr;
       if (need(t, p + ".skip_in_linear.weight", {D, 2 * D}, &sw) || need(t, p + ".skip_in_linear.bias", {D}, &sb)) return 1;
+      if (make_linear(arena, sw->data.data(), sb->data.data(), D, 2 * D, {WP16_ALWAYS}, &B.skip_in)) return 1;
       if (make_linear(arena, col_slice(sw->data, D, 2 * D, 0, D).data(), sb->data.data(), D, D, {WP16_ALWAYS}, &B.skip_a)) return 1;
       if (make_linear(arena, col_slice(sw->data, D, 2 * D, D, 2 * D).data(), nullptr, D, D, {WP16_ALWAYS}, &B.skip_b)) return 1;
     }
@@ -94,6 +97,12 @@
   const int Win = 2 * C + D + cfg.style_dim;
   if (linear_from(t, arena, e + ".cond_projection", D, cfg.content_dim, true, WP16_ALWAYS, &cond_proj)) return 1;
   if (linear_from(t, arena, e + ".cond_x_merge_linear", D, Win, true, WP16_ALWAYS, &merge)) return 1;
+  if (C % 16 == 0 && (Win - C) % 16 == 0) {
+    HostTensor *mw = nullptr, *mb = nullptr;
+    if (need(t, e + ".cond_x_merge_linear.weight", {D, Win}, &mw) || need(t, e + ".cond_x_merge_linear.bias", {D}, &mb)) return 1;
+    if (make_linear(arena, col_slice(mw->data, D, Win, 0, C).data(), nullptr, D, C, {WP16_ALWAYS}, &merge_x)) return 1;
+    if (make_linear(arena, col_slice(mw->data, D, Win, C, Win).data(), mb->data.data(), D, Win - C, {WP16_ALWAYS}, &merge_c)) return 1;
+  }
   if (linear_from(t, arena, e + ".t_embedder.mlp.0", D, 256, true, WP16_ALWAYS, &temb0) || linear_from(t, arena, e + ".t_embedder.mlp.2", D, D, true, WP16_ALWAYS, &temb2)) return 1;
   if (linear_from(t, arena, e + ".t_embedder2.mlp.0", Wh, 256, true, WP16_ALWAYS, &t2emb0) || linear_from(t, arena, e + ".t_embedder2.mlp.2", Wh, Wh, true, WP16_ALWAYS, &t2emb2)) return 1;
   {
@@ -139,6 +148,7 @@
       if (l < L - 1) {
         std::vector<float> w_res(rw->data.begin(), rw->data.begin() + (size_t)Wh * Wh), b_res(rb->data.begin(), rb->data.begin() + Wh);
         std::vector<float> w_skip(rw->data.begin() + (size_t)Wh * Wh, rw->data.end()), b_skip(rb->data.begin() + Wh, rb->data.end());
+        if (make_linear(arena, rw->data.data(), rb->data.data(), 2 * Wh, Wh, {WP16_ALWAYS}, &W.res_skip)) return 1;
         if (make_linear(arena, w_res.data(), b_res.data(), Wh, Wh, {WP16_ALWAYS}, &W.res) || make_linear(arena, w_skip.data(), b_skip.data(), Wh, Wh, {WP16_ALWAYS}, &W.skip)) return 1;
       } else {
         W.has_res = false;
@@ -200,6 +210,8 @@
 
 struct CfmBuffers {
   float *x_in, *ha, *hb, *hmid, *hn, *qkv, *att, *ff, *xres, *wn_x, *wn_acts, *wn_out, *vout, *condp, *xstate;
+  float* base;
+  bool base_ready = false;
   void *hn_p, *att_p, *ff_p, *acts_p;
   void *h_p, *wnx_p, *xres_p;
   std::vector<void*> skips_p;
@@ -239,6 +251,7 @@
   b.vout = k.take<float>(M2 * C);
   b.condp = k.take<float>((size_t)B * T * D);
   b.xstate = k.take<float>((size_t)B * C * T);
+  b.base = k.take<float>(M2 * D);
   for (int i = 0; i < c.depth / 2; ++i) b.skips.push_back(k.take<float>(M2 * D));
   for (int i = 0; i < c.depth / 2; ++i) b.skips_p.push_back(k.take<float>(M2 * D));
   b.t1 = k.take<float>((size_t)n_steps * D);
@@ -266,7 +279,7 @@
   auto shp = [&](void* p, int cols) -> void* { return static_cast<float*>(p) + R * cols; };
   v.x_in = sh(w.x_in, Win); v.ha = sh(w.ha, D); v.hb = sh(w.hb, D); v.hmid = sh(w.hmid, D); v.hn = sh(w.hn, D); v.qkv = sh(w.qkv, 3 * D);
   v.att = sh(w.att, D); v.ff = sh(w.ff, m.ffn); v.xres = sh(w.xres, D); v.wn_x = sh(w.wn_x, Wh); v.wn_acts = sh(w.wn_acts, Wh);
-  v.wn_out = sh(w.wn_out, Wh); v.vout = sh(w.vout, C);
+  v.wn_out = sh(w.wn_out, Wh); v.vout = sh(w.vout, C); v.base = sh(w.base, D);
   v.hn_p = shp(w.hn_p, std::max(D, Wh)); v.att_p = shp(w.att_p, D); v.ff_p = shp(w.ff_p, m.ffn); v.acts_p = shp(w.acts_p, Wh);
   v.h_p = shp(w.h_p, D); v.wnx_p = shp(w.wnx_p, Wh); v.xres_p = shp(w.xres_p, D);
   for (size_t i = 0; i < w.skips.size(); ++i) { v.skips[i] = sh(w.skips[i], D); v.skips_p[i] = shp(w.skips_p[i], D); }
@@ -280,6 +293,24 @@
   a.x = xp ? nullptr : x; a.ldx = ldx; a.y = y; a.ldy = ldy; a.M = M; a.act = act; a.res = res; a.ldr = ldr;
   a.x_planes = xp; a.y_planes = yp;
   return gemm_forward(w, a, st);
+}
+
+static int g_s2mel_fused = [] { const char* e = getenv("IDXTTS_S2MEL_FUSED"); return e ? atoi(e) & S2MEL_FUSE_ALL : (int)S2MEL_FUSE_ALL; }();
+static std::atomic<long long> g_fused_launches[3];
+void set_s2mel_fused(int mask) { g_s2mel_fused = mask & S2MEL_FUSE_ALL; }
+int get_s2mel_fused() { return g_s2mel_fused; }
+long long s2mel_fused_launches(int form) { return form >= 0 && form < 3 ? g_fused_launches[form].load() : -1; }
+
+static int merge_base(S2MelModel& m, CfmBuffers& w, int rows, int M, hipStream_t st) {
+  const auto& c = m.cfg;
+  const int D = c.hidden_dim, C = c.in_channels, Win = 2 * C + D + c.style_dim;
+  w.base_ready = false;
+  GemmArgs pr;
+  pr.M = M;
+  if (!(g_s2mel_fused & S2MEL_FUSE_MERGE) || !gemm_uses_planes(m.merge_x, pr) || !gemm_uses_planes(m.merge_c, pr)) return 0;
+  if (gemm(m.merge_c, w.x_in + C, Win, w.base, D, rows, st)) return 1;
+  w.base_ready = true;
+  return 0;
 }
 
 static int dit_eval(S2MelModel& m, CfmBuffers& w, int N2, int T, int step, hipStream_t st, hipEvent_t lag_event) {
@@ -329,7 +360,10 @@
   auto ada = [&](const float* x, const float* g, int mod_idx) { return ada_rows(x, g, mod_idx, M, chain); };
   if (lag_event && depth < 2) IDX_HIP(hipEventRecord(lag_event, st));
   bool h_compact = false;
-  if (gemm(m.merge, w.x_in, Win, w.ha, D, M, st)) return 1;
+  if (w.base_ready) {
+    if (gemm(m.merge_x, w.x_in, Win, w.ha, D, M, st, ACT_NONE, w.base, D)) return 1;
+    ++g_fused_launches[2];
+  } else if (gemm(m.merge, w.x_in, Win, w.ha, D, M, st)) return 1;
   float* h = w.ha;
   int pushed = 0;
   for (int i = 0; i < depth; ++i) {
@@ -337,9 +371,16 @@
     if (i > half) {
       float* skip = w.skips[--pushed];
       void* skip_p = chain ? w.skips_p[pushed] : nullptr;
-      if (gemm(B.skip_a, h, D, w.hmid, D, M, st, ACT_NONE, nullptr, 0, chain ? w.h_p : nullptr)) return 1;
       float* dst = (h == w.ha) ? w.hb : w.ha;
-      if (gemm(B.skip_b, skip, D, dst, D, M, st, ACT_NONE, w.hmid, D, skip_p)) return 1;
+      GemmArgs g;
+      g.x_planes = w.h_p; g.x2_planes = skip_p; g.k2_chunk = D / 16; g.ldx = D; g.y = dst; g.ldy = D; g.M = M;
+      if (chain && (g_s2mel_fused & S2MEL_FUSE_SKIP_IN) && gemm_uses_planes(B.skip_in, g)) {
+        if (gemm_forward(B.skip_in, g, st)) return 1;
+        ++g_fused_launches[0];
+      } else {
+        if (gemm(B.skip_a, h, D, w.hmid, D, M, st, ACT_NONE, nullptr, 0, chain ? w.h_p : nullptr)) return 1;
+        if (gemm(B.skip_b, skip, D, dst, D, M, st, ACT_NONE, w.hmid, D, skip_p)) return 1;
+      }
       h = dst;
     }
     if (ada(h, B.attn_g, 2 * i)) return 1;
@@ -426,6 +467,13 @@
     if (W.has_res) {
       GemmArgs r;
       r.x = chain_t ? nullptr : w.wn_acts; r.x_planes = chain_t ? w.acts_p : nullptr; r.ldx = Wh; r.y = w.wn_x; r.y_planes = chain_wn_t ? w.wnx_p : nullptr; r.ldy = Wh; r.res = w.wn_x; r.ldr = Wh; r.M = Mt; r.seq_len = Tt; r.row_len = lens_t;
+      if ((g_s2mel_fused & S2MEL_FUSE_RES_SKIP) && Wh % 128 == 0 && gemm_uses_planes(W.res_skip, r)) {
+        r.n_split = Wh; r.y2 = w.wn_out; r.ldy2 = Wh; r.mask_hi = false;
+        if (l > 0) { r.res2 = w.wn_out; r.ldr2 = Wh; }
+        if (gemm_forward(W.res_skip, r, st)) return 1;
+        ++g_fused_launches[1];
+        continue;
+      }
       if (gemm_forward(W.res, r, st)) return 1;
     }
     GemmArgs sk;
@@ -560,6 +608,7 @@
     pk.B = B; pk.T = T; pk.C = C; pk.D = D; pk.S = cfg.style_dim; pk.Tp_max = Tp_max;
     pk.x_only = s > 0;
     if (cfm_pack(pk, st)) return 1;
+    if (s == 0 && merge_base(*this, w, 2 * B * T, two_streams ? B * T : 2 * B * T, st)) return 1;
     if (dit_eval_halves(*this, w, B, T, s, two_streams, st)) return 1;
     CfmEulerArgs eu;
     eu.x = w.xstate; eu.v = w.vout; eu.v_null = two_streams ? w.vout + (size_t)B * T * C : nullptr; eu.ldv = C; eu.prompt_len = w.plen; eu.B = B; eu.T = T; eu.C = C; eu.dt = dt_host[s]; eu.cfg_rate = cfg_rate;
@@ -656,6 +705,7 @@
   pk.B = B; pk.T = T; pk.C = C; pk.D = D; pk.S = cfg.style_dim; pk.Tp_max = Tp_max;
   if (cfm_pack(pk, st)) return 1;
   {
+    if (merge_base(*this, w, B * T, B * T, st)) return 1;
     CfmBuffers v0 = half_view(*this, w, 0, B, T);
     if (dit_eval(*this, v0, B, T, 0, st, nullptr)) return 1;
   }
diff --git a/index-tts_amd/indextts_amd/_lib.py b/index-tts_amd/indextts_amd/_lib.py
--- a/index-tts_amd/indextts_amd/_lib.py
+++ b/index-tts_amd/indextts_amd/_lib.py
@@ -23,6 +23,7 @@
     "idxtts_gpt_session_admit_beam",
     "idxtts_s2mel_create", "idxtts_s2mel_cond_workspace_bytes", "idxtts_s2mel_prepare_cond",
     "idxtts_s2mel_cfm_workspace_bytes", "idxtts_s2mel_cfm", "idxtts_set_gemm_mode", "idxtts_get_gemm_mode", "idxtts_set_decode_geometry", "idxtts_get_decode_geometry", "idxtts_set_decode_plane_rows", "idxtts_get_decode_plane_rows", "idxtts_s2mel_set_overlap", "idxtts_s2mel_get_overlap",
+    "idxtts_s2mel_set_fused", "idxtts_s2mel_get_fused", "idxtts_s2mel_fused_launches",
     "idxtts_s2mel_estimator", "idxtts_s2mel_cfm_rows_workspace_bytes", "idxtts_s2mel_cfm_rows", "idxtts_s2mel_regulate", "idxtts_cond_create", "idxtts_cond_workspace_bytes", "idxtts_cond_forward", "idxtts_emovec_merge",
     "idxtts_gpt_graph_cache_entries", "idxtts_w2vbert_create", "idxtts_w2vbert_workspace_bytes", "idxtts_w2vbert_forward",
     "idxtts_repcodec_create", "idxtts_repcodec_workspace_bytes", "idxtts_repcodec_quantize",
@@ -371,3 +372,18 @@
 
 def get_s2mel_overlap() -> bool:
     return bool(load().idxtts_s2mel_get_overlap())
+
+
+def set_s2mel_fused(mask: int) -> None:
+    check(load().idxtts_s2mel_set_fused(int(mask)))
+
+
+def get_s2mel_fused() -> int:
+    return int(load().idxtts_s2mel_get_fused())
+
+
+def s2mel_fused_launches(form: int) -> int:
+    lib = load()
+    lib.idxtts_s2mel_fused_launches.restype = ctypes.c_longlong
+    lib.idxtts_s2mel_fused_launches.argtypes = [c_int]
+    return int(lib.idxtts_s2mel_fused_launches(int(form)))
```

After: 185.1, median of 6. Within noise of the previous version (+0.8%).
